# Bergvca/string_grouper

Hardware: AMD Instinct MI355X
Metric: hot-path rows/sec (the device path of match_strings: tokenise + tf-idf + postings + SpGEMM-topn, inputs resident in HBM), 663k-name self-join ntop=10 min_sim=0.8; match_strings end to end: match_strings_rows_per_s (higher is better)
Workload: dtype f32

## Files before the change

string_grouper_amd/csrc/sg_api.hip:

```cpp
#include <stdarg.h>
#include <stdlib.h>

#include "sg_internal.h"
#include "sg_scan.h"

static thread_local char g_err[512] = "";

void sg_set_error(const char *fmt, ...) {
    va_list ap;
    va_start(ap, fmt);
    vsnprintf(g_err, sizeof(g_err), fmt, ap);
    va_end(ap);
}

extern "C" const char *sg_last_error(void) { return g_err; }
extern "C" int sg_abi_version(void) { return SG_ABI_VERSION; }

extern "C" int sg_device_count(int *count) {
    SG_REQUIRE(count != nullptr, "count is null");
    int n = 0;
    hipError_t e = hipGetDeviceCount(&n);
    if (e != hipSuccess) {
        (void)hipGetLastError();
        n = 0;
// ... 345 lines not shown
    SG_HIP_TRY(hipMemcpyAsync(dp, indptr, sizeof(int64_t) * (size_t)(n_rows + 1), hipMemcpyHostToDevice, ctx->stream));
    if (nnz > 0) {
        SG_HIP_TRY(hipMemcpyAsync(di, indices, sizeof(int32_t) * (size_t)nnz, hipMemcpyHostToDevice, ctx->stream));
        SG_HIP_TRY(hipMemcpyAsync(dd, data, dtype_size(dtype) * (size_t)nnz, hipMemcpyHostToDevice, ctx->stream));
    }
    SG_HIP_TRY(hipStreamSynchronize(ctx->stream));
    *out = m;
    return SG_OK;
}

extern "C" int sg_csr_from_device(sg_ctx *ctx, int64_t n_rows, int64_t n_cols, int64_t nnz, const int64_t *d_indptr,
                                  const int32_t *d_indices, const void *d_data, int32_t dtype, sg_csr **out) {
    SG_REQUIRE(ctx && d_indptr && out, "null argument");
    SG_REQUIRE(n_rows >= 0 && n_cols >= 0 && nnz >= 0, "negative shape");
    SG_REQUIRE(dtype == SG_F32 || dtype == SG_F64, "dtype must be SG_F32 or SG_F64");
    if (n_cols > INT32_MAX || n_rows > INT32_MAX) {
        sg_set_error("matrix shape exceeds int32 indices");
        return SG_ERR_OVERFLOW;
    }
    sg_csr *m = new (std::nothrow) sg_csr();
    if (!m) return SG_ERR_OOM;
    m->ctx = ctx;
    m->n_rows = n_rows;
    m->n_cols = n_cols;
    m->nnz = nnz;
    m->dtype = dtype;
    m->d_indptr = d_indptr;
    m->d_indices = d_indices;
    m->d_data = d_data;
    m->owned = false;
    *out = m;
    return SG_OK;
}

extern "C" int sg_csr_dims(const sg_csr *m, int64_t *n_rows, int64_t *n_cols, int64_t *nnz, int32_t *dtype) {
    SG_REQUIRE(m != nullptr, "matrix is null");
    if (n_rows) *n_rows = m->n_rows;
    if (n_cols) *n_cols = m->n_cols;
    if (nnz) *nnz = m->nnz;
    if (dtype) *dtype = m->dtype;
    return SG_OK;
}

extern "C" int sg_csr_device_ptrs(const sg_csr *m, const int64_t **d_indptr, const int32_t **d_indices,
                                  const void **d_data) {
    SG_REQUIRE(m != nullptr, "matrix is null");
    if (d_indptr) *d_indptr = m->d_indptr;
    if (d_indices) *d_indices = m->d_indices;
    if (d_data) *d_data = m->d_data;
    return SG_OK;
}

extern "C" int sg_csr_to_host(sg_ctx *ctx, const sg_csr *m, int64_t *indptr, int32_t *indices, void *data) {
    SG_REQUIRE(ctx && m && indptr, "null argument");
    SG_HIP_TRY(hipMemcpyAsync(indptr, m->d_indptr, sizeof(int64_t) * (size_t)(m->n_rows + 1), hipMemcpyDeviceToHost,
                              ctx->stream));
    SG_HIP_TRY(hipStreamSynchronize(ctx->stream));
    const int64_t base = indptr[0];
    const int64_t nnz = indptr[m->n_rows] - base;
    if (nnz > 0) {
        SG_REQUIRE(indices && data, "null output");
        SG_HIP_TRY(hipMemcpyAsync(indices, m->d_indices + base, sizeof(int32_t) * (size_t)nnz, hipMemcpyDeviceToHost,
                                  ctx->stream));
        SG_HIP_TRY(hipMemcpyAsync(data, (const char *)m->d_data + dtype_size(m->dtype) * (size_t)base,
                                  dtype_size(m->dtype) * (size_t)nnz, hipMemcpyDeviceToHost, ctx->stream));
        SG_HIP_TRY(hipStreamSynchronize(ctx->stream));
    }
    if (base != 0)
        for (int64_t i = 0; i <= m->n_rows; ++i) indptr[i] -= base;
    return SG_OK;
}

extern "C" int sg_csr_row_block(sg_ctx *ctx, const sg_csr *m, int64_t r0, int64_t r1, sg_csr **out) {
    SG_REQUIRE(ctx && m && out, "null argument");
    SG_REQUIRE(0 <= r0 && r0 <= r1 && r1 <= m->n_rows, "row range out of bounds");
    sg_csr *v = new (std::nothrow) sg_csr();
    if (!v) return SG_ERR_OOM;
    *v = *m;
    v->owned = false;
    v->left_groups = nullptr;
    v->left_state = 0;
    v->n_rows = r1 - r0;
    v->d_indptr = m->d_indptr + r0;
    int64_t ends[2] = {0, 0};
    SG_HIP_TRY(hipMemcpyAsync(&ends[0], m->d_indptr + r0, sizeof(int64_t), hipMemcpyDeviceToHost, ctx->stream));
    SG_HIP_TRY(hipMemcpyAsync(&ends[1], m->d_indptr + r1, sizeof(int64_t), hipMemcpyDeviceToHost, ctx->stream));
    SG_HIP_TRY(hipStreamSynchronize(ctx->stream));
    v->nnz = ends[1] - ends[0];
    *out = v;
    return SG_OK;
}

extern "C" int sg_csr_free(sg_csr *m) {
    if (!m) return SG_OK;
    if (m->left_groups) sg_collapse_free(m->left_groups);
    if (m->owned) {
        m->ctx->release((void *)m->d_indptr);
        m->ctx->release((void *)m->d_indices);
        m->ctx->release((void *)m->d_data);
        m->ctx->release(m->d_props_words);
    }
    delete m;
    return SG_OK;
}

struct SgZeroJobs {
    uint32_t *ptr[8];
    uint64_t words[8];
    uint64_t first[8];
    int n;
};
__global__ void __launch_bounds__(256) zero_ranges_kernel(SgZeroJobs jobs) {
    const uint64_t total = jobs.first[jobs.n < 8 ? jobs.n : 7] + (jobs.n == 8 ? jobs.words[7] : 0);
    for (uint64_t q = ((uint64_t)blockIdx.x * blockDim.x + threadIdx.x) * 4; q < total; q += (uint64_t)gridDim.x * blockDim.x * 4) {
        int r = 0;
#pragma unroll
        for (int i = 1; i < 8; ++i)
            if (i < jobs.n && q >= jobs.first[i]) r = i;
        const uint64_t w = q - jobs.first[r];
        uint32_t *p = jobs.ptr[r] + w;
        const uint64_t left = jobs.words[r] - w;
        if (left >= 4 && ((uintptr_t)p & 15u) == 0) {
            *reinterpret_cast<uint4 *>(p) = make_uint4(0u, 0u, 0u, 0u);
        } else {
            for (uint64_t e = 0; e < 4 && e < left; ++e) p[e] = 0u;
        }
    }
}

int sg_zero_ranges(sg_ctx *ctx, int n, void *const *ptrs, const size_t *bytes) {
    SgZeroJobs jobs;
    jobs.n = 0;
    uint64_t first = 0;
    for (int i = 0; i < n; ++i) {
        if (!ptrs[i] || bytes[i] == 0) continue;
        if (jobs.n == 8 || (bytes[i] & 3u) || ((uintptr_t)ptrs[i] & 3u)) {
            SG_HIP_TRY(hipMemsetAsync(ptrs[i], 0, bytes[i], ctx->stream));
            continue;
        }
        jobs.ptr[jobs.n] = (uint32_t *)ptrs[i];
        jobs.words[jobs.n] = bytes[i] / 4;
        jobs.first[jobs.n] = first;
        first += (jobs.words[jobs.n] + 3) & ~(uint64_t)3;
        ++jobs.n;
    }
    if (jobs.n == 0) return SG_OK;
    for (int i = jobs.n; i < 8; ++i) {
        jobs.ptr[i] = nullptr;
        jobs.words[i] = 0;
        jobs.first[i] = first;
    }
    uint64_t threads = first / 4;
    unsigned grid = (unsigned)((threads + 255) / 256);
    if (grid > (unsigned)ctx->num_cu * 16u) grid = (unsigned)ctx->num_cu * 16u;
    if (grid < 1) grid = 1;
    hipLaunchKernelGGL(zero_ranges_kernel, dim3(grid), dim3(256), 0, ctx->stream, jobs);
    SG_HIP_TRY(hipGetLastError());
    return SG_OK;
}

int sg_exclusive_scan_u32(sg_ctx *ctx, const uint32_t *d_in, uint32_t *d_out, int64_t n, uint32_t *d_total) {
    return scan_impl<uint32_t, uint32_t>(ctx, d_in, d_out, n, d_total);
}

int sg_exclusive_scan_positive_i32(sg_ctx *ctx, const int32_t *d_in, uint32_t *d_out, int64_t n, uint32_t *d_total) {
    return scan_impl<int32_t, uint32_t, true>(ctx, d_in, d_out, n, d_total);
}

int sg_exclusive_scan_i32_to_i64(sg_ctx *ctx, const int32_t *d_in, int64_t *d_out, int64_t n) {
    return scan_impl<int32_t, int64_t>(ctx, d_in, d_out, n, d_out + n);
}

extern "C" int sg_device_upload(sg_ctx *ctx, const void *host, int64_t bytes, void **d_out) {
    SG_REQUIRE(ctx && d_out && bytes >= 0 && (bytes == 0 || host != nullptr), "null argument or negative size");
    void *d = nullptr;
    SG_TRY(ctx->alloc((size_t)std::max<int64_t>(bytes, 16), &d));
    hipError_t e = bytes > 0 ? hipMemcpyAsync(d, host, (size_t)bytes, hipMemcpyHostToDevice, ctx->stream) : hipSuccess;
    if (e == hipSuccess) e = hipStreamSynchronize(ctx->stream);
    if (e != hipSuccess) {
        ctx->release(d);
        sg_set_error("sg_device_upload: %s", hipGetErrorString(e));
        return SG_ERR_HIP;
    }
    *d_out = d;
    return SG_OK;
}
```

string_grouper_amd/csrc/sg_collapse.hip:

```cpp
#include "sg_internal.h"
#include "sg_scan.h"

template <typename T>
__global__ void __launch_bounds__(256) row_hash_kernel(const int64_t *__restrict__ indptr, const int32_t *__restrict__ indices,
                                                       const T *__restrict__ data, int64_t n_rows, uint64_t *__restrict__ hash,
                                                       uint32_t *__restrict__ row_id ) {
    const int64_t r = ((int64_t)blockIdx.x * blockDim.x + threadIdx.x) >> 4;
    const int sub = threadIdx.x & 15;
    uint64_t h = 0;
    if (r < n_rows) {
        const int64_t lo = indptr[r], hi = indptr[r + 1];
        for (int64_t p = lo + sub; p < hi; p += 16) {
            uint64_t v;
            if (sizeof(T) == 4) v = (uint64_t)__float_as_uint((float)data[p]);
            else v = (uint64_t)__double_as_longlong((double)data[p]);
            uint64_t x = ((uint64_t)(uint32_t)indices[p] << 32) ^ v ^ ((uint64_t)(p - lo) * 0x9E3779B97F4A7C15ull);
            x ^= x >> 33;
            x *= 0xff51afd7ed558ccdull;
            x ^= x >> 33;
            x *= 0xc4ceb9fe1a85ec53ull;
            x ^= x >> 33;
            h += x;
        }
    }
#pragma unroll
    for (int d = 8; d > 0; d >>= 1) {
        const uint32_t lo32 = (uint32_t)__shfl_xor((int)(uint32_t)h, d, 64), hi32 = (uint32_t)__shfl_xor((int)(uint32_t)(h >> 32), d, 64);
        h += ((uint64_t)hi32 << 32) | lo32;
    }
    if (r < n_rows && sub == 0) {
        const int64_t len = indptr[r + 1] - indptr[r];
        hash[r] = h ^ ((uint64_t)len * 0xD6E8FEB86659FD93ull);
        if (row_id) row_id[r] = (uint32_t)r;
    }
}

#define SG_GROUP_SORT_LDS 8192
#define SG_GROUP_LARGE_MAX 28u
#define SG_GROUP_NO_SLOT 0xFFFFFFFFu

#define SG_GROUP_ROWS 2
template <typename T>
__global__ void __launch_bounds__(256) group_rows_kernel(const int64_t *__restrict__ indptr, const int32_t *__restrict__ indices,
                                                         const T *__restrict__ data, int64_t n_rows, unsigned long long *table,
                                                         uint32_t mask, uint32_t *__restrict__ slot_of_row) {
    const int64_t grp = ((int64_t)blockIdx.x * blockDim.x + threadIdx.x) >> 4;
    const int sub = threadIdx.x & 15;
    const int lead = (int)(threadIdx.x & 48u);
    int64_t r[SG_GROUP_ROWS], lo[SG_GROUP_ROWS];
    int32_t len[SG_GROUP_ROWS];
    bool valid[SG_GROUP_ROWS];
#pragma unroll
    for (int i = 0; i < SG_GROUP_ROWS; ++i) {
        r[i] = grp * SG_GROUP_ROWS + i;
        valid[i] = r[i] < n_rows;
        lo[i] = valid[i] ? indptr[r[i]] : 0;
        len[i] = valid[i] ? (int32_t)(indptr[r[i] + 1] - lo[i]) : 0;
    }
    int32_t k0[SG_GROUP_ROWS], k1[SG_GROUP_ROWS];
    T v0[SG_GROUP_ROWS], v1[SG_GROUP_ROWS];
#pragma unroll
    for (int i = 0; i < SG_GROUP_ROWS; ++i) {
        k0[i] = k1[i] = -1;
        v0[i] = v1[i] = (T)0;
        if (sub < len[i]) {
            k0[i] = indices[lo[i] + sub];
            v0[i] = data[lo[i] + sub];
        }
        if (sub + 16 < len[i]) {
            k1[i] = indices[lo[i] + sub + 16];
            v1[i] = data[lo[i] + sub + 16];
        }
    }
    unsigned long long mine[SG_GROUP_ROWS];
    uint32_t s[SG_GROUP_ROWS], result[SG_GROUP_ROWS];
    bool walking[SG_GROUP_ROWS];
#pragma unroll
    for (int i = 0; i < SG_GROUP_ROWS; ++i) {
        uint64_t h = 0;
        for (int32_t e = sub; e < len[i]; e += 16) {
            const int32_t k = e < 16 ? k0[i] : (e < 32 ? k1[i] : indices[lo[i] + e]);
            const T v = e < 16 ? v0[i] : (e < 32 ? v1[i] : data[lo[i] + e]);
            uint64_t vb;
            if (sizeof(T) == 4) vb = (uint64_t)__float_as_uint((float)v);
            else vb = (uint64_t)__double_as_longlong((double)v);
            uint64_t x = ((uint64_t)(uint32_t)k << 32) ^ vb ^ ((uint64_t)e * 0x9E3779B97F4A7C15ull);
            x ^= x >> 33;
            x *= 0xff51afd7ed558ccdull;
            x ^= x >> 33;
            x *= 0xc4ceb9fe1a85ec53ull;
            x ^= x >> 33;
            h += x;
        }
#pragma unroll
        for (int d = 8; d > 0; d >>= 1) {
            const uint32_t lo32 = (uint32_t)__shfl_xor((int)(uint32_t)h, d, 64), hi32 = (uint32_t)__shfl_xor((int)(uint32_t)(h >> 32), d, 64);
            h += ((uint64_t)hi32 << 32) | lo32;
        }
        h ^= (uint64_t)(uint32_t)len[i] * 0xD6E8FEB86659FD93ull;
        h ^= h >> 31;
        mine[i] = ((unsigned long long)(uint32_t)(h >> 32) << 32) | (unsigned long long)(~(uint32_t)r[i]);
        s[i] = (uint32_t)h & mask;
        result[i] = SG_GROUP_NO_SLOT;
        walking[i] = valid[i];
    }
    while (__ballot(walking[0] || walking[1]) != 0) {
        unsigned long long cur[SG_GROUP_ROWS];
#pragma unroll
        for (int i = 0; i < SG_GROUP_ROWS; ++i) {
            cur[i] = 0;
            if (walking[i] && sub == 0) cur[i] = __hip_atomic_load(&table[s[i]], __ATOMIC_RELAXED, __HIP_MEMORY_SCOPE_AGENT);
        }
#pragma unroll
        for (int i = 0; i < SG_GROUP_ROWS; ++i)
            if (walking[i] && sub == 0 && cur[i] == 0ull) cur[i] = atomicCAS(&table[s[i]], 0ull, mine[i]);
        uint32_t c_lo[SG_GROUP_ROWS], c_hi[SG_GROUP_ROWS];
        bool cmp[SG_GROUP_ROWS];
        int64_t o[SG_GROUP_ROWS], olo[SG_GROUP_ROWS];
        int32_t olen[SG_GROUP_ROWS];
#pragma unroll
        for (int i = 0; i < SG_GROUP_ROWS; ++i) {
            c_lo[i] = (uint32_t)__shfl((int)(uint32_t)cur[i], lead, 64);
            c_hi[i] = (uint32_t)__shfl((int)(uint32_t)(cur[i] >> 32), lead, 64);
            cmp[i] = walking[i] && !(c_lo[i] == 0u && c_hi[i] == 0u) && c_hi[i] == (uint32_t)(mine[i] >> 32);
            o[i] = (int64_t)(~c_lo[i]);
            olo[i] = cmp[i] ? indptr[o[i]] : 0;
            olen[i] = cmp[i] ? (int32_t)(indptr[o[i] + 1] - olo[i]) : -1;
        }
        int32_t ok0[SG_GROUP_ROWS], ok1[SG_GROUP_ROWS];
        T ov0[SG_GROUP_ROWS], ov1[SG_GROUP_ROWS];
#pragma unroll
        for (int i = 0; i < SG_GROUP_ROWS; ++i) {
            const bool go = cmp[i] && olen[i] == len[i];
            ok0[i] = ok1[i] = -1;
            ov0[i] = ov1[i] = (T)0;
            if (go && sub < len[i]) {
                ok0[i] = indices[olo[i] + sub];
                ov0[i] = data[olo[i] + sub];
            }
            if (go && sub + 16 < len[i]) {
                ok1[i] = indices[olo[i] + sub + 16];
                ov1[i] = data[olo[i] + sub + 16];
            }
        }
#pragma unroll
        for (int i = 0; i < SG_GROUP_ROWS; ++i) {
            if (!walking[i]) continue;
            if (c_lo[i] == 0u && c_hi[i] == 0u) {
                result[i] = s[i];
                walking[i] = false;
            } else if (cmp[i]) {
                bool same = olen[i] == len[i];
                if (same) {
                    same = ok0[i] == k0[i] && ov0[i] == v0[i] && ok1[i] == k1[i] && ov1[i] == v1[i];
                    for (int32_t e = sub + 32; e < len[i]; e += 16)
                        same = same && indices[olo[i] + e] == indices[lo[i] + e] && data[olo[i] + e] == data[lo[i] + e];
                }
#pragma unroll
                for (int d = 8; d > 0; d >>= 1) same = same && (__shfl_xor((int)same, d, 64) != 0);
                if (same) {
                    if (sub == 0 && o[i] > r[i]) atomicMax(&table[s[i]], mine[i]);
                    result[i] = s[i];
                }
                walking[i] = false;
            } else {
                s[i] = (s[i] + 1u) & mask;
            }
        }
    }
#pragma unroll
    for (int i = 0; i < SG_GROUP_ROWS; ++i)
        if (valid[i] && sub == 0) slot_of_row[r[i]] = result[i];
}

__device__ __forceinline__ uint32_t sg_group_rep(const unsigned long long *__restrict__ table, const uint32_t *__restrict__ slot_of_row,
                                                 int64_t r) {
    const uint32_t s = slot_of_row[r];
    return s == SG_GROUP_NO_SLOT ? (uint32_t)r : ~(uint32_t)table[s];
}
struct GroupRepLoad {
    const unsigned long long *table;
    const uint32_t *slot_of_row;
    uint32_t *rep_of_row;
    __device__ __forceinline__ uint32_t operator()(int64_t r) const {
        const uint32_t rep = sg_group_rep(table, slot_of_row, r);
        rep_of_row[r] = rep;
        return rep == (uint32_t)r ? 1u : 0u;
    }
};

__global__ void __launch_bounds__(256) group_scatter_kernel(const uint32_t *__restrict__ gid, const uint32_t *__restrict__ group_ptr,
                                                            int64_t n_rows, uint32_t *cursor, uint32_t *__restrict__ members) {
    const int64_t r = (int64_t)blockIdx.x * blockDim.x + threadIdx.x;
    if (r >= n_rows) return;
    const uint32_t g = gid[r];
    const uint32_t lo = group_ptr[g], m = group_ptr[g + 1] - lo;
    if (m > (uint32_t)SG_GROUP_SORT_LDS) return;
    members[lo + (m == 1u ? 0u : atomicAdd(&cursor[g], 1u))] = (uint32_t)r;
}

__global__ void __launch_bounds__(256) large_group_flag_kernel(const uint32_t *__restrict__ gid, int64_t n_rows, uint32_t g,
                                                               uint32_t *__restrict__ flag) {
    const int64_t r = (int64_t)blockIdx.x * blockDim.x + threadIdx.x;
    if (r < n_rows) flag[r] = gid[r] == g ? 1u : 0u;
}
__global__ void __launch_bounds__(256) large_group_fill_kernel(const uint32_t *__restrict__ gid, const uint32_t *__restrict__ at,
                                                               int64_t n_rows, uint32_t g, const uint32_t *__restrict__ group_ptr,
                                                               uint32_t *__restrict__ members) {
    const int64_t r = (int64_t)blockIdx.x * blockDim.x + threadIdx.x;
    if (r < n_rows && gid[r] == g) members[group_ptr[g] + at[r]] = (uint32_t)r;
// ... 235 lines not shown
    }
    return st;
}

static int collapse_unique_matrix(sg_ctx *ctx, const sg_csr *B, SgCollapse *c, int64_t nnz_u, int64_t *ptr ,
                                  bool defer_rows) {
    const int64_t n_u = c->n_u;
    int32_t *idx = nullptr;
    void *val = nullptr;
    const size_t vs = B->dtype == SG_F64 ? 8 : 4;
    int st = SG_OK;
    if (!ptr) st = sg_alloc(ctx, (size_t)n_u + 2, &ptr);
    if (st == SG_OK) st = sg_alloc(ctx, (size_t)nnz_u + 64, &idx);
    if (st == SG_OK) st = ctx->alloc(((size_t)nnz_u + 64) * vs, &val);
    sg_csr *m = st == SG_OK ? new (std::nothrow) sg_csr() : nullptr;
    if (st == SG_OK && !m) st = SG_ERR_OOM;
    if (st != SG_OK) {
        ctx->release(ptr);
        ctx->release(idx);
        ctx->release(val);
        return st;
    }
    m->ctx = ctx;
    m->n_rows = n_u;
    m->n_cols = B->n_cols;
    m->nnz = nnz_u;
    m->dtype = B->dtype;
    m->d_indptr = ptr;
    m->d_indices = idx;
    m->d_data = val;
    m->owned = true;
    m->props_state = B->props_state;
    m->props_max_norm2 = B->props_max_norm2;
    m->props_max_nnz = B->props_max_nnz;
    m->rows_of = c;
    c->unique = m;
    c->pending_src = B;
    if (!defer_rows) return sg_collapse_materialize(ctx, c);
    return SG_OK;
}

static int collapse_groups_table(sg_ctx *ctx, const sg_csr *B, bool forced, bool defer_rows, SgCollapse **out) {
    *out = nullptr;
    ctx->group_table_overflow = false;
    const int64_t n = B->n_rows;
    uint64_t table_size = 1024;
    while (table_size < 2 * (uint64_t)n) table_size <<= 1;
    unsigned long long *table = nullptr;
    uint32_t *slot_of_row = nullptr, *rep_of_row = nullptr, *rep_excl = nullptr, *size = nullptr, *cursor = nullptr, *queue = nullptr;
    uint32_t *totals = nullptr;
    SgCollapse *c = new (std::nothrow) SgCollapse();
    if (!c) return SG_ERR_OOM;
    c->ctx = ctx;
    c->n_orig = n;
    int st = sg_alloc(ctx, (size_t)table_size, &table);
    if (st == SG_OK) st = sg_alloc(ctx, (size_t)n + 1, &slot_of_row);
    if (st == SG_OK) st = sg_alloc(ctx, (size_t)n + 1, &rep_of_row);
    if (st == SG_OK) st = sg_alloc(ctx, (size_t)n + 1, &rep_excl);
    if (st == SG_OK) st = sg_alloc(ctx, (size_t)n + 2, &size);
    if (st == SG_OK) st = sg_alloc(ctx, (size_t)n + 2, &cursor);
    if (st == SG_OK) st = sg_alloc(ctx, (size_t)n + 2, &queue);
    if (st == SG_OK) st = sg_alloc(ctx, (size_t)(64 + 32 * 32), &totals);
    if (st == SG_OK) st = sg_alloc(ctx, (size_t)n + 1, &c->d_gid);
    if (st == SG_OK) st = sg_alloc(ctx, (size_t)n + 2, &c->d_group_ptr);
    if (st == SG_OK) st = sg_alloc(ctx, (size_t)n + 1, &c->d_members);
    if (st == SG_OK) st = sg_alloc(ctx, (size_t)n + 1, &c->d_rep_rows);
    if (st == SG_OK) st = sg_alloc(ctx, (size_t)n + 2, &c->d_rep_start);
    if (st == SG_OK) st = sg_alloc(ctx, (size_t)n + 2, &c->d_rep_len);
    auto cleanup = [&]() {
        ctx->release(table);
        ctx->release(slot_of_row);
        ctx->release(rep_of_row);
        ctx->release(rep_excl);
        ctx->release(size);
        ctx->release(cursor);
        ctx->release(queue);
        ctx->release(totals);
    };
    const unsigned g1 = (unsigned)((n + 255) / 256), g16 = (unsigned)((((n + SG_GROUP_ROWS - 1) / SG_GROUP_ROWS) * 16 + 255) / 256);
    if (st == SG_OK)
        st = SG_ZERO4(ctx, table, sizeof(unsigned long long) * (size_t)table_size, size, sizeof(uint32_t) * (size_t)(n + 2), cursor,
                      sizeof(uint32_t) * (size_t)(n + 2), totals, (64 + 32 * 32) * sizeof(uint32_t));
    if (st == SG_OK) {
        if (B->dtype == SG_F64)
            hipLaunchKernelGGL(group_rows_kernel<double>, dim3(g16), dim3(256), 0, ctx->stream, B->d_indptr, B->d_indices,
                               (const double *)B->d_data, n, table, (uint32_t)(table_size - 1), slot_of_row);
        else
            hipLaunchKernelGGL(group_rows_kernel<float>, dim3(g16), dim3(256), 0, ctx->stream, B->d_indptr, B->d_indices,
                               (const float *)B->d_data, n, table, (uint32_t)(table_size - 1), slot_of_row);
        st = sg_scan_launch<uint32_t>(ctx, GroupRepLoad{table, slot_of_row, rep_of_row}, SgScanStoreArray<uint32_t>{rep_excl}, n, totals);
    }
    if (st == SG_OK) {
        hipLaunchKernelGGL(group_ids_kernel, dim3(g1), dim3(256), 0, ctx->stream, (const uint32_t *)rep_of_row, (const uint32_t *)rep_excl,
                           (const uint32_t *)nullptr, n, c->d_gid, size, c->d_rep_rows, B->d_indptr, c->d_rep_start, c->d_rep_len,
                           (unsigned long long *)(totals + 64));
        st = sg_exclusive_scan_u32(ctx, size, c->d_group_ptr, n + 1, nullptr);
    }
    if (st == SG_OK) {
        hipLaunchKernelGGL(group_scatter_kernel, dim3(g1), dim3(256), 0, ctx->stream, (const uint32_t *)c->d_gid,
                           (const uint32_t *)c->d_group_ptr, n, cursor, c->d_members);
        hipLaunchKernelGGL(group_sort_small_kernel, dim3(g1), dim3(256), 0, ctx->stream, (const uint32_t *)c->d_group_ptr,
                           (const uint32_t *)totals, c->d_members, totals + 4, queue);
        hipLaunchKernelGGL(group_sort_lds_kernel, dim3(512), dim3(256), 0, ctx->stream, (const uint32_t *)c->d_group_ptr, c->d_members,
                           (const uint32_t *)(totals + 4), (const uint32_t *)queue);
        if (hipGetLastError() != hipSuccess) st = SG_ERR_HIP;
    }
    uint32_t h[64 + 32 * 32];
    for (auto &w : h) w = 0;
    static_assert(sizeof(h) <= SG_H_FETCH_WORDS * sizeof(uint32_t), "the pinned read-back buffer holds the grouping's words");
    if (st == SG_OK) {
        if (hipMemcpyAsync(ctx->h_fetch, totals, sizeof(h), hipMemcpyDeviceToHost, ctx->stream) != hipSuccess ||
            hipStreamSynchronize(ctx->stream) != hipSuccess)
            st = SG_ERR_HIP;
        else memcpy(h, ctx->h_fetch, sizeof(h));
    }
    const uint32_t n_groups = h[0];
    int64_t nnz_u = 0;
    for (int q = 0; q < 32; ++q) nnz_u += (int64_t)(((uint64_t)h[64 + 32 * q + 1] << 32) | (uint64_t)h[64 + 32 * q]);
    const uint32_t *h_words = h + 4;
    if (st != SG_OK || n_groups == 0 || (!forced && (double)n_groups > 0.97 * (double)n) || (int64_t)n_groups == n) {
        cleanup();
        sg_collapse_free(c);
        return st;
    }
    if (h_words[2] > SG_GROUP_LARGE_MAX) {
        ctx->group_table_overflow = true;
        cleanup();
        sg_collapse_free(c);
        return SG_OK;
    }
    c->n_u = n_groups;
    for (uint32_t q = 0; q < h_words[2] && st == SG_OK; ++q) {
        const uint32_t g = h_words[3 + q];
        hipLaunchKernelGGL(large_group_flag_kernel, dim3(g1), dim3(256), 0, ctx->stream, (const uint32_t *)c->d_gid, n, g, size);
        st = sg_exclusive_scan_u32(ctx, size, rep_excl, n, nullptr);
        if (st == SG_OK) {
            hipLaunchKernelGGL(large_group_fill_kernel, dim3(g1), dim3(256), 0, ctx->stream, (const uint32_t *)c->d_gid,
                               (const uint32_t *)rep_excl, n, g, (const uint32_t *)c->d_group_ptr, c->d_members);
            if (hipGetLastError() != hipSuccess) st = SG_ERR_HIP;
        }
    }
    cleanup();
    if (st == SG_OK) st = collapse_unique_matrix(ctx, B, c, nnz_u, nullptr, defer_rows);
    if (st != SG_OK) {
        sg_collapse_free(c);
        return st;
    }
    *out = c;
    return SG_OK;
}

static int collapse_groups(sg_ctx *ctx, const sg_csr *B, bool forced, bool by_table, bool defer_rows, SgCollapse **out) {
    if (by_table) return collapse_groups_table(ctx, B, forced, defer_rows, out);
    *out = nullptr;
    ctx->group_table_overflow = false;
    const int64_t n = B->n_rows;
    uint64_t *hash = nullptr, *hash_sorted = nullptr;
    uint32_t *row_id = nullptr, *row_sorted = nullptr, *head = nullptr, *run_excl = nullptr, *head_pos = nullptr;
    uint32_t *rep_of_row = nullptr, *rank_of_row = nullptr, *is_rep = nullptr, *rep_excl = nullptr, *size = nullptr;
    uint32_t *totals = nullptr;
    SgCollapse *c = nullptr;
    int st = sg_alloc(ctx, (size_t)n + 1, &hash);
    if (st == SG_OK) st = sg_alloc(ctx, (size_t)40, &totals);
    if (st == SG_OK) st = sg_alloc(ctx, (size_t)n + 1, &hash_sorted);
    if (st == SG_OK) st = sg_alloc(ctx, (size_t)n + 1, &row_id);
    if (st == SG_OK) st = sg_alloc(ctx, (size_t)n + 1, &row_sorted);
    if (st == SG_OK) st = sg_alloc(ctx, (size_t)n + 1, &head);
    if (st == SG_OK) st = sg_alloc(ctx, (size_t)n + 1, &run_excl);
    auto cleanup = [&]() {
        ctx->release(hash);
        ctx->release(hash_sorted);
        ctx->release(row_id);
// ... 254 lines not shown
```

string_grouper_amd/csrc/sg_internal.h:

```cpp
#pragma once

#include <hip/hip_runtime.h>
#include <stdint.h>
#include <stdio.h>
#include <stdlib.h>
#include <string.h>

#include <map>
#include <mutex>
#include <new>
#include <string>
#include <vector>

#include "../../include/sg_hip.h"

#define SG_WAVE 64
#define SG_NUM_XCD 8

void sg_set_error(const char *fmt, ...);

#define SG_HIP_TRY(expr)                                                                        \
    do {                                                                                        \
        hipError_t _e = (expr);                                                                 \
        if (_e != hipSuccess) {                                                                 \
// ... 44 lines not shown
    uint32_t *h_fetch = nullptr;

    std::map<std::string, std::string> opts;
    const char *opt(const char *name) const {
        auto it = opts.find(name);
        return it == opts.end() ? nullptr : it->second.c_str();
    }
    int opt_int(const char *name, int dflt) const {
        const char *v = opt(name);
        return v && *v ? atoi(v) : dflt;
    }
    double opt_double(const char *name, double dflt) const {
        const char *v = opt(name);
        return v && *v ? atof(v) : dflt;
    }
    bool opt_is(const char *name, char c) const {
        const char *v = opt(name);
        return v && v[0] == c;
    }
    bool poison = false;

    unsigned long long *d_scan_desc = nullptr;
    size_t scan_desc_cap = 0;
    uint32_t scan_ticket_base = 0, scan_epoch = 0;
    struct IdfTable {
        int64_t n_docs;
        int32_t dtype;
        void *d;
        bool trusted;
    };
    std::vector<IdfTable> idf_tables;
    int inner_multiply_depth = 0;
    bool group_table_overflow = false;

    int alloc(size_t bytes, void **out);
    void release(void *p);
    void trim();
};

template <typename T>
static inline int sg_alloc(sg_ctx *ctx, size_t count, T **out) {
    void *p = nullptr;
    int s = ctx->alloc(count * sizeof(T), &p);
    *out = (T *)p;
    return s;
}

struct SgTimer {
    sg_ctx *ctx;
    int which;
    SgTimer(sg_ctx *c, int w) : ctx(c), which(w) { (void)hipEventRecord(ctx->ev_start[w], ctx->stream); }
    ~SgTimer() {
        (void)hipEventRecord(ctx->ev_stop[which], ctx->stream);
        ctx->ev_valid[which] = true;
    }
};

struct sg_strings {
    sg_ctx *ctx = nullptr;
    const uint8_t *d_bytes = nullptr;
    const int64_t *d_offsets = nullptr;
    int64_t n = 0;
    int64_t total_bytes = 0;
    bool owned = false;
    int32_t sym_width = 1;
    int32_t alphabet = 0;
    bool prelowered = false;
};

struct sg_csr {
    sg_ctx *ctx = nullptr;
    int64_t n_rows = 0, n_cols = 0, nnz = 0;
    int32_t dtype = SG_F32;
    const int64_t *d_indptr = nullptr;
    const int32_t *d_indices = nullptr;
    const void *d_data = nullptr;
    bool owned = false;
    mutable int props_state = 0;
    mutable float props_max_norm2 = 0.f;
    mutable uint32_t props_max_nnz = 0;
    bool from_vectoriser = false;
    mutable bool props_by_construction = false;
    uint32_t *d_props_words = nullptr;
    mutable int left_state = 0;
    mutable struct SgCollapse *left_groups = nullptr;
    struct SgCollapse *rows_of = nullptr;
};

struct SgScoreCtx {
    const uint32_t *fwd_ptr = nullptr;
    const void *fwd = nullptr;
    const uint32_t *orig_of = nullptr;
    const void *blk = nullptr;
    uint32_t blk_bytes = 0;
    const uint4 *q8 = nullptr;
    float q8_scale = 0.f;
    uint32_t pad_ = 0;
};
#define SG_Q8_STRIDE 256u
#define SG_Q8_MAX_ENTRIES 60u

struct SgCollapse {
    sg_ctx *ctx = nullptr;
    int64_t n_orig = 0, n_u = 0;
    uint32_t *d_gid = nullptr;
    uint32_t *d_group_ptr = nullptr;
    uint32_t *d_members = nullptr;
    uint32_t *d_rep_rows = nullptr;
    int64_t *d_rep_start = nullptr;
    int32_t *d_rep_len = nullptr;
    struct sg_csr *unique = nullptr;
    const struct sg_csr *pending_src = nullptr;
};

struct sg_postings {
    sg_ctx *ctx = nullptr;
    int64_t n_right = 0, n_terms = 0, nnz = 0;
    int32_t dtype = SG_F32;
    int32_t tile_log2 = 12;
    int32_t n_tiles = 0;
    const int64_t *b_indptr = nullptr;
    const int32_t *b_indices = nullptr;
    const void *b_data = nullptr;
    uint32_t *d_seg = nullptr;
    uint32_t *d_term_len = nullptr;
    uint32_t *d_term_start = nullptr;
    int32_t *d_rows = nullptr;
    void *d_vals = nullptr;
    sg_csr src;
    int32_t split = 1;
    void *d_fwd = nullptr;
    uint32_t *d_fwd_ptr = nullptr;
    void *d_blk = nullptr;
    uint32_t blk_bytes = 0;
    void *d_q8 = nullptr;
    uint32_t *d_filt = nullptr;
    sg_csr *permuted = nullptr;
    uint32_t *d_orig_of = nullptr, *d_pos_of = nullptr;
    struct SgScoreCtx *d_score_ctx = nullptr;
    uint32_t *d_ends = nullptr;
    int32_t nt_pad = 0;
    int32_t fold_log2 = 0;
    uint32_t *d_ends8 = nullptr;
    int32_t nv_pad = 0;
    float norm_up = 0.f;
    uint32_t freq_min = 0;
    bool cosine_like = false;
    float max_norm2 = 0.f;
    SgCollapse *collapse = nullptr;
    const sg_csr *caller_b = nullptr;
    sg_csr caller_b_copy;
    int64_t n_right_caller = 0;
    mutable sg_postings *plain = nullptr;
    mutable sg_postings *exact_native = nullptr;
    mutable sg_postings *alt_tile = nullptr;
    sg_csr built_from;
    bool built_from_valid = false;
    bool tile_form = false;
    const sg_postings *view_of = nullptr;
    int32_t build_tile_cols = 0, build_flags = 0;
};

struct sg_topn {
    sg_ctx *ctx = nullptr;
    int64_t n_rows = 0, n_cols = 0;
    int32_t stride = 0;
    int32_t dtype = SG_F32;
    int32_t top_n_asked = 0;
    int32_t *d_cols = nullptr;
    void *d_vals = nullptr;
    int32_t *d_counts = nullptr;
};

struct sg_vocab {
    sg_ctx *ctx = nullptr;
    sg_vec_params params;
    int32_t bits_per_char = 7;
    int64_t n_terms = 0, n_docs = 0;
    int64_t key_space = 0;
    bool sorted_mode = false;
    int32_t *d_key_to_col = nullptr;
    uint64_t *d_keys = nullptr;
    int32_t *d_df = nullptr;
    void *d_idf = nullptr;
    bool idf_trusted = false;
    struct VocabImpl *impl = nullptr;
};

int sg_matchlist_device_view(const sg_matchlist *ml, int64_t *n_rows, int64_t *n_cols, int64_t *n_entries, int32_t *dtype,
                             const int64_t **row_ptr, const int32_t **cols, const void **vals);

#define SG_POSTINGS_NO_COLLAPSE (1 << 8)
#define SG_POSTINGS_TILE_FORM (1 << 11)
#define SG_POSTINGS_EXACT_ONLY (1 << 10)
int sg_csr_props(sg_ctx *ctx, const sg_csr *m, bool *cosine_like, float *max_norm2, uint32_t *max_nnz = nullptr);
bool sg_pruned_supports_tile(int32_t tile_log2);
int sg_postings_ensure_full(sg_ctx *ctx, const sg_postings *p);
bool sg_q8_applies(const sg_ctx *ctx, const sg_postings *Bt, double threshold);
int sg_spgemm_pruned_launch(sg_ctx *ctx, const sg_csr *A, const sg_postings *Bt, int32_t keep, sg_topn *r,
                            double threshold, double delta, uint32_t *row_counter,
                            uint32_t *flagged_count, uint32_t *flagged_rows, unsigned long long *stats);

int sg_spgemm_pruned_symmetric(sg_ctx *ctx, const sg_csr *A, const sg_postings *Bt, int32_t keep, sg_topn *r,
                               double threshold, double delta, unsigned long long *stats, bool *done, int64_t row_lo = 0,
                               int64_t row_hi = -1 , int32_t **export_pairs = nullptr,
                               int64_t *export_n = nullptr, int64_t row_step = 1 ,
                               bool exact_all = false );
int sg_selfjoin_merge_pairs(sg_ctx *ctx, sg_topn *r, const int32_t *d_pairs, int64_t n_pairs, int64_t row_lo, int64_t row_hi,
                            const uint32_t *pos_of ,
                            int64_t row_step = 1);

#define SG_PAIR_CHUNK 256u
#define SG_PAIR_NO_CHUNK 0xFFFFFFFFu
struct SgPairSink {
    uint32_t *d_i = nullptr;
    uint32_t *d_j = nullptr;
    void *d_s = nullptr;
    uint32_t *d_row_count = nullptr;
    uint32_t *d_chunk_count = nullptr;
    uint32_t *d_chunks_used = nullptr;
    unsigned long long *d_totals = nullptr;
    uint32_t chunks = 0;
};
unsigned sg_spgemm_exact_selfjoin_grid(const sg_ctx *ctx, const sg_postings *Bt = nullptr );
int sg_spgemm_exact_selfjoin_rows(sg_ctx *ctx, const sg_csr *A, const sg_postings *Bt, int32_t keep, sg_topn *r,
                                  double threshold, uint32_t *row_counter, const uint32_t *row_list,
                                  const uint32_t *row_list_len, const SgPairSink &sink, bool all_rows = false);

int sg_collapse_build(sg_ctx *ctx, const sg_csr *B, SgCollapse **out, bool left_side = false, bool defer_rows = false);
int sg_collapse_materialize(sg_ctx *ctx, SgCollapse *c);
int sg_csr_ensure_rows(sg_ctx *ctx, const sg_csr *m);
void sg_collapse_free(SgCollapse *c);
int sg_collapse_expand(sg_ctx *ctx, const SgCollapse *c, const sg_topn *ru, bool rows_are_groups, sg_topn *out,
                       const int32_t *row_list = nullptr);
int sg_sort_pairs_u64_u32(sg_ctx *ctx, const uint64_t *d_keys, const uint32_t *d_vals, int64_t n, uint64_t *d_keys_out,
                          uint32_t *d_vals_out);
int sg_sort_unique_u64(sg_ctx *ctx, uint64_t *d_keys, int64_t n, uint64_t *d_unique, int32_t *d_counts, int64_t *n_unique);

int sg_zero_ranges(sg_ctx *ctx, int n, void *const *ptrs, const size_t *bytes);
#define SG_ZERO2(ctx, p0, b0, p1, b1) [&]() { void *const pp_[] = {(void *)(p0), (void *)(p1)}; const size_t bb_[] = {(size_t)(b0), (size_t)(b1)}; return sg_zero_ranges(ctx, 2, pp_, bb_); }()
#define SG_ZERO3(ctx, p0, b0, p1, b1, p2, b2) [&]() { void *const pp_[] = {(void *)(p0), (void *)(p1), (void *)(p2)}; const size_t bb_[] = {(size_t)(b0), (size_t)(b1), (size_t)(b2)}; return sg_zero_ranges(ctx, 3, pp_, bb_); }()
#define SG_ZERO4(ctx, p0, b0, p1, b1, p2, b2, p3, b3) [&]() { void *const pp_[] = {(void *)(p0), (void *)(p1), (void *)(p2), (void *)(p3)}; const size_t bb_[] = {(size_t)(b0), (size_t)(b1), (size_t)(b2), (size_t)(b3)}; return sg_zero_ranges(ctx, 4, pp_, bb_); }()
int sg_exclusive_scan_positive_i32(sg_ctx *ctx, const int32_t *d_in, uint32_t *d_out, int64_t n, uint32_t *d_total);
int sg_exclusive_scan_u32(sg_ctx *ctx, const uint32_t *d_in, uint32_t *d_out, int64_t n, uint32_t *d_total);
int sg_exclusive_scan_i32_to_i64(sg_ctx *ctx, const int32_t *d_in, int64_t *d_out, int64_t n);
```

string_grouper_amd/csrc/sg_postings.hip:

```cpp
#include <stdlib.h>

#include "sg_internal.h"
#include "sg_scan.h"

__device__ __forceinline__ int64_t row_of_thread(int64_t g, int32_t tile_log2, int32_t n_tiles) {
    return ((g % n_tiles) << tile_log2) | (g / n_tiles);
}

template <typename T>
__global__ void __launch_bounds__(256) postings_count(const int64_t *__restrict__ indptr,
                                                      const int32_t *__restrict__ indices, int64_t n_rows,
                                                      int32_t tile_log2, int32_t n_tiles, uint32_t *seg_counts) {
    const int64_t j = row_of_thread((int64_t)blockIdx.x * blockDim.x + threadIdx.x, tile_log2, n_tiles);
    if (j >= n_rows) return;
    const int64_t lo = indptr[j], hi = indptr[j + 1];
    const uint32_t t = (uint32_t)(j >> tile_log2);
    for (int64_t p = lo; p < hi; ++p) {
        const int64_t bin = (int64_t)indices[p] * n_tiles + t;
        atomicAdd(&seg_counts[bin], 1u);
    }
}

template <typename T>
__device__ __forceinline__ void store_posting(int32_t *rows, T *vals, uint32_t pos, int32_t j, T v);
// ... 205 lines not shown
    uint32_t *freq_bits = cursor + n_terms;
    const int64_t t = blockIdx.x / split;
    const int32_t part = blockIdx.x % split;
    for (int k = threadIdx.x; k < (n_terms + 31) / 32; k += blockDim.x) freq_bits[k] = 0;
    const uint32_t *mine = cnt + (int64_t)blockIdx.x * n_terms;
    for (int k = threadIdx.x; k < n_terms; k += blockDim.x) cursor[k] = term_start[k] + mine[k];
    __syncthreads();
    if (out_filt)
        for (int k = threadIdx.x; k < n_terms; k += blockDim.x)
            if (is_frequent[k]) atomicOr(&freq_bits[k >> 5], 1u << (k & 31));
    __syncthreads();
    const int64_t part_rows = ((int64_t)1 << tile_log2) / split;
    const int64_t j0 = (t << tile_log2) + part * part_rows;
    int64_t j1 = j0 + part_rows;
    if (j1 > n_rows) j1 = n_rows;
    const int lane = threadIdx.x & 63, sub = lane & 15;
    (void)lane;
    const int64_t groups = blockDim.x >> 4;
    const int64_t trips = (j1 - j0 + groups * SG_POST_ROWS - 1) / (groups * SG_POST_ROWS);
    for (int64_t it = 0; it < trips; ++it) {
        const int64_t jb = j0 + (it * groups + (threadIdx.x >> 4)) * SG_POST_ROWS;
        int64_t lo[SG_POST_ROWS], hi[SG_POST_ROWS];
#pragma unroll
        for (int r = 0; r < SG_POST_ROWS; ++r) {
            const bool valid = jb + r < j1;
            lo[r] = valid ? indptr[jb + r] : 0;
            hi[r] = valid ? indptr[jb + r + 1] : 0;
        }
        int32_t k0[SG_POST_ROWS];
        T v0[SG_POST_ROWS];
#pragma unroll
        for (int r = 0; r < SG_POST_ROWS; ++r) {
            const bool have = lo[r] + sub < hi[r];
            k0[r] = have ? indices[lo[r] + sub] : -1;
            v0[r] = have ? data[lo[r] + sub] : (T)0;
        }
        float fq[SG_POST_ROWS];
#pragma unroll
        for (int r = 0; r < SG_POST_ROWS; ++r) {
            fq[r] = 0.f;
#if defined(SG_K3_PROBE_NO_FQ)
            if (out_filt && n_rows < 0) {
#else
            if (out_filt) {
#endif
                double f2 = 0.0;
                if (k0[r] >= 0 && ((freq_bits[k0[r] >> 5] >> (k0[r] & 31)) & 1u)) f2 = (double)v0[r] * (double)v0[r];
                for (int64_t p = lo[r] + sub + 16; p < hi[r]; p += 16) {
                    const int32_t k = indices[p];
                    if ((freq_bits[k >> 5] >> (k & 31)) & 1u) f2 += (double)data[p] * (double)data[p];
                }
#pragma unroll
                for (int d = 8; d > 0; d >>= 1) {
                    const uint64_t bits = (uint64_t)__double_as_longlong(f2);
                    const uint32_t l = (uint32_t)__shfl_xor((int)(uint32_t)bits, d, 64), h = (uint32_t)__shfl_xor((int)(uint32_t)(bits >> 32), d, 64);
                    f2 += __longlong_as_double((long long)(((uint64_t)h << 32) | l));
                }
                fq[r] = frequent_norm_ratio_of(f2, inv_norm_up);
            }
        }
#pragma unroll
        for (int r = 0; r < SG_POST_ROWS; ++r) {
            const uint32_t col = (uint32_t)(jb + r - (t << tile_log2));
            if (k0[r] >= 0) {
#if defined(SG_K3_PROBE_NO_ATOMIC)
                const uint32_t pos = cursor[k0[r]] + (uint32_t)(threadIdx.x & 3);
#else
                const uint32_t pos = atomicAdd(&cursor[k0[r]], 1u);
#endif
#if defined(SG_K3_PROBE_NO_STORE)
                if (pos == 0xFFFFFFF0u)
#endif
                emit_posting<T>(out_rows, out_vals, out_filt, pos, col, v0[r], fq[r], tile_log2, inv_norm_up, (uint32_t)t, fold_log2);
            }
            for (int64_t p = lo[r] + sub + 16; p < hi[r]; p += 16) {
                const uint32_t pos = atomicAdd(&cursor[indices[p]], 1u);
                emit_posting<T>(out_rows, out_vals, out_filt, pos, col, data[p], fq[r], tile_log2, inv_norm_up, (uint32_t)t, fold_log2);
            }
        }
    }
}

__device__ __forceinline__ uint32_t lds_get16(const uint32_t *w, uint32_t k) { return (w[k >> 1] >> ((k & 1u) << 4)) & 0xffffu; }
template <typename T>
__global__ void __launch_bounds__(1024) postings_fill_staged(const int64_t *__restrict__ indptr, const int32_t *__restrict__ indices,
                                                             const T *__restrict__ data, int64_t n_rows, int32_t tile_log2,
                                                             int32_t n_terms, int32_t split, int32_t chunk_rows, uint32_t stage_cap,
                                                             uint32_t *cnt , const uint32_t *__restrict__ term_start,
                                                             const uint8_t *__restrict__ is_frequent, uint32_t *__restrict__ out_filt,
                                                             float inv_norm_up, int32_t fold_log2) {
    extern __shared__ uint32_t lds[];
    const uint32_t w16 = ((uint32_t)n_terms + 1u) >> 1;
    uint32_t *lcnt = lds;
    uint32_t *freq_bits = lcnt + ((w16 + 3u) & ~3u);
    float *fqrow = reinterpret_cast<float *>(freq_bits + (((uint32_t)n_terms + 31u) >> 5));
    uint32_t *wave_tot = reinterpret_cast<uint32_t *>(fqrow + chunk_rows);
    uint32_t *stage = wave_tot + 32;
    const int64_t t = blockIdx.x / split;
    const int32_t part = blockIdx.x % split;
    uint32_t *mine = cnt + (int64_t)blockIdx.x * n_terms;
    for (uint32_t k = threadIdx.x; k < (((uint32_t)n_terms + 31u) >> 5); k += blockDim.x) freq_bits[k] = 0;
    __syncthreads();
    for (int k = threadIdx.x; k < n_terms; k += blockDim.x)
        if (is_frequent[k]) atomicOr(&freq_bits[k >> 5], 1u << (k & 31));
    __syncthreads();
    const int64_t part_rows = ((int64_t)1 << tile_log2) / split;
    const int64_t j0 = (t << tile_log2) + part * part_rows;
    int64_t j1 = j0 + part_rows;
    if (j1 > n_rows) j1 = n_rows;
    const int lane = threadIdx.x & 63, sub = lane & 15, wave = threadIdx.x >> 6;
    const int64_t groups = blockDim.x >> 4;
    const uint32_t last_k = (uint32_t)n_terms - 1u;
    bool any_big = false;
    for (int64_t c0 = j0; c0 < j1; c0 += chunk_rows) {
        const int64_t c1 = c0 + chunk_rows < j1 ? c0 + chunk_rows : j1;
        const int64_t e = indptr[c1] - indptr[c0];
        any_big = any_big || e > (int64_t)stage_cap || e > 65535;
    }
    for (int64_t c0 = j0; c0 < j1; c0 += chunk_rows) {
        const int64_t c1 = c0 + chunk_rows < j1 ? c0 + chunk_rows : j1;
        const int64_t trips = (c1 - c0 + groups * SG_POST_ROWS - 1) / (groups * SG_POST_ROWS);
        if (any_big) {
            for (int64_t it = 0; it < trips; ++it) {
                const int64_t jb = c0 + (it * groups + (threadIdx.x >> 4)) * SG_POST_ROWS;
#pragma unroll
                for (int r = 0; r < SG_POST_ROWS; ++r) {
                    const bool valid = jb + r < c1;
                    const int64_t lo = valid ? indptr[jb + r] : 0, hi = valid ? indptr[jb + r + 1] : 0;
                    double f2 = 0.0;
                    for (int64_t p = lo + sub; p < hi; p += 16) {
                        const int32_t k = indices[p];
                        if ((freq_bits[k >> 5] >> (k & 31)) & 1u) f2 += (double)data[p] * (double)data[p];
                    }
#pragma unroll
                    for (int d = 8; d > 0; d >>= 1) {
                        const uint64_t bits = (uint64_t)__double_as_longlong(f2);
                        const uint32_t l = (uint32_t)__shfl_xor((int)(uint32_t)bits, d, 64), h = (uint32_t)__shfl_xor((int)(uint32_t)(bits >> 32), d, 64);
                        f2 += __longlong_as_double((long long)(((uint64_t)h << 32) | l));
                    }
                    const float fq = frequent_norm_ratio_of(f2, inv_norm_up);
                    const uint32_t col = (uint32_t)(jb + r - (t << tile_log2));
                    for (int64_t p = lo + sub; p < hi; p += 16) {
                        const int32_t k = indices[p];
                        const uint32_t pos = term_start[k] + atomicAdd(&mine[k], 1u);
                        out_filt[pos] = filter_posting(col, (float)data[p], fq, tile_log2, inv_norm_up, (uint32_t)t, fold_log2);
                    }
                }
            }
            __syncthreads();
            continue;
        }
        for (uint32_t w = threadIdx.x; w < w16; w += blockDim.x) lcnt[w] = 0;
        __syncthreads();
        for (int64_t it = 0; it < trips; ++it) {
            const int64_t jb = c0 + (it * groups + (threadIdx.x >> 4)) * SG_POST_ROWS;
            int64_t lo[SG_POST_ROWS], hi[SG_POST_ROWS];
#pragma unroll
            for (int r = 0; r < SG_POST_ROWS; ++r) {
                const bool valid = jb + r < c1;
                lo[r] = valid ? indptr[jb + r] : 0;
                hi[r] = valid ? indptr[jb + r + 1] : 0;
            }
            int32_t k0[SG_POST_ROWS];
            T v0[SG_POST_ROWS];
#pragma unroll
            for (int r = 0; r < SG_POST_ROWS; ++r) {
                const bool have = lo[r] + sub < hi[r];
                k0[r] = have ? indices[lo[r] + sub] : -1;
                v0[r] = have ? data[lo[r] + sub] : (T)0;
            }
#pragma unroll
            for (int r = 0; r < SG_POST_ROWS; ++r) {
                double f2 = 0.0;
                if (k0[r] >= 0) {
                    atomicAdd(&lcnt[(uint32_t)k0[r] >> 1], 1u << (((uint32_t)k0[r] & 1u) << 4));
                    if ((freq_bits[k0[r] >> 5] >> (k0[r] & 31)) & 1u) f2 = (double)v0[r] * (double)v0[r];
                }
                for (int64_t p = lo[r] + sub + 16; p < hi[r]; p += 16) {
                    const int32_t k = indices[p];
                    atomicAdd(&lcnt[(uint32_t)k >> 1], 1u << (((uint32_t)k & 1u) << 4));
                    if ((freq_bits[k >> 5] >> (k & 31)) & 1u) f2 += (double)data[p] * (double)data[p];
                }
#pragma unroll
                for (int d = 8; d > 0; d >>= 1) {
                    const uint64_t bits = (uint64_t)__double_as_longlong(f2);
                    const uint32_t l = (uint32_t)__shfl_xor((int)(uint32_t)bits, d, 64), h = (uint32_t)__shfl_xor((int)(uint32_t)(bits >> 32), d, 64);
                    f2 += __longlong_as_double((long long)(((uint64_t)h << 32) | l));
                }
                if (sub == 0 && jb + r < c1) fqrow[jb + r - c0] = frequent_norm_ratio_of(f2, inv_norm_up);
            }
        }
        __syncthreads();
        {
            const uint32_t per = (w16 + blockDim.x - 1u) / blockDim.x;
            const uint32_t wa = threadIdx.x * per, wb = wa + per < w16 ? wa + per : w16;
            uint32_t sum = 0;
            for (uint32_t w = wa; w < wb; ++w) sum += (lcnt[w] & 0xffffu) + (lcnt[w] >> 16);
            uint32_t tot;
            uint32_t run = block_exclusive_scan<uint32_t>(sum, wave_tot, &tot);
            for (uint32_t w = wa; w < wb; ++w) {
                const uint32_t c = lcnt[w];
                const uint32_t a = run;
                run += c & 0xffffu;
                const uint32_t b = run;
                run += c >> 16;
                lcnt[w] = a | (b << 16);
            }
        }
        __syncthreads();
        for (int64_t it = 0; it < trips; ++it) {
            const int64_t jb = c0 + (it * groups + (threadIdx.x >> 4)) * SG_POST_ROWS;
            int64_t lo[SG_POST_ROWS], hi[SG_POST_ROWS];
#pragma unroll
            for (int r = 0; r < SG_POST_ROWS; ++r) {
                const bool valid = jb + r < c1;
                lo[r] = valid ? indptr[jb + r] : 0;
                hi[r] = valid ? indptr[jb + r + 1] : 0;
            }
            int32_t k0[SG_POST_ROWS];
            T v0[SG_POST_ROWS];
#pragma unroll
            for (int r = 0; r < SG_POST_ROWS; ++r) {
                const bool have = lo[r] + sub < hi[r];
                k0[r] = have ? indices[lo[r] + sub] : -1;
                v0[r] = have ? data[lo[r] + sub] : (T)0;
            }
#pragma unroll
            for (int r = 0; r < SG_POST_ROWS; ++r) {
                const float fq = jb + r < c1 ? fqrow[jb + r - c0] : 0.f;
                const uint32_t col = (uint32_t)(jb + r - (t << tile_log2));
                if (k0[r] >= 0) {
                    const uint32_t sh = ((uint32_t)k0[r] & 1u) << 4;
                    const uint32_t pos = (atomicAdd(&lcnt[(uint32_t)k0[r] >> 1], 1u << sh) >> sh) & 0xffffu;
                    stage[pos] = filter_posting(col, (float)v0[r], fq, tile_log2, inv_norm_up, (uint32_t)t, fold_log2);
                }
                for (int64_t p = lo[r] + sub + 16; p < hi[r]; p += 16) {
                    const uint32_t k = (uint32_t)indices[p];
                    const uint32_t sh = (k & 1u) << 4;
                    const uint32_t pos = (atomicAdd(&lcnt[k >> 1], 1u << sh) >> sh) & 0xffffu;
                    stage[pos] = filter_posting(col, (float)data[p], fq, tile_log2, inv_norm_up, (uint32_t)t, fold_log2);
                }
            }
        }
        __syncthreads();
        {
            constexpr int FB = 8;
            const uint32_t n_tg = ((uint32_t)n_terms + 63u) >> 6, waves = (uint32_t)(blockDim.x >> 6);
            for (uint32_t tg0 = (uint32_t)wave; tg0 < n_tg; tg0 += waves * FB) {
                uint32_t end_k[FB], start_k[FB], before[FB], G[FB];
                bool mine_has[FB];
#pragma unroll
                for (int b = 0; b < FB; ++b) {
                    const uint32_t tg = tg0 + (uint32_t)b * waves;
                    const uint32_t k = tg * 64u + (uint32_t)lane;
                    const bool live = tg < n_tg;
                    const uint32_t kc = k < last_k ? k : last_k;
                    end_k[b] = live ? lds_get16(lcnt, kc) : 0u;
                    start_k[b] = (!live || k == 0u) ? 0u : lds_get16(lcnt, (k - 1u) < last_k ? k - 1u : last_k);
                    mine_has[b] = live && k <= last_k && end_k[b] > start_k[b];
                }
#pragma unroll
                for (int b = 0; b < FB; ++b) {
                    const uint32_t k = (tg0 + (uint32_t)b * waves) * 64u + (uint32_t)lane;
                    before[b] = mine_has[b] ? mine[k] : 0u;
                    G[b] = mine_has[b] ? term_start[k] : 0u;
                }
#pragma unroll
                for (int b = 0; b < FB; ++b) {
                    const uint32_t tg = tg0 + (uint32_t)b * waves;
                    if (tg >= n_tg) break;
                    const uint32_t k = tg * 64u + (uint32_t)lane;
                    G[b] += before[b];
                    const uint32_t S = (uint32_t)__builtin_amdgcn_readlane((int)start_k[b], 0);
                    const uint32_t Eg = (uint32_t)__builtin_amdgcn_readlane((int)end_k[b], 63);
                    for (uint32_t e0 = S; e0 < Eg; e0 += 64u) {
                        const uint32_t e = e0 + (uint32_t)lane;
                        uint32_t lo = 0u, hi = 63u;
#pragma unroll
                        for (int step = 0; step < 6; ++step) {
                            const uint32_t mid = (lo + hi) >> 1;
                            const uint32_t km = tg * 64u + mid;
                            const bool right = lds_get16(lcnt, km < last_k ? km : last_k) > e;
                            hi = right ? mid : hi;
                            lo = right ? lo : mid + 1u;
                        }
                        const uint32_t tsel = lo < 63u ? lo : 63u;
                        const uint32_t kt = tg * 64u + tsel;
                        const uint32_t start_t = kt == 0u ? 0u : lds_get16(lcnt, (kt - 1u) < last_k ? kt - 1u : last_k);
                        const uint32_t G_t = (uint32_t)__shfl((int)G[b], (int)tsel, 64);
                        if (e < Eg) out_filt[G_t + (e - start_t)] = stage[e];
                    }
                    if (mine_has[b]) mine[k] = before[b] + (end_k[b] - start_k[b]);
                }
            }
        }
        __syncthreads();
    }
}

__global__ void __launch_bounds__(256) term_len_kernel(const uint32_t *__restrict__ seg, int64_t n_terms, int32_t n_tiles,
                                                       uint32_t *__restrict__ term_len) {
    const int64_t k = (int64_t)blockIdx.x * blockDim.x + threadIdx.x;
    if (k < n_terms) term_len[k] = seg[(k + 1) * n_tiles] - seg[k * n_tiles];
}

template <typename T>
__global__ void __launch_bounds__(256) fwd_pack(const int64_t *__restrict__ indptr, const int32_t *__restrict__ indices,
                                                const T *__restrict__ data, int64_t n_rows, int64_t nnz,
                                                const uint32_t *__restrict__ orig_of ,
                                                uint32_t *__restrict__ fwd_ptr , void *__restrict__ fwd) {
    const int64_t i = (int64_t)blockIdx.x * blockDim.x + threadIdx.x;
    const int64_t base = indptr[0];
    if (i <= n_rows)
        reinterpret_cast<uint2 *>(fwd_ptr)[i] = make_uint2((uint32_t)(indptr[i] - base), i < n_rows ? (orig_of ? orig_of[i] : (uint32_t)i) : 0u);
    if (i >= nnz || fwd == nullptr) return;
    const int64_t p = base + i;
    if (sizeof(T) == 4) {
        reinterpret_cast<int2 *>(fwd)[i] = make_int2(indices[p], __float_as_int((float)data[p]));
    } else {
        const long long bits = __double_as_longlong((double)data[p]);
        reinterpret_cast<int4 *>(fwd)[i] = make_int4(indices[p], 0, (int)(bits & 0xffffffffll), (int)(bits >> 32));
    }
}

template <typename T>
__global__ void __launch_bounds__(256) row_blocks_kernel(const int64_t *__restrict__ indptr, const int32_t *__restrict__ indices,
                                                         const T *__restrict__ data, int64_t n_rows,
                                                         const uint32_t *__restrict__ orig_of ,
                                                         uint32_t blk_bytes, void *__restrict__ blk) {
    constexpr int ES = sizeof(T) == 4 ? 8 : 16;
    const int64_t chunks = blk_bytes / 16;
    const int64_t g = (int64_t)blockIdx.x * blockDim.x + threadIdx.x;
    const int64_t p = g / chunks;
    const int32_t c = (int32_t)(g - p * chunks);
    if (p >= n_rows) return;
    const int64_t lo = indptr[p];
    const int32_t nnz = (int32_t)(indptr[p + 1] - lo);
    const int32_t used = (((nnz + 1) * ES + 127) / 128) * 128;
    if (c * 16 >= used) return;
    uint4 w = make_uint4(0u, 0u, 0u, 0u);
    if (sizeof(T) == 4) {
        const int32_t e0 = 2 * c, e1 = 2 * c + 1;
        if (e0 == 0) {
            w.x = orig_of ? orig_of[p] : (uint32_t)p;
            w.y = (uint32_t)nnz;
        } else if (e0 <= nnz) {
            w.x = (uint32_t)indices[lo + e0 - 1];
            w.y = __float_as_uint((float)data[lo + e0 - 1]);
        }
        if (e1 <= nnz) {
            w.z = (uint32_t)indices[lo + e1 - 1];
            w.w = __float_as_uint((float)data[lo + e1 - 1]);
        }
    } else {
        if (c == 0) {
            w.x = orig_of ? orig_of[p] : (uint32_t)p;
            w.y = (uint32_t)nnz;
        } else if (c <= nnz) {
            const long long bits = __double_as_longlong((double)data[lo + c - 1]);
            w.x = (uint32_t)indices[lo + c - 1];
            w.z = (uint32_t)(bits & 0xffffffffll);
            w.w = (uint32_t)(bits >> 32);
        }
    }
    reinterpret_cast<uint4 *>(reinterpret_cast<char *>(blk) + (size_t)p * blk_bytes)[c] = w;
}

__global__ void __launch_bounds__(256) ends_from_seg_kernel(const uint32_t *__restrict__ seg, int64_t n_terms, int32_t n_tiles,
                                                            uint32_t *__restrict__ ends, int32_t nt_pad, uint32_t *__restrict__ ends8,
                                                            int32_t nv_pad, int32_t fold_log2) {
    const int64_t k = (int64_t)blockIdx.x * blockDim.x + threadIdx.x;
    if (k > n_terms) return;
    if (ends)
        for (int32_t t = 0; t < nt_pad; ++t)
            ends[k * nt_pad + t] = k == n_terms ? 0u : seg[k * n_tiles + (t < n_tiles ? t : n_tiles - 1) + 1] << 2;
// ... 235 lines not shown
    if (st == SG_OK) st = sg_alloc(ctx, (size_t)B->nnz + 64, &idx);
    if (st == SG_OK) st = ctx->alloc(((size_t)B->nnz + 64) * vs, &val);
    if (st == SG_OK)
        st = sg_scan_launch<int64_t>(ctx, PermutedLenLoad{n, minv, (uint64_t)(~0ull / n) + 1ull, by_group ? pending->d_rep_len : (const int32_t *)nullptr, B->d_indptr, pos_of, orig_of},
                                     SgScanStoreArray<int64_t>{ptr}, (int64_t)n, ptr + n);
    if (st == SG_OK) {
        const unsigned grid = (unsigned)((((n + 1 + SG_GATHER_ROWS - 1) / SG_GATHER_ROWS) * 16 + 255) / 256);
        const sg_csr *src = from_groups ? pending->pending_src : B;
        const uint32_t *rep_rows = from_groups ? pending->d_rep_rows : nullptr;
        const int64_t *rep_start = by_group ? pending->d_rep_start : nullptr;
        const int32_t *rep_len = by_group ? pending->d_rep_len : nullptr;
        if (B->dtype == SG_F64)
            hipLaunchKernelGGL(gather_rows_kernel<double>, dim3(grid), dim3(256), 0, ctx->stream, src->d_indptr, src->d_indices,
                               (const double *)src->d_data, B->n_rows, (const uint32_t *)orig_of, rep_rows, rep_start, rep_len,
                               (const int64_t *)ptr, idx, (double *)val, fwd_ptr, fwd, (uint4 *)(fwd_ptr ? q8 : nullptr), inv_norm);
        else
            hipLaunchKernelGGL(gather_rows_kernel<float>, dim3(grid), dim3(256), 0, ctx->stream, src->d_indptr, src->d_indices,
                               (const float *)src->d_data, B->n_rows, (const uint32_t *)orig_of, rep_rows, rep_start, rep_len,
                               (const int64_t *)ptr, idx, (float *)val, fwd_ptr, fwd, (uint4 *)(fwd_ptr ? q8 : nullptr), inv_norm);
        if (hipGetLastError() != hipSuccess) st = SG_ERR_HIP;
        if (st == SG_OK) *fwd_done = fwd_ptr != nullptr;
    }
    ctx->release(len_by_pos);
    sg_csr *m = st == SG_OK ? new (std::nothrow) sg_csr() : nullptr;
    if (st == SG_OK && !m) st = SG_ERR_OOM;
    if (st != SG_OK) {
        ctx->release(orig_of);
        ctx->release(pos_of);
        ctx->release(ptr);
        ctx->release(idx);
        ctx->release(val);
        return st;
    }
    m->ctx = ctx;
    m->n_rows = B->n_rows;
    m->n_cols = B->n_cols;
    m->nnz = B->nnz;
    m->dtype = B->dtype;
    m->d_indptr = ptr;
    m->d_indices = idx;
    m->d_data = val;
    m->owned = true;
    m->props_state = B->props_state;
    m->props_max_norm2 = B->props_max_norm2;
    m->props_max_nnz = B->props_max_nnz;
    *out_perm = m;
    *out_orig_of = orig_of;
    *out_pos_of = pos_of;
    return SG_OK;
}

extern "C" int sg_postings_build(sg_ctx *ctx, const sg_csr *B, int32_t tile_cols, sg_postings **out) {
    return sg_postings_build_flags(ctx, B, tile_cols, 0, out);
}

#define SG_POSTINGS_INNER (1 << 9)

static thread_local SgCollapse *tl_pending_groups = nullptr;

extern "C" int sg_postings_build_flags(sg_ctx *ctx, const sg_csr *B_in, int32_t tile_cols, int32_t flags, sg_postings **out) {
    SG_REQUIRE(ctx && B_in && out, "null argument");
    SgCollapse *pending = tl_pending_groups;
    tl_pending_groups = nullptr;
    if (!(flags & SG_POSTINGS_NO_COLLAPSE)) {
        bool cl = false;
        float n2 = 0.f;
        SG_TRY(sg_csr_props(ctx, B_in, &cl, &n2));
        SgCollapse *col = nullptr;
        SgTimer timer(ctx, SG_K_POSTINGS);
        if (cl) SG_TRY(sg_collapse_build(ctx, B_in, &col, false, true));
        if (col) {
            sg_postings *inner = nullptr;
            tl_pending_groups = col;
            const int st = sg_postings_build_flags(ctx, col->unique, tile_cols, flags | SG_POSTINGS_NO_COLLAPSE | SG_POSTINGS_INNER, &inner);
            tl_pending_groups = nullptr;
            if (st != SG_OK) {
                sg_collapse_free(col);
                return st;
            }
            inner->collapse = col;
            inner->caller_b_copy = *B_in;
            inner->caller_b_copy.owned = false;
            inner->caller_b_copy.d_props_words = nullptr;
            inner->caller_b_copy.left_groups = nullptr;
            inner->caller_b_copy.left_state = 0;
            inner->caller_b = &inner->caller_b_copy;
            inner->n_right_caller = B_in->n_rows;
            inner->build_tile_cols = tile_cols;
            inner->build_flags = flags;
            *out = inner;
            return SG_OK;
        }
        flags |= SG_POSTINGS_INNER;
        const int st = sg_postings_build_flags(ctx, B_in, tile_cols, flags | SG_POSTINGS_NO_COLLAPSE, out);
        if (st == SG_OK) {
            (*out)->build_tile_cols = tile_cols;
            (*out)->build_flags = flags & 0xff;
        }
        return st;
    }
    const sg_csr *B = B_in;
    bool cosine_like = false;
    float max_norm2 = 0.f;
    SG_TRY(sg_csr_props(ctx, B, &cosine_like, &max_norm2));
    const char *pr = ctx->opt("SG_PRUNE");
    const bool want_pruned = cosine_like && !(pr && pr[0] == '0') && !(flags & SG_POSTINGS_EXACT_ONLY);
    if (tile_cols == 0) {
        tile_cols = B->dtype == SG_F64 ? 1024 : 2048;
        if (want_pruned) {
            tile_cols = 4096;
            if (flags & SG_POSTINGS_TILE_FORM) tile_cols = 2048;
            else if (const char *v = ctx->opt("SG_PRUNE_TILE")) tile_cols = atoi(v) == 13 ? 8192 : (atoi(v) == 11 ? 2048 : 4096);
        }
    }
    SG_REQUIRE(tile_cols >= 256 && tile_cols <= 32768 && (tile_cols & (tile_cols - 1)) == 0,
               "tile_cols must be a power of two in [256, 32768]");
    int64_t max_entries = (int64_t)1 << 29;
    if (const char *v = ctx->opt("SG_MAX_POSTINGS")) {
        const long long o = atoll(v);
        if (o > 0 && o < max_entries) max_entries = o;
    }
    if (B->nnz + 64 >= max_entries) {
        sg_set_error("right-hand matrix has %lld non-zeros; one postings block holds < 2^29 (use more right-hand blocks)",
                     (long long)B->nnz);
        return SG_ERR_OVERFLOW;
    }
    int32_t tile_log2 = 0;
    while ((1 << tile_log2) < tile_cols) ++tile_log2;
    const int64_t n_tiles64 = B->n_rows == 0 ? 1 : ((B->n_rows + tile_cols - 1) >> tile_log2);
    const int64_t n_bins = B->n_cols * n_tiles64;
    if (n_bins + 1 >= (int64_t)1 << 31) {
        sg_set_error("segment table of %lld x %lld entries is too large; use more right-hand blocks",
                     (long long)B->n_cols, (long long)n_tiles64);
        return SG_ERR_OVERFLOW;
    }
    sg_csr *permuted = nullptr;
    uint32_t *orig_of = nullptr, *pos_of = nullptr;
    SgTimer *timer = (flags & SG_POSTINGS_INNER) ? nullptr : new (std::nothrow) SgTimer(ctx, SG_K_POSTINGS);
    struct TimerGuard {
        SgTimer *t;
        ~TimerGuard() { delete t; }
    } timer_guard{timer};
    void *early_fwd = nullptr;
    uint32_t *early_fwd_ptr = nullptr;
    void *early_q8 = nullptr;
    const float norm_up_build = __builtin_nextafterf(sqrtf(max_norm2) * 1.000001f, 2.f);
    const bool q8_forced = ctx->opt("SG_Q8") && ctx->opt("SG_Q8")[0] == '1';
    const bool want_q8 = want_pruned && !(flags & SG_POSTINGS_TILE_FORM) && B_in->n_cols < ((int64_t)1 << 24) && !(ctx->opt("SG_Q8") && ctx->opt("SG_Q8")[0] == '0') &&
                         (q8_forced || (double)B_in->nnz <= 45.0 * (double)B_in->n_rows) &&
                         (ctx->total_mem == 0 || (size_t)SG_Q8_STRIDE * ((size_t)B_in->n_rows + 1) < ctx->total_mem / 16);
    bool fwd_done = false;
    bool aux_written = false;
    {
        const bool filt = want_pruned && sg_pruned_supports_tile(tile_log2) &&
                          (B->n_cols + 1) * ((n_tiles64 + 3) & ~(int64_t)3) < ((int64_t)1 << 30);
        const bool blk = ctx->opt("SG_ROW_BLOCKS") && ctx->opt("SG_ROW_BLOCKS")[0] == '1';
        if (filt && !blk && !(flags & SG_POSTINGS_NO_PERMUTATION) && B_in->n_rows > 0) {
            int st0 = ctx->alloc(((size_t)B_in->nnz + 8) * (B_in->dtype == SG_F64 ? 16 : 8), &early_fwd);
            if (st0 == SG_OK) st0 = sg_alloc(ctx, 2 * ((size_t)B_in->n_rows + 2), &early_fwd_ptr);
            if (st0 == SG_OK && want_q8) st0 = ctx->alloc((size_t)SG_Q8_STRIDE * ((size_t)B_in->n_rows + 1), &early_q8);
            if (st0 != SG_OK) {
                ctx->release(early_fwd);
                ctx->release(early_fwd_ptr);
                return st0;
            }
        }
    }
    if (!(flags & SG_POSTINGS_NO_PERMUTATION)) {
        const int stp = build_permuted(ctx, B_in, tile_cols, &permuted, &orig_of, &pos_of, pending, early_fwd_ptr, early_fwd, &fwd_done,
                                       early_q8, 1.0f / norm_up_build);
        if (stp != SG_OK) {
            ctx->release(early_fwd);
            ctx->release(early_fwd_ptr);
            ctx->release(early_q8);
            return stp;
        }
    }
    if (!fwd_done) {
        ctx->release(early_fwd);
        ctx->release(early_fwd_ptr);
        ctx->release(early_q8);
        early_fwd = nullptr;
        early_fwd_ptr = nullptr;
        early_q8 = nullptr;
    }
    if (pending && pending->pending_src && !permuted) {
        const int stm = sg_collapse_materialize(ctx, pending);
        if (stm != SG_OK) {
            sg_csr_free(permuted);
            ctx->release(orig_of);
            ctx->release(pos_of);
            return stm;
        }
    }
    if (permuted) B = permuted;
    sg_postings *p = new (std::nothrow) sg_postings();
    if (!p) {
        sg_csr_free(permuted);
        ctx->release(orig_of);
        ctx->release(pos_of);
        ctx->release(early_fwd);
        ctx->release(early_fwd_ptr);
        ctx->release(early_q8);
        return SG_ERR_OOM;
    }
    p->permuted = permuted;
    p->d_orig_of = orig_of;
    p->d_pos_of = pos_of;
    p->ctx = ctx;
    p->n_right = B->n_rows;
    p->n_terms = B->n_cols;
    p->nnz = B->nnz;
    p->dtype = B->dtype;
    p->tile_log2 = tile_log2;
    p->tile_form = (flags & SG_POSTINGS_TILE_FORM) != 0;
    p->built_from = *B_in;
    p->built_from.owned = false;
    p->built_from.d_props_words = nullptr;
    p->built_from.left_groups = nullptr;
    p->built_from.left_state = 0;
    p->built_from_valid = true;
    p->n_tiles = (int32_t)n_tiles64;
    p->b_indptr = B_in->d_indptr;
    p->b_indices = B_in->d_indices;
    p->b_data = B_in->d_data;
    p->cosine_like = cosine_like;
    p->max_norm2 = max_norm2;
    const size_t vs = 8;
    int st = sg_alloc(ctx, (size_t)n_bins + 1, &p->d_seg);
    if (st == SG_OK) st = sg_alloc(ctx, (size_t)B->n_cols + 1, &p->d_term_len);
    const bool will_filter = want_pruned && sg_pruned_supports_tile(tile_log2) &&
                             (B->n_cols + 1) * ((n_tiles64 + 3) & ~(int64_t)3) < ((int64_t)1 << 30);
    const size_t lds_need = (size_t)B->n_cols * 4 + ((size_t)(B->n_cols + 31) / 32) * 4;
    bool lds_path = B->n_rows > 0 && lds_need <= 124 * 1024 && B->n_cols > 0;
    if (const char *e = ctx->opt("SG_POSTINGS_LDS")) lds_path = lds_path && e[0] != '0';
    const bool lazy_full = will_filter && lds_path && !(ctx->opt("SG_POSTINGS_LAZY") && ctx->opt("SG_POSTINGS_LAZY")[0] == '0');
    p->src = *B;
    p->src.owned = false;
    p->src.d_props_words = nullptr;
    p->src.left_groups = nullptr;
    p->src.left_state = 0;
    if (st == SG_OK && !lazy_full && B->dtype == SG_F64) st = sg_alloc(ctx, (size_t)B->nnz + 64, &p->d_rows);
    if (st == SG_OK && !lazy_full) st = ctx->alloc(((size_t)B->nnz + 64) * vs, &p->d_vals);
    if (st == SG_OK && will_filter) {
        {
            uint32_t max_nnz = 0;
            bool cl = false;
            float n2 = 0.f;
            const bool want_blk = ctx->opt("SG_ROW_BLOCKS") && ctx->opt("SG_ROW_BLOCKS")[0] == '1';
            if (want_blk) {
                if (B->props_max_nnz == 0 && !B->d_props_words) B->props_state = 0;
                st = sg_csr_props(ctx, B, &cl, &n2, &max_nnz);
            }
            const size_t es = B->dtype == SG_F64 ? 16 : 8;
            const size_t need = (((size_t)max_nnz + 1) * es + 127) / 128 * 128;
            if (st == SG_OK && want_blk && need <= 1024 && (double)need * (double)B->n_rows < 3.5e9 &&
                (ctx->total_mem == 0 || need * (size_t)B->n_rows < ctx->total_mem / 8)) {
                p->blk_bytes = (uint32_t)need;
                st = ctx->alloc(need * ((size_t)B->n_rows + 1), &p->d_blk);
            }
        }
        if (early_fwd && !p->d_blk) {
            p->d_fwd = early_fwd;
            p->d_fwd_ptr = early_fwd_ptr;
            p->d_q8 = early_q8;
            early_fwd = nullptr;
            early_fwd_ptr = nullptr;
            early_q8 = nullptr;
        } else {
            if (st == SG_OK && !p->d_blk) st = ctx->alloc(((size_t)B->nnz + 8) * (B->dtype == SG_F64 ? 16 : 8), &p->d_fwd);
            if (st == SG_OK) st = sg_alloc(ctx, 2 * ((size_t)B->n_rows + 2), &p->d_fwd_ptr);
            if (st == SG_OK && want_q8 && !p->d_blk) st = ctx->alloc((size_t)SG_Q8_STRIDE * ((size_t)B->n_rows + 1), &p->d_q8);
            fwd_done = false;
        }
        if (st == SG_OK) st = sg_alloc(ctx, (size_t)B->nnz + 512, &p->d_filt);
        p->nt_pad = (int32_t)((n_tiles64 + 3) & ~(int64_t)3);
        if (st == SG_OK) st = sg_alloc(ctx, (size_t)(B->n_cols + 1) * (size_t)p->nt_pad + 4, &p->d_ends);
        p->fold_log2 = 0;
        if (tile_log2 == 12 && !(ctx->opt("SG_K4_STREAM") && ctx->opt("SG_K4_STREAM")[0] == '0')) p->fold_log2 = 3;
        if (p->fold_log2 > 0) {
            const int64_t n_super = (n_tiles64 + ((int64_t)1 << p->fold_log2) - 1) >> p->fold_log2;
            p->nv_pad = (int32_t)((n_super + 3) & ~(int64_t)3);
            if (st == SG_OK) st = sg_alloc(ctx, (size_t)(B->n_cols + 1) * (size_t)p->nv_pad + 4, &p->d_ends8);
        }
        p->norm_up = norm_up_build;
        double frac = 0.005;
        if (const char *v = ctx->opt("SG_PRUNE_FREQ")) frac = atof(v);
        const double fm = frac * (double)B->n_rows;
        p->freq_min = fm < 1.0 ? 1u : (uint32_t)fm;
    }
    ctx->release(early_fwd);
    ctx->release(early_fwd_ptr);
    ctx->release(early_q8);
    if (st != SG_OK) {
        sg_postings_free(p);
        return st;
    }
    {
        const unsigned grid = (unsigned)((((int64_t)p->n_tiles << tile_log2) + 255) / 256);
        const size_t lds = (size_t)B->n_cols * 4 + ((size_t)(B->n_cols + 31) / 32) * 4;
        bool in_lds = B->n_rows > 0 && lds <= 124 * 1024 && B->n_cols > 0;
        if (const char *e = ctx->opt("SG_POSTINGS_LDS")) in_lds = in_lds && e[0] != '0';
        const float inv_norm = p->d_filt ? 1.0f / p->norm_up : 0.f;
        bool tables_done = false;
        if (in_lds) {
            static bool attr_done = false;
            if (!attr_done) {
                (void)hipFuncSetAttribute((const void *)postings_count_lds, hipFuncAttributeMaxDynamicSharedMemorySize, 124 * 1024);
                (void)hipFuncSetAttribute((const void *)postings_fill_lds<float>, hipFuncAttributeMaxDynamicSharedMemorySize, 124 * 1024);
                (void)hipFuncSetAttribute((const void *)postings_fill_lds<double>, hipFuncAttributeMaxDynamicSharedMemorySize, 124 * 1024);
                (void)hipFuncSetAttribute((const void *)postings_fill_staged<float>, hipFuncAttributeMaxDynamicSharedMemorySize, 160 * 1024);
                (void)hipFuncSetAttribute((const void *)postings_fill_staged<double>, hipFuncAttributeMaxDynamicSharedMemorySize, 160 * 1024);
                attr_done = true;
            }
            bool staged = p->d_filt != nullptr && p->d_vals == nullptr && !(ctx->opt("SG_FILL_STAGED") && ctx->opt("SG_FILL_STAGED")[0] == '0');
            uint32_t stage_cap = 0;
            int32_t chunk_rows = 0;
            size_t staged_lds = 0;
            const double mean_nnz = B->n_rows > 0 ? (double)B->nnz / (double)B->n_rows : 1.0;
            if (staged) {
                const size_t fixed0 = ((((size_t)B->n_cols + 1) / 2 + 3) & ~(size_t)3) * 4 + (((size_t)B->n_cols + 31) / 32) * 4 + 32 * 4;
                chunk_rows = 2048;
                for (;;) {
                    const size_t fixed = fixed0 + (size_t)chunk_rows * 4;
                    const size_t room = fixed + 16384 < 158 * 1024 ? 158 * 1024 - fixed : 0;
                    stage_cap = (uint32_t)(room / 4);
                    if (stage_cap > 65535u) stage_cap = 65535u;
                    if ((double)chunk_rows * mean_nnz * 1.2 + 64.0 <= (double)stage_cap || chunk_rows <= 64) break;
                    chunk_rows >>= 1;
                }
                staged = (double)chunk_rows * mean_nnz * 1.2 + 64.0 <= (double)stage_cap;
                staged_lds = fixed0 + (size_t)chunk_rows * 4 + (size_t)stage_cap * 4;
                if (const char *v = ctx->opt("SG_FILL_STAGE_CAP"))
                    if (atoi(v) > 0 && (uint32_t)atoi(v) < stage_cap) stage_cap = (uint32_t)atoi(v);
            }
            int32_t split = 1;
            while (split < 4 && (int64_t)p->n_tiles * split < ctx->num_cu && (tile_cols / (split * 2)) >= 1024 &&
                   (n_bins * split * 2 + 1) < ((int64_t)1 << 31))
                split *= 2;
            if (staged)
                while (split < 8 && (int64_t)p->n_tiles * split < 2 * (int64_t)ctx->num_cu && (tile_cols / (split * 2)) >= 512 &&
                       (n_bins * split * 2 + 1) < ((int64_t)1 << 31))
                    split *= 2;
            if (const char *e = ctx->opt("SG_POSTINGS_SPLIT")) {
                const int o = atoi(e);
                if ((o == 1 || o == 2 || o == 4) && tile_cols / o >= 64 && n_bins * o + 1 < ((int64_t)1 << 31)) split = o;
            }
            p->split = split;
            const int64_t wgs64 = (int64_t)p->n_tiles * split;
            uint32_t *cnt = nullptr;
            uint8_t *is_frequent = nullptr;
            st = sg_alloc(ctx, (size_t)(wgs64 * B->n_cols) + 1, &cnt);
            if (st == SG_OK) st = sg_alloc(ctx, (size_t)B->n_cols + 4, &is_frequent);
            if (st == SG_OK) st = sg_alloc(ctx, (size_t)B->n_cols + 2, &p->d_term_start);
            if (st == SG_OK) {
                const unsigned wgs = (unsigned)wgs64;
                const unsigned strips = (unsigned)((B->n_cols + 63) / 64), strips1 = (unsigned)((B->n_cols + 64) / 64);
                hipLaunchKernelGGL(postings_count_lds, dim3(wgs), dim3(1024), (size_t)B->n_cols * 4, ctx->stream, B->d_indptr,
                                   B->d_indices, B->n_rows, tile_log2, (int32_t)B->n_cols, split, cnt);
                hipLaunchKernelGGL(postings_colscan_kernel, dim3(strips), dim3(1024), 0, ctx->stream, cnt, (int32_t)wgs64,
                                   (int32_t)B->n_cols, p->freq_min, p->d_term_len, is_frequent);
                st = sg_exclusive_scan_u32(ctx, p->d_term_len, p->d_term_start, B->n_cols, p->d_term_start + B->n_cols);
                if (st == SG_OK) {
                    if (staged)
                        ;
                    else if (B->dtype == SG_F64)
                        hipLaunchKernelGGL(postings_fill_lds<double>, dim3(wgs), dim3(1024), lds, ctx->stream, B->d_indptr,
                                           B->d_indices, (const double *)B->d_data, B->n_rows, tile_log2, (int32_t)B->n_cols, split,
                                           (const uint32_t *)cnt, (const uint32_t *)p->d_term_start, (const uint8_t *)is_frequent,
                                           p->d_rows, (double *)p->d_vals, p->d_filt, inv_norm, p->fold_log2);
                    else
                        hipLaunchKernelGGL(postings_fill_lds<float>, dim3(wgs), dim3(1024), lds, ctx->stream, B->d_indptr,
                                           B->d_indices, (const float *)B->d_data, B->n_rows, tile_log2, (int32_t)B->n_cols, split,
                                           (const uint32_t *)cnt, (const uint32_t *)p->d_term_start, (const uint8_t *)is_frequent,
                                           p->d_rows, (float *)p->d_vals, p->d_filt, inv_norm, p->fold_log2);
                    SgScoreCtx sc;
                    if (p->d_fwd_ptr) {
                        st = ctx->alloc(256, (void **)&p->d_score_ctx);
                        sc.fwd_ptr = p->d_fwd_ptr;
                        sc.fwd = p->d_fwd;
                        sc.blk = p->d_blk;
                        sc.blk_bytes = p->blk_bytes;
                        sc.orig_of = p->d_orig_of;
                        sc.q8 = (const uint4 *)p->d_q8;
                        sc.q8_scale = p->d_q8 ? __builtin_nextafterf((float)(255.0 / (double)p->norm_up * (1.0 - 1e-6)), 0.f) : 0.f;
                    }
                    if (st == SG_OK) {
                        hipLaunchKernelGGL(postings_tables_kernel, dim3(strips1), dim3(1024), 0, ctx->stream, (const uint32_t *)cnt,
                                           (const uint32_t *)p->d_term_start, (int32_t)B->n_cols, p->n_tiles, split, p->d_seg, p->d_ends,
                                           p->nt_pad, p->d_ends8, p->nv_pad, p->fold_log2, sc, p->d_score_ctx,
                                           p->d_filt ? p->d_filt + B->nnz : (uint32_t *)nullptr);
                        if (staged && B->dtype == SG_F64)
                            hipLaunchKernelGGL(postings_fill_staged<double>, dim3(wgs), dim3(1024), staged_lds, ctx->stream, B->d_indptr,
                                               B->d_indices, (const double *)B->d_data, B->n_rows, tile_log2, (int32_t)B->n_cols, split,
                                               chunk_rows, stage_cap, cnt, (const uint32_t *)p->d_term_start, (const uint8_t *)is_frequent,
                                               p->d_filt, inv_norm, p->fold_log2);
                        else if (staged)
                            hipLaunchKernelGGL(postings_fill_staged<float>, dim3(wgs), dim3(1024), staged_lds, ctx->stream, B->d_indptr,
                                               B->d_indices, (const float *)B->d_data, B->n_rows, tile_log2, (int32_t)B->n_cols, split,
                                               chunk_rows, stage_cap, cnt, (const uint32_t *)p->d_term_start, (const uint8_t *)is_frequent,
                                               p->d_filt, inv_norm, p->fold_log2);
                        if (hipGetLastError() != hipSuccess) st = SG_ERR_HIP;
                        aux_written = st == SG_OK;
                    }
                }
            }
            ctx->release(cnt);
            ctx->release(is_frequent);
            tables_done = true;
        } else {
            uint32_t *cursor = nullptr;
            st = sg_alloc(ctx, (size_t)n_bins + 1, &cursor);
            if (st == SG_OK) {
                SG_HIP_TRY(hipMemsetAsync(p->d_seg, 0, sizeof(uint32_t) * (size_t)(n_bins + 1), ctx->stream));
                SG_HIP_TRY(hipMemsetAsync(cursor, 0, sizeof(uint32_t) * (size_t)(n_bins + 1), ctx->stream));
            }
            if (st == SG_OK && grid > 0) {
                if (B->dtype == SG_F64)
                    hipLaunchKernelGGL(postings_count<double>, dim3(grid), dim3(256), 0, ctx->stream, B->d_indptr,
                                       B->d_indices, B->n_rows, tile_log2, p->n_tiles, p->d_seg);
                else
                    hipLaunchKernelGGL(postings_count<float>, dim3(grid), dim3(256), 0, ctx->stream, B->d_indptr,
                                       B->d_indices, B->n_rows, tile_log2, p->n_tiles, p->d_seg);
                SG_HIP_TRY(hipGetLastError());
            }
            if (st == SG_OK) st = sg_exclusive_scan_u32(ctx, p->d_seg, p->d_seg, n_bins, p->d_seg + n_bins);
            if (st == SG_OK && grid > 0) {
                if (B->dtype == SG_F64)
                    hipLaunchKernelGGL(postings_fill<double>, dim3(grid), dim3(256), 0, ctx->stream, B->d_indptr,
                                       B->d_indices, (const double *)B->d_data, B->n_rows, tile_log2, p->n_tiles,
                                       p->d_seg, cursor, p->d_rows, (double *)p->d_vals, p->d_filt, p->freq_min, inv_norm, p->fold_log2);
                else
                    hipLaunchKernelGGL(postings_fill<float>, dim3(grid), dim3(256), 0, ctx->stream, B->d_indptr,
                                       B->d_indices, (const float *)B->d_data, B->n_rows, tile_log2, p->n_tiles,
                                       p->d_seg, cursor, p->d_rows, (float *)p->d_vals, p->d_filt, p->freq_min, inv_norm, p->fold_log2);
                if (hipGetLastError() != hipSuccess) st = SG_ERR_HIP;
            }
            ctx->release(cursor);
        }
        if (st == SG_OK && !tables_done && B->n_cols > 0) {
            hipLaunchKernelGGL(term_len_kernel, dim3((unsigned)((B->n_cols + 255) / 256)), dim3(256), 0, ctx->stream,
                               (const uint32_t *)p->d_seg, B->n_cols, p->n_tiles, p->d_term_len);
            if (p->d_ends || p->d_ends8)
                hipLaunchKernelGGL(ends_from_seg_kernel, dim3((unsigned)((B->n_cols + 256) / 256)), dim3(256), 0, ctx->stream,
                                   (const uint32_t *)p->d_seg, B->n_cols, p->n_tiles, p->d_ends, p->nt_pad, p->d_ends8, p->nv_pad,
                                   p->fold_log2);
            if (hipGetLastError() != hipSuccess) st = SG_ERR_HIP;
        }
        if (st == SG_OK && p->d_fwd && !fwd_done) {
            const size_t es = B->dtype == SG_F64 ? 16 : 8;
            if (hipMemsetAsync((char *)p->d_fwd + (size_t)B->nnz * es, 0, 8 * es, ctx->stream) != hipSuccess) st = SG_ERR_HIP;
        }
        if (st == SG_OK && p->d_blk && B->n_rows > 0) {
            const int64_t work = B->n_rows * (int64_t)(p->blk_bytes / 16);
            const unsigned g3 = (unsigned)((work + 255) / 256);
            if (B->dtype == SG_F64)
                hipLaunchKernelGGL(row_blocks_kernel<double>, dim3(g3), dim3(256), 0, ctx->stream, B->d_indptr, B->d_indices,
                                   (const double *)B->d_data, B->n_rows, (const uint32_t *)p->d_orig_of, p->blk_bytes, p->d_blk);
            else
                hipLaunchKernelGGL(row_blocks_kernel<float>, dim3(g3), dim3(256), 0, ctx->stream, B->d_indptr, B->d_indices,
                                   (const float *)B->d_data, B->n_rows, (const uint32_t *)p->d_orig_of, p->blk_bytes, p->d_blk);
            if (hipGetLastError() != hipSuccess) st = SG_ERR_HIP;
        }
        if (st == SG_OK && p->d_fwd_ptr && !fwd_done) {
            const int64_t work = B->nnz > B->n_rows + 1 ? B->nnz : B->n_rows + 1;
            const unsigned g2 = (unsigned)((work + 255) / 256);
            if (B->dtype == SG_F64)
                hipLaunchKernelGGL(fwd_pack<double>, dim3(g2), dim3(256), 0, ctx->stream, B->d_indptr, B->d_indices,
                                   (const double *)B->d_data, B->n_rows, B->nnz, (const uint32_t *)p->d_orig_of, p->d_fwd_ptr, p->d_fwd);
            else
                hipLaunchKernelGGL(fwd_pack<float>, dim3(g2), dim3(256), 0, ctx->stream, B->d_indptr, B->d_indices,
                                   (const float *)B->d_data, B->n_rows, B->nnz, (const uint32_t *)p->d_orig_of, p->d_fwd_ptr, p->d_fwd);
            if (p->d_q8 && B->n_rows > 0) {
                const unsigned g4 = (unsigned)((B->n_rows * 16 + 255) / 256);
                if (B->dtype == SG_F64)
                    hipLaunchKernelGGL(q8_pack_kernel<double>, dim3(g4), dim3(256), 0, ctx->stream, B->d_indptr, B->d_indices,
                                       (const double *)B->d_data, B->n_rows, (const uint32_t *)p->d_orig_of, (uint4 *)p->d_q8, 1.0f / p->norm_up);
                else
                    hipLaunchKernelGGL(q8_pack_kernel<float>, dim3(g4), dim3(256), 0, ctx->stream, B->d_indptr, B->d_indices,
                                       (const float *)B->d_data, B->n_rows, (const uint32_t *)p->d_orig_of, (uint4 *)p->d_q8, 1.0f / p->norm_up);
            }
            if (hipGetLastError() != hipSuccess) st = SG_ERR_HIP;
        }
    }
// ... 101 lines not shown
```

string_grouper_amd/csrc/sg_spgemm_pruned.hip:

```cpp
#define SG_WATCH_NAME sg_debug_watch_pruned
#include "sg_k4_device.h"

#ifdef SG_DEBUG_WAVE_TIMES
__device__ unsigned long long sg_debug_wave_times[4 * 16384];
extern "C" int sg_debug_read_wave_times(unsigned long long *out, int clear) {
    if (hipMemcpyFromSymbol(out, HIP_SYMBOL(sg_debug_wave_times), sizeof(sg_debug_wave_times)) != hipSuccess) return 1;
    if (clear) {
        static unsigned long long zero[4 * 16384];
        if (hipMemcpyToSymbol(HIP_SYMBOL(sg_debug_wave_times), zero, sizeof(zero)) != hipSuccess) return 1;
    }
    return 0;
}
#endif

#ifndef SG_F64_STREAM_WAVES
#define SG_F64_STREAM_WAVES 4
#endif
#define SG_SCHED_FENCE() __builtin_amdgcn_sched_barrier(0)
#define SG_ROW_PARTS_LOG2 6
#define SG_ROW_PARTS 64u
#define SG_SURV_CAP 128

__device__ __forceinline__ uint64_t ballot64(bool p) { return __builtin_amdgcn_ballot_w64(p); }

// ... 1358 lines not shown
        len = (uint32_t)(indptr[i + 1] - indptr[i]);
        double s = 0.0;
        int prev = -1;
        for (int64_t p = indptr[i]; p < indptr[i + 1]; ++p) {
            const T v = data[p];
            const int k = indices[p];
            if (!(v >= (T)0)) bad = 1;
            if (k <= prev) bad = 1;
            prev = k;
            s += (double)v * (double)v;
        }
        n2 = __double2float_ru(s);
    }
    uint32_t nb = __float_as_uint(n2);
#pragma unroll
    for (int d = 32; d > 0; d >>= 1) {
        nb = max(nb, (uint32_t)__shfl_xor((int)nb, d, 64));
        len = max(len, (uint32_t)__shfl_xor((int)len, d, 64));
        bad |= (uint32_t)__shfl_xor((int)bad, d, 64);
    }
    if ((threadIdx.x & 63) == 0) {
        if (bad) atomicOr(out, 1u);
        atomicMax(out + 1, nb);
        atomicMax(out + 2, len);
    }
}

int sg_csr_props(sg_ctx *ctx, const sg_csr *m, bool *cosine_like, float *max_norm2, uint32_t *max_nnz) {
    if (m->props_state == 0 && m->from_vectoriser && max_nnz == nullptr) {
        m->props_max_norm2 = 1.000001f;
        m->props_max_nnz = 0;
        m->props_state = 1;
        m->props_by_construction = true;
    }
    if (m->props_state == 0 || (max_nnz != nullptr && m->props_by_construction && m->props_max_nnz == 0)) {
        uint32_t *d = nullptr;
        SG_TRY(sg_alloc(ctx, (size_t)4, &d));
        uint32_t h[4] = {0, 0, 0, 0};
        hipError_t e = hipMemsetAsync(d, 0, 16, ctx->stream);
        if (e == hipSuccess && m->d_props_words) {
            e = hipMemcpyAsync(d, m->d_props_words, 12, hipMemcpyDeviceToDevice, ctx->stream);
        } else if (e == hipSuccess && m->n_rows > 0) {
            const unsigned grid = (unsigned)((m->n_rows + 255) / 256);
            if (m->dtype == SG_F64)
                hipLaunchKernelGGL(csr_props_kernel<double>, dim3(grid), dim3(256), 0, ctx->stream, m->d_indptr,
                                   m->d_indices, (const double *)m->d_data, m->n_rows, d);
            else
                hipLaunchKernelGGL(csr_props_kernel<float>, dim3(grid), dim3(256), 0, ctx->stream, m->d_indptr,
                                   m->d_indices, (const float *)m->d_data, m->n_rows, d);
            e = hipGetLastError();
        }
        if (e == hipSuccess) e = hipMemcpyAsync(h, d, 16, hipMemcpyDeviceToHost, ctx->stream);
        if (e == hipSuccess) e = hipStreamSynchronize(ctx->stream);
        ctx->release(d);
        if (e != hipSuccess) {
            sg_set_error("sg_csr_props: %s", hipGetErrorString(e));
            return SG_ERR_HIP;
        }
        float n2;
        memcpy(&n2, &h[1], 4);
        if (!m->props_by_construction) m->props_max_norm2 = n2;
        m->props_max_nnz = h[2];
        m->props_state = (h[0] == 0 && n2 <= 1.0001f) ? 1 : 2;
    }
    *cosine_like = m->props_state == 1;
    *max_norm2 = m->props_max_norm2;
    if (max_nnz) *max_nnz = m->props_max_nnz;
    return SG_OK;
}

struct PairList {
    uint32_t *d_i = nullptr;
    uint32_t *d_j = nullptr;
    void *d_s = nullptr;
    uint32_t *d_row_count = nullptr;
    uint32_t *d_chunk_count = nullptr;
    uint32_t *d_chunks_used = nullptr;
    unsigned long long *d_totals = nullptr;
    uint32_t chunks = 0;
    uint32_t row_lo = 0, row_hi = 0;
    uint32_t row_step = 1;
    uint32_t rows() const { return (row_hi - row_lo + row_step - 1u) / row_step; }
    const SgPairSink *d_sink = nullptr;
};

__global__ void pair_sink_kernel(SgPairSink v, SgPairSink *out) { *out = v; }

bool sg_q8_applies(const sg_ctx *ctx, const sg_postings *Bt, double threshold) {
    if (!Bt->d_q8 || Bt->fold_log2 <= 0) return false;
    return threshold >= ctx->opt_double("SG_Q8_MIN_THRESHOLD", 0.65);
}

static size_t pruned_lds(int32_t tile_log2, int32_t fold_log2, int32_t dtype) {
    return ((size_t)2 << tile_log2) + 512 + 1024 + (size_t)SG_SURV_CAP * 4 + (fold_log2 > 0 && dtype == SG_F64 ? 512 : 0);
}
static unsigned pruned_grid(const sg_ctx *ctx, int32_t tile_log2, int64_t n_rows, int32_t fold_log2 = 0, int32_t dtype = SG_F32) {
    const size_t lds = pruned_lds(tile_log2, fold_log2, dtype);
    int waves_per_cu = (int)(ctx->lds_per_cu / lds);
    if (waves_per_cu > 32) waves_per_cu = 32;
    if (waves_per_cu < 1) waves_per_cu = 1;
    const int forced = ctx->opt_int("SG_PRUNE_WAVES_PER_CU", 0);
    if (forced > 0) waves_per_cu = forced;
    unsigned grid = (unsigned)ctx->num_cu * (unsigned)waves_per_cu;
    if ((int64_t)grid > n_rows) grid = (unsigned)(n_rows > 0 ? n_rows : 1);
    return grid;
}

template <typename T, int TILE_LOG2, bool SYM, bool WIDE, int FOLD_LOG2>
static int launch_pruned(sg_ctx *ctx, const sg_csr *A, const sg_postings *Bt, int32_t keep, sg_topn *r, T thr,
                         float s_budget, uint32_t *row_counter, uint32_t *flagged_count, uint32_t *flagged_rows,
                         unsigned long long *stats, const PairList &pl, const uint32_t *row_list, const uint32_t *row_list_len,
                         uint32_t *heavy_count = nullptr, uint32_t *heavy_rows = nullptr, uint32_t part_cfg = 0) {
    const size_t lds = pruned_lds(TILE_LOG2, FOLD_LOG2, A->dtype);
    unsigned grid = pruned_grid(ctx, TILE_LOG2, SYM ? (int64_t)pl.rows() : A->n_rows, FOLD_LOG2, A->dtype);
    if (WIDE && grid > (unsigned)ctx->num_cu * 4u && (double)A->nnz <= 48.0 * (double)A->n_rows) grid = (unsigned)ctx->num_cu * 4u;
    constexpr bool SPLITS = SYM && !WIDE && FOLD_LOG2 > 0;
    const bool share = SPLITS && (heavy_count != nullptr || part_cfg != 0u);
    auto kernel = share ? spgemm_topn_pruned_kernel<T, TILE_LOG2, SYM, WIDE, FOLD_LOG2, SPLITS>
                        : spgemm_topn_pruned_kernel<T, TILE_LOG2, SYM, WIDE, FOLD_LOG2, false>;
    hipLaunchKernelGGL(kernel, dim3(grid), dim3(64), lds, ctx->stream, A->d_indptr,
                       A->d_indices, (const T *)A->d_data, (uint32_t)A->n_rows, (const uint32_t *)Bt->d_seg,
                       (const uint32_t *)Bt->d_ends, Bt->nt_pad, (uint32_t)Bt->n_terms,
                       (const uint32_t *)Bt->d_filt, Bt->n_tiles,
                       (const SgScoreCtx *)Bt->d_score_ctx + (sg_q8_applies(ctx, Bt, (double)thr) ? 0 : 1), keep, r->stride, thr, s_budget,
                       Bt->norm_up, Bt->freq_min, r->d_cols,
                       (T *)r->d_vals,
                       r->d_counts, row_counter, flagged_count, flagged_rows, stats, pl.d_sink, pl.chunks, pl.row_lo, pl.row_hi, row_list,
                       row_list_len, (const uint32_t *)Bt->d_ends8, Bt->nv_pad, (uint32_t)(Bt->nnz * 4), (uint32_t)Bt->n_right,
                       heavy_count, heavy_rows, pl.row_step, part_cfg);
    SG_HIP_TRY(hipGetLastError());
    return SG_OK;
}

template <typename T, int TILE_LOG2, bool SYM, int FOLD_LOG2>
static int launch_both(sg_ctx *ctx, const sg_csr *A, const sg_postings *Bt, int32_t keep, sg_topn *r, T thr,
                       float s_budget, uint32_t *row_counter, uint32_t *flagged_count, uint32_t *flagged_rows,
                       unsigned long long *stats, const PairList &pl) {
    uint32_t *l1 = nullptr;
    SG_TRY(sg_alloc(ctx, (size_t)A->n_rows + 8, &l1));
    int st = hipMemsetAsync(l1, 0, 4 * sizeof(uint32_t), ctx->stream) == hipSuccess ? SG_OK : SG_ERR_HIP;
    uint32_t *heavy = nullptr;
    uint32_t heavy_rounds = 0;
    if (SYM && FOLD_LOG2 > 0 && st == SG_OK) {
        if ((pl.row_lo > 0 || (int64_t)pl.row_hi < A->n_rows || pl.row_step > 1) && 2 * (int64_t)pl.rows() < A->n_rows) {
            const double n_idx = (double)A->n_rows;
            const double rows_per_wave = (double)pl.rows() / (double)pruned_grid(ctx, TILE_LOG2, (int64_t)pl.rows(), FOLD_LOG2, A->dtype);
            const double rounds_per_row = 2.0 * 7.2e-5 * n_idx * (0.5 * ((double)pl.row_lo + (double)pl.row_hi) / n_idx);
            const double share = ctx->opt_double("SG_HEAVY_SHARE", 0.0);
            const double bar_share = share > 0.0 ? share : 0.05;
            const double bar = bar_share * rows_per_wave * rounds_per_row;
            heavy_rounds = bar < 128.0 ? 128u : (bar > 1.0e9 ? 1000000000u : (uint32_t)bar);
        }
        heavy_rounds = (uint32_t)ctx->opt_int("SG_HEAVY_ROUNDS", (int)heavy_rounds) & 0x7fffffffu;
        if (heavy_rounds > 0x0fffffffu) heavy_rounds = 0x0fffffffu;
        uint32_t handover_shift = heavy_rounds >= 512u ? 1u : (heavy_rounds >= 256u ? 2u : 3u);
        handover_shift = (uint32_t)ctx->opt_int("SG_HANDOVER_SHIFT", (int)handover_shift) & 7u;
        if (heavy_rounds) heavy_rounds |= handover_shift << 28;
        if (heavy_rounds) {
            st = sg_alloc(ctx, 2 * (size_t)A->n_rows + 8, &heavy);
            if (st == SG_OK && hipMemsetAsync(heavy, 0, 4 * sizeof(uint32_t), ctx->stream) != hipSuccess) st = SG_ERR_HIP;
        }
    }
    if (st == SG_OK)
        st = launch_pruned<T, TILE_LOG2, SYM, false, FOLD_LOG2>(ctx, A, Bt, keep, r, thr, s_budget, row_counter, l1, l1 + 4, stats, pl,
                                                     nullptr, nullptr, heavy, heavy ? heavy + 4 : nullptr, heavy ? heavy_rounds : 0u);
    if (st == SG_OK && heavy)
        st = launch_pruned<T, TILE_LOG2, SYM, false, FOLD_LOG2>(ctx, A, Bt, keep, r, thr, s_budget, heavy + 1, l1, l1 + 4, stats, pl,
                                                     heavy + 4, heavy, nullptr, nullptr, 0x80000000u);
    if (heavy) ctx->release(heavy);
    if (st == SG_OK && !ctx->opt_is("SG_PRUNE_WIDE", '0'))
        st = launch_pruned<T, TILE_LOG2, SYM, true, FOLD_LOG2>(ctx, A, Bt, keep, r, thr, s_budget, l1 + 1, flagged_count, flagged_rows, stats,
                                                    pl, l1 + 4, l1);
    else if (st == SG_OK) {
        if (hipMemcpyAsync(flagged_count, l1, 4, hipMemcpyDeviceToDevice, ctx->stream) != hipSuccess ||
            hipMemcpyAsync(flagged_rows, l1 + 4, sizeof(uint32_t) * (size_t)A->n_rows, hipMemcpyDeviceToDevice, ctx->stream) !=
                hipSuccess)
            st = SG_ERR_HIP;
    }
    ctx->release(l1);
    return st;
}

template <typename T, bool SYM>
static int dispatch_pruned(sg_ctx *ctx, const sg_csr *A, const sg_postings *Bt, int32_t keep, sg_topn *r, T thr,
                           float s_budget, uint32_t *row_counter, uint32_t *flagged_count, uint32_t *flagged_rows,
                           unsigned long long *stats, const PairList &pl) {
    if (Bt->fold_log2 > 0) {
        if (Bt->fold_log2 != 3 || Bt->tile_log2 != 12 || !Bt->d_ends8) {
            sg_set_error("postings folded 2^%d over tiles of 2^%d columns are not supported by the pruned multiply", Bt->fold_log2,
                         Bt->tile_log2);
            return SG_ERR_UNSUPPORTED;
        }
        return launch_both<T, 12, SYM, 3>(ctx, A, Bt, keep, r, thr, s_budget, row_counter, flagged_count, flagged_rows, stats, pl);
    }
    switch (Bt->tile_log2) {
        case 11: return launch_both<T, 11, SYM, 0>(ctx, A, Bt, keep, r, thr, s_budget, row_counter, flagged_count, flagged_rows, stats, pl);
        case 12: return launch_both<T, 12, SYM, 0>(ctx, A, Bt, keep, r, thr, s_budget, row_counter, flagged_count, flagged_rows, stats, pl);
        case 13: return launch_both<T, 13, SYM, 0>(ctx, A, Bt, keep, r, thr, s_budget, row_counter, flagged_count, flagged_rows, stats, pl);
        default:
            sg_set_error("postings tile of 2^%d columns is not supported by the pruned multiply (2^11..2^13)", Bt->tile_log2);
            return SG_ERR_UNSUPPORTED;
    }
}

bool sg_pruned_supports_tile(int32_t tile_log2) { return tile_log2 >= 11 && tile_log2 <= 13; }

static float prune_budget(const sg_postings *Bt, double threshold, double delta) {
    const double nb = (double)Bt->norm_up;
    const double beta = threshold - delta;
    const double budget = (beta / nb) * (beta / nb) * (1.0 - 1e-6);
    return __builtin_nextafterf((float)budget, 0.f);
}

int sg_spgemm_pruned_launch(sg_ctx *ctx, const sg_csr *A, const sg_postings *Bt, int32_t keep, sg_topn *r,
                            double threshold, double delta, uint32_t *row_counter, uint32_t *flagged_count,
                            uint32_t *flagged_rows, unsigned long long *stats) {
    const float s_budget = prune_budget(Bt, threshold, delta);
    PairList none;
    if (A->dtype == SG_F64)
        return dispatch_pruned<double, false>(ctx, A, Bt, keep, r, (double)threshold, s_budget, row_counter, flagged_count,
                                              flagged_rows, stats, none);
    return dispatch_pruned<float, false>(ctx, A, Bt, keep, r, (float)threshold, s_budget, row_counter, flagged_count,
                                         flagged_rows, stats, none);
}

__global__ void __launch_bounds__(256) all_rows_descending_kernel(uint32_t n, uint32_t first, uint32_t count, uint32_t *__restrict__ rows,
                                                                  uint32_t *len, uint32_t *listed) {
    const uint32_t i = blockIdx.x * blockDim.x + threadIdx.x;
    if (i < count) rows[i] = n - 1u - first - i;
    if (i == 0) {
        *len = count;
        *listed = first + count;
    }
}

int sg_spgemm_pruned_symmetric(sg_ctx *ctx, const sg_csr *A, const sg_postings *Bt, int32_t keep, sg_topn *r,
                               double threshold, double delta, unsigned long long *stats, bool *done, int64_t row_lo,
                               int64_t row_hi, int32_t **export_pairs, int64_t *export_n, int64_t row_step, bool exact_all) {
    *done = false;
    if (A->n_rows >= ((int64_t)1 << 30)) return SG_OK;
    if (Bt->permuted) A = Bt->permuted;
    else SG_TRY(sg_csr_ensure_rows(ctx, A));
    const size_t vs = A->dtype == SG_F64 ? 8 : 4;
    const int64_t n = A->n_rows;
    if (row_hi < 0) row_hi = n;
    PairList pl;
    pl.row_lo = (uint32_t)row_lo;
    pl.row_hi = (uint32_t)row_hi;
    pl.row_step = row_step > 1 ? (uint32_t)row_step : 1u;
    int64_t cap = (exact_all ? 512 : ((keep > SG_TOPN_LANES || Bt->tile_form) ? 256 : 64)) * n + ((int64_t)1 << 20);
    if (ctx->total_mem > 0) {
        const int64_t by_memory = (int64_t)(ctx->total_mem / 16 / (8 + vs));
        if (cap > by_memory) cap = by_memory;
    }
    if (cap < 8 * n + ((int64_t)1 << 20)) cap = 8 * n + ((int64_t)1 << 20);
    bool cap_forced = false;
    if (const char *v = ctx->opt("SG_SYM_PAIR_CAP"))
        if (atoll(v) > 0) {
            cap = atoll(v);
            cap_forced = true;
        }
    if (cap >= ((int64_t)1 << 31)) cap = ((int64_t)1 << 31) - 1;
    pl.chunks = (uint32_t)(cap / SG_PAIR_CHUNK);
    if (!cap_forced) pl.chunks += 2u * pruned_grid(ctx, Bt->tile_log2, n, Bt->fold_log2, A->dtype) + (uint32_t)ctx->num_cu * 4u +
                                  sg_spgemm_exact_selfjoin_grid(ctx, Bt);
    if (pl.chunks < 1) pl.chunks = 1;
    cap = (int64_t)pl.chunks * SG_PAIR_CHUNK;
    uint32_t *words = nullptr;
    uint32_t *cnt = nullptr, *cursor = nullptr;
    int32_t *lcol = nullptr;
    void *lval = nullptr;
    uint32_t *flagged_rows = nullptr;
    int st = sg_alloc(ctx, (size_t)128 + pl.chunks, &words);
    if (st == SG_OK) st = sg_alloc(ctx, (size_t)cap, &pl.d_i);
    if (st == SG_OK) st = sg_alloc(ctx, (size_t)cap, &pl.d_j);
    if (st == SG_OK) st = ctx->alloc((size_t)cap * vs, &pl.d_s);
    if (st == SG_OK) st = sg_alloc(ctx, (size_t)n + 2, &cnt);
    if (st == SG_OK) st = sg_alloc(ctx, (size_t)n + 2, &cursor);
    if (st == SG_OK) st = sg_alloc(ctx, (size_t)n + 2, &flagged_rows);
    unsigned long long *h = (unsigned long long *)ctx->h_stat_words;
    auto cleanup = [&]() {
        ctx->release(words);
        ctx->release(pl.d_i);
        ctx->release(pl.d_j);
        ctx->release(pl.d_s);
        ctx->release(cnt);
        ctx->release(cursor);
        ctx->release(flagged_rows);
        ctx->release(lcol);
        ctx->release(lval);
    };
    if (st != SG_OK) {
        cleanup();
        return st;
    }
    pl.d_totals = (unsigned long long *)(words + 2);
    pl.d_chunks_used = words + 4;
    pl.d_row_count = cnt;
    pl.d_chunk_count = words + 128;
    pl.d_sink = reinterpret_cast<const SgPairSink *>(words + 64);
    static_assert(sizeof(SgPairSink) <= 64, "the pair list's struct must fit the sixteen words reserved for it");
    unsigned long long *d_stats3 = nullptr;
    st = sg_alloc(ctx, (size_t)8, &d_stats3);
    hipError_t e = hipSuccess;
    if (st == SG_OK) {
        st = SG_ZERO4(ctx, words, (128 + (size_t)pl.chunks) * sizeof(uint32_t), d_stats3, 8 * sizeof(unsigned long long), cnt,
                      sizeof(uint32_t) * (size_t)(n + 2), cursor, sizeof(uint32_t) * (size_t)(n + 2));
    }
    const float s_budget = prune_budget(Bt, threshold, delta);
    SgPairSink sink;
    sink.d_i = pl.d_i;
    sink.d_j = pl.d_j;
    sink.d_s = pl.d_s;
    sink.d_row_count = pl.d_row_count;
    sink.d_chunk_count = pl.d_chunk_count;
    sink.d_chunks_used = pl.d_chunks_used;
    sink.d_totals = pl.d_totals;
    sink.chunks = pl.chunks;
    if (st == SG_OK) {
        hipLaunchKernelGGL(pair_sink_kernel, dim3(1), dim3(1), 0, ctx->stream, sink, (SgPairSink *)(words + 64));
        if (hipGetLastError() != hipSuccess) st = SG_ERR_HIP;
    }
    if (st == SG_OK && exact_all) {
        SgTimer kt(ctx, SG_K_SPGEMM_KERNEL);
        st = sg_postings_ensure_full(ctx, Bt);
        uint32_t k_first = 0;
        if (n >= (int64_t)1000000 && !cap_forced) k_first = (uint32_t)(n / 256 > 4096 ? n / 256 : 4096);
        if (const char *v = ctx->opt("SG_EXACT_SYM_PILOT_ROWS")) k_first = (uint32_t)atoll(v) < (uint32_t)n ? (uint32_t)atoll(v) : 0u;
        auto list_and_launch = [&](uint32_t first, uint32_t count, uint32_t *len_word, uint32_t *counter_word) {
            hipLaunchKernelGGL(all_rows_descending_kernel, dim3((count + 255u) / 256u), dim3(256), 0, ctx->stream, (uint32_t)n, first, count,
                               flagged_rows + first, len_word, words + 1);
            if (hipGetLastError() != hipSuccess) return (int)SG_ERR_HIP;
            return sg_spgemm_exact_selfjoin_rows(ctx, A, Bt, keep, r, threshold, counter_word, flagged_rows + first, len_word, sink,
                                                 true);
        };
        if (st == SG_OK && n > 0 && k_first > 0) {
            st = list_and_launch(0u, k_first, words + 6, words + 5);
            if (st == SG_OK) {
                e = hipMemcpyAsync(h, words, 24, hipMemcpyDeviceToHost, ctx->stream);
                if (e == hipSuccess) e = hipStreamSynchronize(ctx->stream);
                if (e != hipSuccess) st = SG_ERR_HIP;
            }
            if (st == SG_OK) {
                const double open_chunks = 0.5 * (double)sg_spgemm_exact_selfjoin_grid(ctx, Bt);
                const double used = (double)(uint32_t)h[2] > open_chunks ? (double)(uint32_t)h[2] - open_chunks : 0.0;
                if (used * (double)n / (2.0 * (double)k_first) > 0.9 * (double)pl.chunks) {
                    ctx->release(d_stats3);
                    cleanup();
                    return SG_OK;
                }
                st = list_and_launch(k_first, (uint32_t)n - k_first, words + 8, words + 7);
            }
        } else if (st == SG_OK && n > 0) {
            st = list_and_launch(0u, (uint32_t)n, words + 6, words + 5);
        }
    } else if (st == SG_OK) {
        SgTimer kt(ctx, SG_K_SPGEMM_KERNEL);
        auto pruned_pass = [&](const PairList &range) {
            if (A->dtype == SG_F64)
                return dispatch_pruned<double, true>(ctx, A, Bt, keep, r, (double)threshold, s_budget, words, words + 1, flagged_rows,
                                                     d_stats3, range);
            return dispatch_pruned<float, true>(ctx, A, Bt, keep, r, (float)threshold, s_budget, words, words + 1, flagged_rows, d_stats3,
                                                range);
        };
        uint32_t k_first = 0;
        const bool whole = pl.row_lo == 0 && (int64_t)pl.row_hi == n && pl.row_step == 1 && !export_pairs;
        if (Bt->tile_form && whole && n >= (int64_t)1000000 && !cap_forced) k_first = (uint32_t)(n / 256 > 4096 ? n / 256 : 4096);
        if (const char *v = ctx->opt("SG_SYM_PILOT_ROWS"))
            k_first = whole && atoll(v) > 0 && atoll(v) < n ? (uint32_t)atoll(v) : 0u;
        if (k_first > 0) {
            PairList first = pl, rest = pl;
            first.row_lo = (uint32_t)n - k_first;
            rest.row_hi = (uint32_t)n - k_first;
            st = pruned_pass(first);
            if (st == SG_OK) {
                e = hipMemcpyAsync(h, words, 24, hipMemcpyDeviceToHost, ctx->stream);
                if (e == hipSuccess) e = hipStreamSynchronize(ctx->stream);
                if (e != hipSuccess) st = SG_ERR_HIP;
            }
            if (st == SG_OK) {
                const double open_chunks = 0.5 * (double)pruned_grid(ctx, Bt->tile_log2, (int64_t)k_first, Bt->fold_log2, A->dtype);
                const double used = (double)(uint32_t)h[2] > open_chunks ? (double)(uint32_t)h[2] - open_chunks : 0.0;
                if (used * (double)n / (2.0 * (double)k_first) > 0.9 * (double)pl.chunks) {
                    ctx->release(d_stats3);
                    cleanup();
                    return SG_OK;
                }
                if (hipMemsetAsync(words, 0, sizeof(uint32_t), ctx->stream) != hipSuccess) st = SG_ERR_HIP;
            }
            if (st == SG_OK) st = pruned_pass(rest);
        } else {
            st = pruned_pass(pl);
        }
    }
    auto read_back = [&]() {
        e = hipMemcpyAsync(h, words, 24, hipMemcpyDeviceToHost, ctx->stream);
        if (e == hipSuccess) e = hipStreamSynchronize(ctx->stream);
        if (e != hipSuccess) {
            sg_set_error("symmetric multiply: %s", hipGetErrorString(e));
            st = SG_ERR_HIP;
        }
    };
    if (st == SG_OK) read_back();
    if (st == SG_OK && (uint32_t)(h[0] >> 32) > 0 && !exact_all) {
        st = sg_postings_ensure_full(ctx, Bt);
        const bool many = (uint32_t)(h[0] >> 32) > 2u * sg_spgemm_exact_selfjoin_grid(ctx);
        if (st == SG_OK) st = sg_spgemm_exact_selfjoin_rows(ctx, A, Bt, keep, r, threshold, words + 5, flagged_rows, words + 1, sink, many);
        if (st == SG_OK) read_back();
    }
    if (st != SG_OK) {
        ctx->release(d_stats3);
        cleanup();
        return st;
    }
    const unsigned long long n_pairs = h[1];
    const uint32_t chunks_used = (uint32_t)h[2];
    if (chunks_used > pl.chunks) {
        ctx->release(d_stats3);
        cleanup();
        return SG_OK;
    }
    const dim3 pgrid(chunks_used > 0 ? chunks_used : 1);
    if (export_pairs) {
        const int W = A->dtype == SG_F64 ? 4 : 3;
        uint32_t *chunk_start = nullptr;
        int32_t *flat = nullptr;
        st = sg_alloc(ctx, (size_t)chunks_used + 2, &chunk_start);
        if (st == SG_OK && chunks_used > 0)
            st = sg_exclusive_scan_u32(ctx, pl.d_chunk_count, chunk_start, chunks_used, nullptr);
        if (st == SG_OK) st = sg_alloc(ctx, (size_t)(n_pairs + 1) * W, &flat);
        if (st == SG_OK && chunks_used > 0) {
            if (A->dtype == SG_F64)
                hipLaunchKernelGGL(pairs_export_kernel<double>, pgrid, dim3(SG_PAIR_CHUNK), 0, ctx->stream, pl.d_i, pl.d_j,
                                   (const double *)pl.d_s, pl.d_chunk_count, chunk_start, flat,
                                   (const unsigned long long *)d_stats3, (const uint32_t *)(words + 1), stats);
            else
                hipLaunchKernelGGL(pairs_export_kernel<float>, pgrid, dim3(SG_PAIR_CHUNK), 0, ctx->stream, pl.d_i, pl.d_j,
                                   (const float *)pl.d_s, pl.d_chunk_count, chunk_start, flat,
                                   (const unsigned long long *)d_stats3, (const uint32_t *)(words + 1), stats);
            if (hipGetLastError() != hipSuccess) st = SG_ERR_HIP;
        } else if (st == SG_OK && (hipMemcpyAsync(stats, d_stats3, 3 * sizeof(unsigned long long), hipMemcpyDeviceToDevice,
                                                  ctx->stream) != hipSuccess ||
                                   hipMemcpyAsync(stats + 4, d_stats3 + 4, sizeof(unsigned long long), hipMemcpyDeviceToDevice,
                                                  ctx->stream) != hipSuccess ||
                                   hipMemcpyAsync(stats + 3, words + 1, 4, hipMemcpyDeviceToDevice, ctx->stream) != hipSuccess))
            st = SG_ERR_HIP;
        ctx->release(chunk_start);
        ctx->release(d_stats3);
        cleanup();
        if (st != SG_OK) {
            ctx->release(flat);
            return st;
        }
        *export_pairs = flat;
        *export_n = (int64_t)n_pairs;
        *done = true;
// ... 82 lines not shown
```

string_grouper_amd/csrc/sg_spgemm_topn.hip:

```cpp
#include <cstring>
#include <math.h>

#include <memory>
#include <optional>

#include "sg_internal.h"

#include "sg_k4_device.h"

typedef float f32x4 __attribute__((ext_vector_type(4)));
typedef double f64x2 __attribute__((ext_vector_type(2)));
template <typename T, typename V>
__device__ __forceinline__ bool any_above(const V &v, T thr);
template <>
__device__ __forceinline__ bool any_above<float, f32x4>(const f32x4 &v, float thr) {
    const uint32_t a = __float_as_uint(v[0]), b = __float_as_uint(v[1]), c = __float_as_uint(v[2]),
                   d = __float_as_uint(v[3]);
    const uint32_t ab = a > b ? a : b, cd = c > d ? c : d;
    return (ab > cd ? ab : cd) > __float_as_uint(thr);
}
template <>
__device__ __forceinline__ bool any_above<double, f64x2>(const f64x2 &v, double thr) {
    return __builtin_fmax(v[0], v[1]) > thr;
}
// ... 544 lines not shown
                                  double threshold, uint32_t *row_counter, const uint32_t *row_list,
                                  const uint32_t *row_list_len, const SgPairSink &sink, bool all_rows) {
    if (A->dtype == SG_F64)
        return dispatch_selfjoin_rows<double>(ctx, A, Bt, keep, r, (double)threshold, row_counter, row_list, row_list_len, sink, all_rows);
    return dispatch_selfjoin_rows<float>(ctx, A, Bt, keep, r, (float)threshold, row_counter, row_list, row_list_len, sink, all_rows);
}

struct TopnFree {
    void operator()(sg_topn *r) const { sg_topn_free(r); }
};
using TopnPtr = std::unique_ptr<sg_topn, TopnFree>;

static int topn_alloc(sg_ctx *ctx, int64_t n_rows, int64_t n_cols, int32_t stride, int32_t dtype, TopnPtr *out) {
    TopnPtr r(new (std::nothrow) sg_topn());
    if (!r) return SG_ERR_OOM;
    r->ctx = ctx;
    r->n_rows = n_rows;
    r->n_cols = n_cols;
    r->stride = stride;
    r->dtype = dtype;
    const size_t cells = (size_t)n_rows * (size_t)stride + 64;
    SG_TRY(sg_alloc(ctx, cells, &r->d_cols));
    SG_TRY(ctx->alloc(cells * (dtype == SG_F64 ? 8 : 4), &r->d_vals));
    SG_TRY(sg_alloc(ctx, (size_t)n_rows + 64, &r->d_counts));
    *out = std::move(r);
    return SG_OK;
}

static bool result_stride(int64_t n_rows, int64_t top_n, int64_t n_cols, int32_t *stride) {
    *stride = (int32_t)(top_n < n_cols ? top_n : (n_cols > 0 ? n_cols : 1));
    return (double)n_rows * (double)*stride <= 2.0e9;
}

static int result_overflow(int64_t n_rows, int32_t stride, const char *advice) {
    sg_set_error("result of %lld rows x top_n %lld does not fit the 32-bit result index%s", (long long)n_rows, (long long)stride,
                 advice);
    return SG_ERR_OVERFLOW;
}

static int sort_rows_by_column(sg_ctx *ctx, sg_topn *r) {
    if (r->n_rows <= 0) return SG_OK;
    const unsigned grid = (unsigned)(r->n_rows < 65535 * 16 ? r->n_rows : 65535 * 16);
    const size_t lds = (size_t)r->stride * (4 + (r->dtype == SG_F64 ? 8 : 4));
    if (lds > 64 * 1024) {
        sg_set_error("sort=0 with top_n=%d is not supported", r->stride);
        return SG_ERR_UNSUPPORTED;
    }
    if (r->dtype == SG_F64)
        hipLaunchKernelGGL(topn_sort_by_col_kernel<double>, dim3(grid), dim3(64), lds, ctx->stream, r->d_cols, (double *)r->d_vals,
                           r->d_counts, r->n_rows, r->stride);
    else
        hipLaunchKernelGGL(topn_sort_by_col_kernel<float>, dim3(grid), dim3(64), lds, ctx->stream, r->d_cols, (float *)r->d_vals,
                           r->d_counts, r->n_rows, r->stride);
    return SG_OK;
}

static void record_bytes(sg_ctx *ctx, const sg_csr *A, const sg_postings *Bt, double threshold) {
    const size_t s = A->dtype == SG_F64 ? 8 : 4;
    ctx->spgemm_entry_bytes = (int64_t)(4 + s);
    ctx->spgemm_fixed_bytes = A->nnz * (int64_t)(4 + s) + (A->n_rows + Bt->n_terms + 2) * 4;
    const double mean_row = Bt->n_right > 0 ? (double)Bt->nnz / (double)Bt->n_right : 0.0;
    ctx->prune_q8_bytes = sg_q8_applies(ctx, Bt, s == 8 ? threshold : (double)(float)threshold) ? 16.0 + 4.0 * mean_row : 0.0;
    ctx->prune_row_bytes = (ctx->prune_q8_bytes > 0.0 ? 0.0 : 8.0) + mean_row * (s == 8 ? 16.0 : 8.0);
}

static int prune_pilot(sg_ctx *ctx, const sg_csr *A, const sg_postings *Bt, int32_t stride, double threshold, double delta,
                       bool symmetric, bool *keep_pruned) {
    *keep_pruned = true;
    const int64_t block = 512;
    TopnPtr scratch;
    SG_TRY(topn_alloc(ctx, block, Bt->n_right, stride, A->dtype, &scratch));
    uint32_t *words = nullptr;
    unsigned long long *d_stats = nullptr;
    int st = sg_alloc(ctx, (size_t)block + 8, &words);
    if (st == SG_OK) st = sg_alloc(ctx, (size_t)8, &d_stats);
    hipError_t e = hipSuccess;
    if (st == SG_OK) e = hipMemsetAsync(d_stats, 0, 8 * sizeof(unsigned long long), ctx->stream);
    const int64_t starts[3] = {0, (A->n_rows - block) / 2, A->n_rows - block};
    for (int b = 0; b < 3 && st == SG_OK && e == hipSuccess; ++b) {
        sg_csr view = *A;
        view.n_rows = block;
        view.d_indptr = A->d_indptr + starts[b];
        view.owned = false;
        e = hipMemsetAsync(words, 0, 8 * sizeof(uint32_t), ctx->stream);
        if (e == hipSuccess) e = hipMemsetAsync(scratch->d_counts, 0, sizeof(int32_t) * (size_t)block, ctx->stream);
        if (e == hipSuccess)
            st = sg_spgemm_pruned_launch(ctx, &view, Bt, stride < SG_TOPN_LANES ? stride : SG_TOPN_LANES, scratch.get(), threshold,
                                         delta, words, words + 1, words + 8, d_stats);
    }
    if (st == SG_OK && e == hipSuccess) {
        hipLaunchKernelGGL(count_macs_kernel, dim3(512), dim3(256), 0, ctx->stream, A->d_indptr, A->d_indices, A->n_rows,
                           (const uint32_t *)Bt->d_term_len, d_stats + 3);
        e = hipGetLastError();
    }
    unsigned long long h[4] = {0, 0, 0, 0};
    if (st == SG_OK && e == hipSuccess) e = hipMemcpyAsync(h, d_stats, sizeof(h), hipMemcpyDeviceToHost, ctx->stream);
    if (st == SG_OK && e == hipSuccess) e = hipStreamSynchronize(ctx->stream);
    ctx->release(words);
    ctx->release(d_stats);
    if (st != SG_OK) return st;
    if (e != hipSuccess) {
        sg_set_error("pruning pilot: %s", hipGetErrorString(e));
        return SG_ERR_HIP;
    }
    const double s = A->dtype == SG_F64 ? 8.0 : 4.0;
    const double rows = (double)A->n_rows, sampled = h[0] > 0 ? (double)h[0] : 1.0;
    const double candidates = (double)h[2] * rows / sampled;
    const double row_len = Bt->n_right > 0 ? (double)Bt->nnz / (double)Bt->n_right : 0.0;
    double ms_pruned = rows * (double)Bt->n_tiles * 2.0e-7 + candidates * 2.9e-9 * row_len;
    if (symmetric) ms_pruned = 0.55 * ms_pruned + 0.3;
    const double ms_exact = (double)h[3] * (4.0 + s) * 0.6 / 3.7e9 + rows * (double)Bt->n_tiles * 8.0e-7;
    *keep_pruned = ms_pruned <= ms_exact;
    ctx->pilot_ms_pruned = ms_pruned;
    ctx->pilot_ms_exact = ms_exact;
    return SG_OK;
}

static bool built_from(const sg_csr *A, const sg_postings *Bt) {
    if (Bt->collapse) {
        const sg_csr *cb = &Bt->caller_b_copy;
        return A->n_rows == Bt->collapse->n_orig && A->d_indptr == cb->d_indptr && A->d_indices == cb->d_indices &&
               A->d_data == cb->d_data;
    }
    return A->n_rows == Bt->n_right && A->d_indptr == Bt->b_indptr && A->d_indices == Bt->b_indices && A->d_data == Bt->b_data;
}

static const sg_postings *owner(const sg_postings *Bt) { return Bt->view_of ? Bt->view_of : Bt; }

enum class SgCompanion { plain, alt_tile, exact_native };
static std::mutex g_companion_mu;

static int companion(sg_ctx *ctx, const sg_postings *home, SgCompanion kind, const sg_csr *from, const sg_postings **out) {
    sg_postings **slot = kind == SgCompanion::plain      ? &home->plain
                         : kind == SgCompanion::alt_tile ? &home->alt_tile
                                                         : &home->exact_native;
    std::lock_guard<std::mutex> lock(g_companion_mu);
    if (!*slot) {
        if (kind == SgCompanion::plain) {
            SG_TRY(sg_postings_build_flags(ctx, from, home->build_tile_cols, (home->build_flags & 0xff) | SG_POSTINGS_NO_COLLAPSE, slot));
        } else {
            SG_TRY(sg_csr_ensure_rows(ctx, from));
            SG_TRY(sg_postings_build_flags(ctx, from, 0,
                                           (home->build_flags & SG_POSTINGS_NO_PERMUTATION) | SG_POSTINGS_NO_COLLAPSE |
                                               (kind == SgCompanion::alt_tile ? SG_POSTINGS_TILE_FORM : SG_POSTINGS_EXACT_ONLY),
                                           slot));
        }
    }
    *out = *slot;
    return SG_OK;
}

static const sg_csr *companion_source(const sg_csr *A, const sg_postings *Bt) {
    if (built_from(A, Bt)) return A;
    const sg_postings *home = owner(Bt);
    return home->collapse ? home->collapse->unique : (Bt->built_from_valid ? &Bt->built_from : nullptr);
}

struct SgPlan {
    enum Form { EXACT, EXACT_SELFJOIN, PRUNED, PRUNED_SELFJOIN };
    Form form = EXACT;
    const sg_postings *index = nullptr;
    int32_t stride = 0;
    double threshold = 0.0;
    double delta = 0.0;
};

// ... 710 lines not shown
```

string_grouper_amd/csrc/sg_vectorize.hip:

```cpp
#include <type_traits>

#include "sg_internal.h"

#define TOK_CAP 1024
#define SG_KEY_OOV32 0xFFFFFFFEu
#define SG_KEY_OOV64 0xFFFFFFFFFFFFFFFEull
#define SG_CHAR_ABSENT 0xFFFFu
#define TOK_CHARS (TOK_CAP + 16)

template <typename KeyT>
struct KeyTraits;
template <>
struct KeyTraits<uint32_t> {
    static constexpr uint32_t OOV = SG_KEY_OOV32;
    static constexpr uint32_t PAD = 0xFFFFFFFFu;
};
template <>
struct KeyTraits<uint64_t> {
    static constexpr uint64_t OOV = SG_KEY_OOV64;
    static constexpr uint64_t PAD = 0xFFFFFFFFFFFFFFFFull;
};

struct TokenCache {
    const sg_strings *src = nullptr;
// ... 582 lines not shown
    for (int q = 0; q < c; ++q) dst[d + q] = keys[b + q];
}

template <typename T>
__device__ __forceinline__ T tmul(T a, T b);
template <>
__device__ __forceinline__ float tmul<float>(float a, float b) { return __fmul_rn(a, b); }
template <>
__device__ __forceinline__ double tmul<double>(double a, double b) { return __dmul_rn(a, b); }

template <typename T, typename KeyT, typename Lookup>
__global__ void __launch_bounds__(256) weight_normalize_kernel(const int64_t *__restrict__ ub_ptr,
                                                               const int32_t *__restrict__ cnt,
                                                               const KeyT *__restrict__ keys,
                                                               const int32_t *__restrict__ tf, Lookup lookup,
                                                               const T *__restrict__ idf, int64_t n,
                                                               const int64_t *__restrict__ indptr,
                                                               int32_t *__restrict__ out_idx, T *__restrict__ out_val,
                                                               uint32_t *props ) {
    const int64_t i = (int64_t)blockIdx.x * blockDim.x + threadIdx.x;
    float n2 = 0.f;
    uint32_t len = 0;
    if (i < n) {
        const int64_t b = ub_ptr[i] - ub_ptr[0];
        const int c = cnt[i];
        int64_t o = indptr[i];
        const int64_t o0 = o;
        double acc = 0.0;
        for (int q = 0; q < c; ++q) {
            const int32_t col = lookup(keys[b + q]);
            if (col < 0) continue;
            const T w = tmul<T>((T)tf[b + q], idf[col]);
            out_idx[o] = col;
            out_val[o] = w;
            acc = __dadd_rn(acc, (double)tmul<T>(w, w));
            ++o;
        }
        len = (uint32_t)(o - o0);
        if (acc != 0.0) {
            const double nrm = __dsqrt_rn(acc);
            double s2 = 0.0;
            for (int64_t q = o0; q < o; ++q) {
                const T v = (T)__ddiv_rn((double)out_val[q], nrm);
                out_val[q] = v;
                s2 += (double)v * (double)v;
            }
            n2 = __double2float_ru(s2);
        }
    }
    uint32_t nb = __float_as_uint(n2);
#pragma unroll
    for (int d = 32; d > 0; d >>= 1) {
        nb = max(nb, (uint32_t)__shfl_xor((int)nb, d, 64));
        len = max(len, (uint32_t)__shfl_xor((int)len, d, 64));
    }
    if ((threadIdx.x & 63) == 0 && props) {
        const volatile uint32_t *seen = props;
        if (nb > seen[1]) atomicMax(props + 1, nb);
        if (len > seen[2]) atomicMax(props + 2, len);
    }
}

__device__ __forceinline__ double dpp_from_lower_lane(double v, double lane0_gets) {
    const uint64_t b = (uint64_t)__double_as_longlong(v), o = (uint64_t)__double_as_longlong(lane0_gets);
    const uint32_t lo = (uint32_t)__builtin_amdgcn_update_dpp((int)(uint32_t)o, (int)(uint32_t)b, 0x111 , 0xF, 0xF, false);
    const uint32_t hi =
        (uint32_t)__builtin_amdgcn_update_dpp((int)(uint32_t)(o >> 32), (int)(uint32_t)(b >> 32), 0x111, 0xF, 0xF, false);
    return __longlong_as_double((long long)(((uint64_t)hi << 32) | lo));
}
__device__ __forceinline__ double shfl_double(double v, int src_lane) {
    const uint64_t b = (uint64_t)__double_as_longlong(v);
    const uint32_t lo = (uint32_t)__shfl((int)(uint32_t)b, src_lane, 64), hi = (uint32_t)__shfl((int)(uint32_t)(b >> 32), src_lane, 64);
    return __longlong_as_double((long long)(((uint64_t)hi << 32) | lo));
}

template <typename T, typename KeyT, typename Lookup>
__global__ void __launch_bounds__(256) weight_normalize_rows16_kernel(const int64_t *__restrict__ ub_ptr,
                                                                      const int32_t *__restrict__ cnt,
                                                                      const KeyT *__restrict__ keys,
                                                                      const int32_t *__restrict__ tf, Lookup lookup,
                                                                      const T *__restrict__ idf, int64_t n,
                                                                      const int64_t *__restrict__ indptr,
                                                                      int32_t *__restrict__ out_idx, T *__restrict__ out_val,
                                                                      uint32_t *props) {
    const int lane = threadIdx.x & 63, sub = lane & 15, grp_shift = lane & 48;
    const int64_t row = ((int64_t)blockIdx.x * blockDim.x + threadIdx.x) >> 4;
    const bool valid = row < n;
    const int64_t b = valid ? ub_ptr[row] - ub_ptr[0] : 0;
    const int c = valid ? cnt[row] : 0;
    const int64_t o0 = valid ? indptr[row] : 0;
    int cmax = c;
    cmax = max(cmax, __shfl_xor(cmax, 16, 64));
    cmax = max(cmax, __shfl_xor(cmax, 32, 64));
    double carry = 0.0;
    int32_t col_keep[2] = {-1, -1};
    T w_keep[2] = {(T)0, (T)0};
    for (int base = 0; base < cmax; base += 16) {
        const int q = base + sub;
        double w2 = 0.0;
        if (q < c) {
            const int32_t col = lookup(keys[b + q]);
            if (col >= 0) {
                const T w = tmul<T>((T)tf[b + q], idf[col]);
                w2 = (double)tmul<T>(w, w);
                if (base == 0) {
                    col_keep[0] = col;
                    w_keep[0] = w;
                } else if (base == 16) {
                    col_keep[1] = col;
                    w_keep[1] = w;
                }
            }
        }
        double acc = w2;
#pragma unroll
        for (int k = 0; k < 16; ++k) acc = __dadd_rn(dpp_from_lower_lane(acc, carry), w2);
        carry = shfl_double(acc, lane | 15);
    }
    float n2 = 0.f;
    uint32_t len = 0;
    if (carry != 0.0) {
        const double nrm = __dsqrt_rn(carry);
        double s2 = 0.0;
        int kept_before = 0;
        for (int base = 0; base < cmax; base += 16) {
            const int q = base + sub;
            int32_t col = -1;
            T w = 0;
            if (base < 32) {
                col = base == 0 ? col_keep[0] : col_keep[1];
                w = base == 0 ? w_keep[0] : w_keep[1];
            } else if (q < c) {
                col = lookup(keys[b + q]);
                if (col >= 0) w = tmul<T>((T)tf[b + q], idf[col]);
            }
            const uint32_t km = (uint32_t)(__ballot(col >= 0) >> grp_shift) & 0xFFFFu;
            if (col >= 0) {
                const int64_t o = o0 + kept_before + __popc(km & ((1u << sub) - 1u));
                const T v = (T)__ddiv_rn((double)w, nrm);
                out_idx[o] = col;
                out_val[o] = v;
                s2 += (double)v * (double)v;
            }
            kept_before += __popc(km);
        }
        len = (uint32_t)kept_before;
#pragma unroll
        for (int d = 8; d > 0; d >>= 1) s2 += shfl_double(s2, lane ^ d);
        n2 = __double2float_ru(s2 * (1.0 + 1e-12));
    }
    uint32_t nb = __float_as_uint(n2);
#pragma unroll
    for (int d = 32; d > 0; d >>= 1) {
        nb = max(nb, (uint32_t)__shfl_xor((int)nb, d, 64));
        len = max(len, (uint32_t)__shfl_xor((int)len, d, 64));
    }
    if (lane == 0 && props) {
        const volatile uint32_t *seen = props;
        if (nb > seen[1]) atomicMax(props + 1, nb);
        if (len > seen[2]) atomicMax(props + 2, len);
    }
}

static void free_cache(sg_ctx *ctx, TokenCache &c) {
    ctx->release(c.d_longs);
    c.d_longs = nullptr;
    ctx->release(c.d_cnt);
    ctx->release(c.d_keys);
    ctx->release(c.d_tf);
    ctx->release(c.d_indptr);
    c = TokenCache();
}

static TokParams make_tok_params(const sg_vocab *v, const VocabImpl *im, const sg_strings *s) {
    TokParams tp;
    memset(&tp, 0, sizeof(tp));
    tp.ngram = v->params.ngram_size;
    tp.lower = (v->params.ascii_lower && !(s && s->prelowered)) ? 1 : 0;
    tp.bits = v->bits_per_char;
    for (int c = 0; c < 128; ++c)
        if (v->params.delete_table[c]) tp.del_mask[c >> 5] |= 1u << (c & 31);
    memcpy(tp.rank_of_byte, im->rank_of_byte, sizeof(tp.rank_of_byte));
    return tp;
}

template <typename KeyT, bool SYMBOLS>
static int tokenize_longs_t(sg_ctx *ctx, const sg_strings *s, const TokParams &tp, int32_t *df_table, int32_t df_replicas,
                            int64_t df_stride, TokenCache &c, uint32_t n_long) {
    if (n_long == 0) return SG_OK;
    uint32_t *longs = c.d_longs;
    KeyT *keys = (KeyT *)c.d_keys;
    int64_t *d_sizes = nullptr, *d_coff = nullptr, *d_koff = nullptr;
    std::vector<int64_t> sizes(n_long), coff(n_long + 1, 0), koff(n_long + 1, 0);
    int st = sg_alloc(ctx, (size_t)n_long, &d_sizes);
    if (st == SG_OK) st = sg_alloc(ctx, (size_t)n_long + 1, &d_coff);
    if (st == SG_OK) st = sg_alloc(ctx, (size_t)n_long + 1, &d_koff);
    hipError_t e = hipSuccess;
    if (st == SG_OK) {
        hipLaunchKernelGGL(long_sizes_kernel, dim3((n_long + 255) / 256), dim3(256), 0, ctx->stream, s->d_offsets,
                           (const uint32_t *)(longs + 1), n_long, d_sizes);
        e = hipMemcpyAsync(sizes.data(), d_sizes, sizeof(int64_t) * n_long, hipMemcpyDeviceToHost, ctx->stream);
        if (e == hipSuccess) e = hipStreamSynchronize(ctx->stream);
    }
    uint16_t *lchars = nullptr;
    KeyT *lkeys = nullptr;
    if (st == SG_OK && e == hipSuccess) {
        for (uint32_t i = 0; i < n_long; ++i) {
            int64_t p2 = 64;
            while (p2 < sizes[i]) p2 <<= 1;
            coff[i + 1] = coff[i] + sizes[i] + 8;
            koff[i + 1] = koff[i] + p2;
        }
        st = sg_alloc(ctx, (size_t)coff[n_long] + 8, &lchars);
        if (st == SG_OK) st = sg_alloc(ctx, (size_t)koff[n_long] + 8, &lkeys);
        if (st == SG_OK) {
            e = hipMemcpyAsync(d_coff, coff.data(), sizeof(int64_t) * (n_long + 1), hipMemcpyHostToDevice, ctx->stream);
            if (e == hipSuccess)
                e = hipMemcpyAsync(d_koff, koff.data(), sizeof(int64_t) * (n_long + 1), hipMemcpyHostToDevice, ctx->stream);
            if (e == hipSuccess) {
                hipLaunchKernelGGL((tokenize_long_kernel<KeyT, SYMBOLS>), dim3(n_long), dim3(256), 0, ctx->stream,
                                   (const void *)s->d_bytes, s->d_offsets, tp, (const uint32_t *)(longs + 1),
                                   (const int64_t *)d_coff, (const int64_t *)d_koff, lchars, lkeys,
                                   (const int64_t *)c.d_ub_ptr, c.d_cnt, keys, c.d_tf, df_table, df_replicas, df_stride);
                e = hipGetLastError();
            }
            if (e == hipSuccess) e = hipStreamSynchronize(ctx->stream);
        }
    }
    ctx->release(d_sizes);
    ctx->release(d_coff);
    ctx->release(d_koff);
    ctx->release(lchars);
    ctx->release(lkeys);
// ... 248 lines not shown
            if (st == SG_OK && (hipMemcpyAsync(&t, d + c.n, sizeof(int64_t), hipMemcpyDeviceToHost, ctx->stream) != hipSuccess ||
                                hipStreamSynchronize(ctx->stream) != hipSuccess))
                st = SG_ERR_HIP;
        }
        if (st != SG_OK) break;
        totals.push_back(t);
        total += t;
    }
    uint64_t *all = nullptr;
    if (st == SG_OK) st = sg_alloc(ctx, (size_t)total + 1, &all);
    if (st == SG_OK) st = sg_alloc(ctx, (size_t)total + 1, &v->d_keys);
    if (st == SG_OK) st = sg_alloc(ctx, (size_t)total + 1, &v->d_df);
    int64_t at = 0;
    for (size_t i = 0; i < im->caches.size() && st == SG_OK; ++i) {
        const TokenCache &c = im->caches[i];
        if (c.n > 0 && totals[i] > 0) {
            hipLaunchKernelGGL(gather_keys_kernel, dim3((unsigned)((c.n + 255) / 256)), dim3(256), 0, ctx->stream,
                               (const int64_t *)c.d_ub_ptr, (const int32_t *)c.d_cnt, (const uint64_t *)c.d_keys,
                               (const int64_t *)dst_ptrs[i], c.n, all + at);
            if (hipGetLastError() != hipSuccess) st = SG_ERR_HIP;
        }
        at += totals[i];
    }
    int64_t n_unique = 0;
    if (st == SG_OK) st = sg_sort_unique_u64(ctx, all, total, v->d_keys, v->d_df, &n_unique);
    for (int64_t *d : dst_ptrs) ctx->release(d);
    ctx->release(all);
    if (st != SG_OK) return st;
    if (n_unique > 0) {
        uint64_t last = 0;
        if (hipMemcpyAsync(&last, v->d_keys + (n_unique - 1), 8, hipMemcpyDeviceToHost, ctx->stream) != hipSuccess ||
            hipStreamSynchronize(ctx->stream) != hipSuccess)
            return SG_ERR_HIP;
        if (last == SG_KEY_OOV64) --n_unique;
    }
    v->n_terms = n_unique;
    return SG_OK;
}

static int count_df_by_column(sg_ctx *ctx, sg_vocab *v) {
    VocabImpl *im = v->impl;
    const int32_t max_cols = 30 * 1024;
    static bool attr_done = false;
    if (!attr_done) {
        (void)hipFuncSetAttribute((const void *)df_count_lds_kernel, hipFuncAttributeMaxDynamicSharedMemorySize, max_cols * 4);
        attr_done = true;
    }
    std::vector<int32_t> wgs;
    int32_t n_partial = 0;
    for (const auto &c : im->caches) {
        int64_t g = (c.n + 1023) / 1024;
        if (g > (int64_t)ctx->num_cu) g = (int64_t)ctx->num_cu;
        wgs.push_back((int32_t)g);
        n_partial += (int32_t)g;
    }
    uint32_t *partial = nullptr;
    int st = sg_alloc(ctx, (size_t)((int64_t)(n_partial > 0 ? n_partial : 1) * v->n_terms), &partial);
    if (st != SG_OK) return st;
    int32_t at = 0;
    const bool one_pass = v->n_terms <= max_cols && !(ctx->opt("SG_K2_COLUMNS") && ctx->opt("SG_K2_COLUMNS")[0] == '0');
    for (size_t i = 0; i < im->caches.size(); ++i) {
        TokenCache &c = im->caches[i];
        if (wgs[i] == 0) continue;
        for (int64_t col0 = 0; col0 < v->n_terms; col0 += max_cols) {
            const int32_t n_cols = (int32_t)(v->n_terms - col0 < max_cols ? v->n_terms - col0 : max_cols);
            hipLaunchKernelGGL(df_count_lds_kernel, dim3((unsigned)wgs[i]), dim3(1024), (size_t)n_cols * 4, ctx->stream,
                               (const int64_t *)c.d_ub_ptr, (const int32_t *)c.d_cnt, (uint32_t *)c.d_keys,
                               (const int32_t *)v->d_key_to_col, c.n, (int32_t)col0, n_cols, v->n_terms,
                               partial + (int64_t)at * v->n_terms, one_pass ? 1 : 0);
        }
        if (one_pass) c.keys_are_columns = true;
        at += wgs[i];
    }
    hipLaunchKernelGGL(df_sum_kernel, dim3((unsigned)((v->n_terms + 63) / 64)), dim3(256), 0, ctx->stream, (const uint32_t *)partial,
                       n_partial, v->n_terms, v->d_df);
    if (hipGetLastError() != hipSuccess) {
        sg_set_error("df_count_lds_kernel: %s", hipGetErrorString(hipGetLastError()));
        st = SG_ERR_HIP;
    }
    ctx->release(partial);
    return st;
}

extern "C" int sg_vec_fit_end(sg_ctx *ctx, sg_vocab *v, int64_t n_docs_total) {
    SG_REQUIRE(ctx && v && v->impl, "null argument");
    SG_REQUIRE(v->n_terms == 0, "the vocabulary is already finished");
    VocabImpl *im = v->impl;
    if (n_docs_total > 0) v->n_docs = n_docs_total;
    int st = SG_OK;
    {
        SgTimer timer(ctx, SG_K_VOCAB);
        if (v->sorted_mode) {
            st = finish_sorted_vocabulary(ctx, v);
        } else {
            uint32_t *d_total = nullptr;
            st = sg_alloc(ctx, 4, &d_total);
            if (st == SG_OK) {
                const unsigned grid = (unsigned)((v->key_space + 255) / 256);
                (void)grid;
                st = sg_exclusive_scan_positive_i32(ctx, im->d_df_table, (uint32_t *)v->d_key_to_col, v->key_space, d_total);
            }
            uint32_t n_terms = 0;
            for (int attempt = 0; attempt < 2 && st == SG_OK; ++attempt) {
                std::vector<uint32_t> n_long(im->caches.size(), 0u);
                std::vector<int64_t> nnz_of(im->caches.size(), -1);
                for (size_t q = 0; q < im->caches.size() && st == SG_OK; ++q) {
                    TokenCache &c = im->caches[q];
                    if (c.n <= 0) continue;
                    if (!c.d_indptr) st = sg_alloc(ctx, (size_t)c.n + 1, &c.d_indptr);
                    if (st == SG_OK) st = sg_exclusive_scan_i32_to_i64(ctx, c.d_cnt, c.d_indptr, c.n);
                }
                if (st != SG_OK) break;
                uint32_t *hf = ctx->h_fetch;
                const bool pinned = 4 * im->caches.size() + 4 <= SG_H_FETCH_WORDS;
                hipError_t e = hipMemcpyAsync(pinned ? (void *)hf : (void *)&n_terms, d_total, 4, hipMemcpyDeviceToHost, ctx->stream);
                for (size_t q = 0; q < im->caches.size() && e == hipSuccess; ++q) {
                    if (im->caches[q].d_longs)
                        e = hipMemcpyAsync(pinned ? (void *)(hf + 2 + 4 * q) : (void *)&n_long[q], im->caches[q].d_longs, 4, hipMemcpyDeviceToHost, ctx->stream);
                    if (e == hipSuccess && im->caches[q].d_indptr)
                        e = hipMemcpyAsync(pinned ? (void *)(hf + 4 + 4 * q) : (void *)&nnz_of[q], im->caches[q].d_indptr + im->caches[q].n, 8,
                                           hipMemcpyDeviceToHost, ctx->stream);
                }
                if (e == hipSuccess) e = hipStreamSynchronize(ctx->stream);
                if (pinned && e == hipSuccess) {
                    n_terms = hf[0];
                    for (size_t q = 0; q < im->caches.size(); ++q) {
                        if (im->caches[q].d_longs) n_long[q] = hf[2 + 4 * q];
                        if (im->caches[q].d_indptr) memcpy(&nnz_of[q], hf + 4 + 4 * q, 8);
                    }
                }
                for (size_t q = 0; q < im->caches.size(); ++q) im->caches[q].nnz = nnz_of[q];
                if (e != hipSuccess) {
                    sg_set_error("reading the vocabulary size failed: %s", hipGetErrorString(e));
                    st = SG_ERR_HIP;
                    break;
                }
                bool any_long = false;
                for (size_t q = 0; q < im->caches.size() && st == SG_OK; ++q) {
                    if (!im->caches[q].d_longs) continue;
                    any_long = any_long || n_long[q] > 0;
                    st = resolve_longs(ctx, v, im->caches[q], im->d_df_table, 0, im->df_stride, n_long[q]);
                }
                if (!any_long || st != SG_OK) break;
                const unsigned grid = (unsigned)((v->key_space + 255) / 256);
                (void)grid;
                st = sg_exclusive_scan_positive_i32(ctx, im->d_df_table, (uint32_t *)v->d_key_to_col, v->key_space, d_total);
            }
            ctx->release(d_total);
            if (st == SG_OK) {
                v->n_terms = n_terms;
                if (v->n_terms > 0) {
                    st = sg_alloc(ctx, (size_t)v->n_terms + 1, &v->d_keys);
                    if (st == SG_OK) st = sg_alloc(ctx, (size_t)v->n_terms + 1, &v->d_df);
                    if (st == SG_OK) {
                        const unsigned grid = (unsigned)((v->key_space + 255) / 256);
                        hipLaunchKernelGGL(vocab_finalize_kernel, dim3(grid), dim3(256), 0, ctx->stream, im->d_df_table,
                                           v->key_space, v->d_key_to_col, v->d_keys, v->d_df);
                        if (hipGetLastError() != hipSuccess) st = SG_ERR_HIP;
                    }
                    if (st == SG_OK && im->df_marks) st = count_df_by_column(ctx, v);
                }
            }
        }
        if (st == SG_OK && v->n_terms == 0) {
            sg_set_error("empty vocabulary; perhaps the documents only contain stop words");
            st = SG_ERR_BADARG;
        }
    }
    return st;
}

extern "C" int sg_vec_fit(sg_ctx *ctx, const sg_strings *const *sets, int32_t n_sets, const sg_vec_params *params,
                          sg_vocab **out) {
    SG_REQUIRE(out != nullptr, "null argument");
    sg_vocab *v = nullptr;
    SG_TRY(fit_begin(ctx, sets, n_sets, params, true, &v));
    const int st = sg_vec_fit_end(ctx, v, 0);
    if (st != SG_OK) {
        sg_vocab_free(v);
        return st;
    }
    *out = v;
    return SG_OK;
}

extern "C" int sg_vocab_size(const sg_vocab *v, int64_t *n_terms, int64_t *n_docs) {
    SG_REQUIRE(v != nullptr, "vocab is null");
    if (n_terms) *n_terms = v->n_terms;
    if (n_docs) *n_docs = v->n_docs;
    return SG_OK;
}

extern "C" int sg_vocab_coding(const sg_vocab *v, int32_t *bits_per_char, int32_t *symbols, int32_t *sorted_mode) {
    SG_REQUIRE(v && v->impl, "vocab is null");
    if (bits_per_char) *bits_per_char = v->bits_per_char;
    if (symbols) *symbols = v->impl->symbols ? 1 : 0;
    if (sorted_mode) *sorted_mode = v->sorted_mode ? 1 : 0;
    return SG_OK;
}

extern "C" int sg_vocab_to_host(sg_ctx *ctx, const sg_vocab *v, uint64_t *keys, int64_t *df) {
    SG_REQUIRE(ctx && v && keys && df, "null argument");
    const VocabImpl *im = impl_of(v);
    SG_REQUIRE(im != nullptr, "unknown vocab");
    std::vector<int32_t> hdf((size_t)v->n_terms);
    SG_HIP_TRY(hipMemcpyAsync(keys, v->d_keys, sizeof(uint64_t) * (size_t)v->n_terms, hipMemcpyDeviceToHost, ctx->stream));
    SG_HIP_TRY(hipMemcpyAsync(hdf.data(), v->d_df, sizeof(int32_t) * (size_t)v->n_terms, hipMemcpyDeviceToHost, ctx->stream));
    SG_HIP_TRY(hipStreamSynchronize(ctx->stream));
    for (int64_t i = 0; i < v->n_terms; ++i) df[i] = hdf[(size_t)i];
    return SG_OK;
}

extern "C" int sg_vocab_byte_alphabet(const sg_vocab *v, uint8_t *byte_of_code, int32_t *n_codes) {
    SG_REQUIRE(v && v->impl && byte_of_code && n_codes, "null argument");
    SG_REQUIRE(!v->impl->symbols, "the vocabulary was fitted on symbol columns: the caller holds their alphabet");
    *n_codes = 1 << v->bits_per_char;
    if (*n_codes > 128) *n_codes = 128;
    memcpy(byte_of_code, v->impl->byte_of_rank, (size_t)*n_codes);
    return SG_OK;
}

static bool weights_positive_and_finite(const void *w, int64_t n, int32_t dtype) {
    if (dtype == SG_F64) {
        const double *p = (const double *)w;
        for (int64_t i = 0; i < n; ++i)
            if (!(p[i] > 0.0) || !(p[i] <= 1.79e308)) return false;
    } else {
        const float *p = (const float *)w;
        for (int64_t i = 0; i < n; ++i)
            if (!(p[i] > 0.f) || !(p[i] <= 3.4e38f)) return false;
    }
// ... 19 lines not shown
    int64_t d = df[k];
    if (d < 0) d = 0;
    if (d > n_docs) d = n_docs;
    idf[k] = table[d];
}

extern "C" int sg_ctx_put_idf_table(sg_ctx *ctx, int64_t n_docs, int32_t dtype, const void *table) {
    SG_REQUIRE(ctx && table && n_docs >= 0, "null argument");
    SG_REQUIRE(dtype == SG_F32 || dtype == SG_F64, "dtype must be SG_F32 or SG_F64");
    const size_t bytes = ((size_t)n_docs + 1) * (dtype == SG_F64 ? 8 : 4);
    void *d = nullptr;
    SG_HIP_TRY(hipMalloc(&d, bytes));
    if (hipMemcpyAsync(d, table, bytes, hipMemcpyHostToDevice, ctx->stream) != hipSuccess ||
        hipStreamSynchronize(ctx->stream) != hipSuccess) {
        (void)hipFree(d);
        sg_set_error("upload of the idf table failed");
        return SG_ERR_HIP;
    }
    const bool trusted = weights_positive_and_finite((const char *)table + (dtype == SG_F64 ? 8 : 4), n_docs, dtype);
    for (auto &t : ctx->idf_tables)
        if (t.n_docs == n_docs && t.dtype == dtype) {
            (void)hipFree(t.d);
            t.d = d;
            t.trusted = trusted;
            return SG_OK;
        }
    if (ctx->idf_tables.size() >= 4) {
        (void)hipFree(ctx->idf_tables.front().d);
        ctx->idf_tables.erase(ctx->idf_tables.begin());
    }
    ctx->idf_tables.push_back({n_docs, dtype, d, trusted});
    return SG_OK;
}

extern "C" int sg_vocab_apply_idf_table(sg_ctx *ctx, sg_vocab *v, int32_t *applied) {
    SG_REQUIRE(ctx && v && applied, "null argument");
    *applied = 0;
    SG_REQUIRE(v->d_df != nullptr || v->n_terms == 0, "the vocabulary has no document counts (fit first)");
    const void *table = nullptr;
    bool trusted = false;
    for (const auto &t : ctx->idf_tables)
        if (t.n_docs == v->n_docs && t.dtype == v->params.dtype) {
            table = t.d;
            trusted = t.trusted;
        }
    if (!table) return SG_OK;
    v->idf_trusted = trusted;
    const size_t s = v->params.dtype == SG_F64 ? 8 : 4;
    if (!v->d_idf) SG_TRY(ctx->alloc(((size_t)v->n_terms + 1) * s, &v->d_idf));
    if (v->n_terms > 0) {
        const unsigned grid = (unsigned)((v->n_terms + 255) / 256);
        if (v->params.dtype == SG_F64)
            hipLaunchKernelGGL(idf_from_table_kernel<double>, dim3(grid), dim3(256), 0, ctx->stream, (const int32_t *)v->d_df, v->n_terms,
                               (const double *)table, v->n_docs, (double *)v->d_idf);
        else
            hipLaunchKernelGGL(idf_from_table_kernel<float>, dim3(grid), dim3(256), 0, ctx->stream, (const int32_t *)v->d_df, v->n_terms,
                               (const float *)table, v->n_docs, (float *)v->d_idf);
        SG_HIP_TRY(hipGetLastError());
    }
    *applied = 1;
    return SG_OK;
}

extern "C" int sg_vocab_free(sg_vocab *v) {
    if (!v) return SG_OK;
    VocabImpl *im = v->impl;
    v->impl = nullptr;
    sg_ctx *ctx = v->ctx;
    if (im) {
        for (auto &c : im->caches) free_cache(ctx, c);
        ctx->release(im->d_df_table);
        delete im;
    }
    ctx->release(v->d_key_to_col);
    ctx->release(v->d_keys);
    ctx->release(v->d_df);
    ctx->release(v->d_idf);
    delete v;
    return SG_OK;
}

template <typename T, typename KeyT, typename Lookup>
static void launch_weight(sg_ctx *ctx, const TokenCache *tc, Lookup lookup, const sg_vocab *v, int64_t n, const int64_t *indptr,
                          int32_t *idx, void *val, uint32_t *props) {
    const char *pe = ctx->opt("SG_K2_PLAIN");
    const bool plain = pe && pe[0] == '1';
    if (plain)
        hipLaunchKernelGGL((weight_normalize_kernel<T, KeyT, Lookup>), dim3((unsigned)((n + 255) / 256)), dim3(256), 0, ctx->stream,
                           (const int64_t *)tc->d_ub_ptr, (const int32_t *)tc->d_cnt, (const KeyT *)tc->d_keys,
                           (const int32_t *)tc->d_tf, lookup, (const T *)v->d_idf, n, indptr, idx, (T *)val, props);
    else
        hipLaunchKernelGGL((weight_normalize_rows16_kernel<T, KeyT, Lookup>), dim3((unsigned)((n + 15) / 16)), dim3(256), 0,
                           ctx->stream, (const int64_t *)tc->d_ub_ptr, (const int32_t *)tc->d_cnt, (const KeyT *)tc->d_keys,
                           (const int32_t *)tc->d_tf, lookup, (const T *)v->d_idf, n, indptr, idx, (T *)val, props);
}

extern "C" int sg_vec_transform(sg_ctx *ctx, const sg_vocab *v, const sg_strings *strings, sg_csr **out) {
    SG_REQUIRE(ctx && v && strings && out, "null argument");
    SG_REQUIRE(v->d_idf != nullptr, "sg_vocab_set_idf has not been called");
    VocabImpl *im = impl_of(v);
    SG_REQUIRE(im != nullptr, "unknown vocab");
    SG_REQUIRE((strings->sym_width == 2) == im->symbols && (!im->symbols || strings->alphabet == im->alphabet),
               "the strings are not of the kind (bytes / symbols of this alphabet) the vocabulary was fitted on");
    TokenCache local;
    const TokenCache *tc = nullptr;
    for (const auto &c : im->caches)
        if (c.src == strings && c.n == strings->n) tc = &c;
    int st = SG_OK;
    if (!tc) {
        SgTimer timer(ctx, SG_K_TOKENIZE);
        st = tokenize_set(ctx, v, strings, nullptr, 1, 0, &local);
        if (st != SG_OK) return st;
        tc = &local;
    }
    const int64_t n = strings->n;
    sg_csr *m = new (std::nothrow) sg_csr();
    if (!m) return SG_ERR_OOM;
    m->ctx = ctx;
    m->n_rows = n;
    m->n_cols = v->n_terms;
    m->dtype = v->params.dtype;
    m->owned = true;
    int32_t *kept = nullptr;
    int64_t *indptr = nullptr;
    int64_t nnz = 0;
    const DenseLookup dense{v->d_key_to_col};
    const SortedLookup sorted{v->d_keys, v->n_terms};
    {
        SgTimer timer(ctx, SG_K_WEIGHT);
        const bool all_kept = tc != &local;
        TokenCache *fitted = all_kept ? const_cast<TokenCache *>(tc) : nullptr;
        const bool have_ptr = fitted && fitted->d_indptr && fitted->nnz >= 0 && n > 0;
        if (have_ptr) {
            indptr = fitted->d_indptr;
            nnz = fitted->nnz;
            fitted->d_indptr = nullptr;
            fitted->nnz = -1;
        }
        if (!all_kept) st = sg_alloc(ctx, (size_t)n + 1, &kept);
        if (st == SG_OK && !have_ptr) st = sg_alloc(ctx, (size_t)n + 1, &indptr);
        if (have_ptr) {
            ;
        } else if (st == SG_OK && n > 0) {
            const unsigned grid = (unsigned)((n + 255) / 256);
            if (all_kept)
                ;
            else if (v->sorted_mode)
                hipLaunchKernelGGL((kept_count_kernel<uint64_t, SortedLookup>), dim3(grid), dim3(256), 0, ctx->stream,
                                   (const int64_t *)tc->d_ub_ptr, (const int32_t *)tc->d_cnt, (const uint64_t *)tc->d_keys,
                                   sorted, n, kept);
            else
                hipLaunchKernelGGL((kept_count_kernel<uint32_t, DenseLookup>), dim3(grid), dim3(256), 0, ctx->stream,
                                   (const int64_t *)tc->d_ub_ptr, (const int32_t *)tc->d_cnt, (const uint32_t *)tc->d_keys,
                                   dense, n, kept);
            st = sg_exclusive_scan_i32_to_i64(ctx, all_kept ? tc->d_cnt : kept, indptr, n);
        } else if (st == SG_OK) {
            (void)hipMemsetAsync(indptr, 0, sizeof(int64_t), ctx->stream);
        }
        if (st == SG_OK && !have_ptr) {
            if (hipMemcpyAsync(&nnz, indptr + n, sizeof(int64_t), hipMemcpyDeviceToHost, ctx->stream) != hipSuccess ||
                hipStreamSynchronize(ctx->stream) != hipSuccess)
                st = SG_ERR_HIP;
        }
        int32_t *idx = nullptr;
        void *val = nullptr;
        const size_t s = m->dtype == SG_F64 ? 8 : 4;
        if (st == SG_OK) st = sg_alloc(ctx, (size_t)nnz + 4, &idx);
        if (st == SG_OK) st = ctx->alloc(((size_t)nnz + 4) * s, &val);
        m->d_indptr = indptr;
        m->d_indices = idx;
        m->d_data = val;
        m->nnz = nnz;
        m->from_vectoriser = v->idf_trusted;
        if (st == SG_OK && ctx->opt("SG_ROW_BLOCKS") && ctx->opt("SG_ROW_BLOCKS")[0] == '1') {
            st = sg_alloc(ctx, (size_t)4, &m->d_props_words);
            if (st == SG_OK && hipMemsetAsync(m->d_props_words, 0, 16, ctx->stream) != hipSuccess) st = SG_ERR_HIP;
        }
        if (st == SG_OK && n > 0) {
            uint32_t *props = m->d_props_words;
            if (v->sorted_mode) {
                if (m->dtype == SG_F64) launch_weight<double, uint64_t>(ctx, tc, sorted, v, n, indptr, idx, val, props);
                else launch_weight<float, uint64_t>(ctx, tc, sorted, v, n, indptr, idx, val, props);
            } else if (tc->keys_are_columns) {
                const ColumnsLookup cols{};
                if (m->dtype == SG_F64) launch_weight<double, uint32_t>(ctx, tc, cols, v, n, indptr, idx, val, props);
                else launch_weight<float, uint32_t>(ctx, tc, cols, v, n, indptr, idx, val, props);
            } else {
                if (m->dtype == SG_F64) launch_weight<double, uint32_t>(ctx, tc, dense, v, n, indptr, idx, val, props);
                else launch_weight<float, uint32_t>(ctx, tc, dense, v, n, indptr, idx, val, props);
            }
            if (hipGetLastError() != hipSuccess) st = SG_ERR_HIP;
        }
    }
    ctx->release(kept);
    if (tc == &local) free_cache(ctx, local);
    if (st != SG_OK) {
        sg_csr_free(m);
        return st;
    }
    *out = m;
    return SG_OK;
}
```

Baseline: 104.8 million.

## Fuse row hashing into weighting, add one-pass postings fill, pack fit readbacks

The tf-idf weighting kernel now also computes a per-row content hash, so the collapse grouping kernel can read it instead of re-reading and re-hashing every row. Rows only load their entries when a hash collision requires a full comparison. The postings fill gains a one-pass variant that seeds local counters from precomputed offsets. Vocabulary fit-end gathers its scattered small device words with one tiny kernel and one copy, and the zero-ranges kernel can also write a few words. These cut memory traffic and small transfers, at the cost of an extra hash buffer and more kernel variants.

Result: no change. 105.0 million, median of 2 (+0.1%).

```diff
diff --git a/string_grouper_amd/csrc/sg_api.hip b/string_grouper_amd/csrc/sg_api.hip
--- a/string_grouper_amd/csrc/sg_api.hip
+++ b/string_grouper_amd/csrc/sg_api.hip
@@ -451,6 +451,7 @@
     v->left_state = 0;
     v->n_rows = r1 - r0;
     v->d_indptr = m->d_indptr + r0;
+    if (m->d_row_hash) v->d_row_hash = m->d_row_hash + r0;
     int64_t ends[2] = {0, 0};
     SG_HIP_TRY(hipMemcpyAsync(&ends[0], m->d_indptr + r0, sizeof(int64_t), hipMemcpyDeviceToHost, ctx->stream));
     SG_HIP_TRY(hipMemcpyAsync(&ends[1], m->d_indptr + r1, sizeof(int64_t), hipMemcpyDeviceToHost, ctx->stream));
@@ -468,6 +469,7 @@
         m->ctx->release((void *)m->d_indices);
         m->ctx->release((void *)m->d_data);
         m->ctx->release(m->d_props_words);
+        m->ctx->release(m->d_row_hash);
     }
     delete m;
     return SG_OK;
@@ -478,8 +480,12 @@
     uint64_t words[8];
     uint64_t first[8];
     int n;
+    int put_words;
+    uint32_t *put_dst;
+    uint32_t put[16];
 };
 __global__ void __launch_bounds__(256) zero_ranges_kernel(SgZeroJobs jobs) {
+    if (blockIdx.x == 0 && (int)threadIdx.x < jobs.put_words) jobs.put_dst[threadIdx.x] = jobs.put[threadIdx.x];
     const uint64_t total = jobs.first[jobs.n < 8 ? jobs.n : 7] + (jobs.n == 8 ? jobs.words[7] : 0);
     for (uint64_t q = ((uint64_t)blockIdx.x * blockDim.x + threadIdx.x) * 4; q < total; q += (uint64_t)gridDim.x * blockDim.x * 4) {
         int r = 0;
@@ -497,8 +503,15 @@
     }
 }
 
-int sg_zero_ranges(sg_ctx *ctx, int n, void *const *ptrs, const size_t *bytes) {
+int sg_zero_ranges(sg_ctx *ctx, int n, void *const *ptrs, const size_t *bytes) { return sg_zero_ranges_put(ctx, n, ptrs, bytes, nullptr, nullptr, 0); }
+
+int sg_zero_ranges_put(sg_ctx *ctx, int n, void *const *ptrs, const size_t *bytes, void *put_dst, const void *put, size_t put_bytes) {
     SgZeroJobs jobs;
+    SG_REQUIRE(put_bytes <= sizeof(jobs.put) && (put_bytes & 3u) == 0 && ((uintptr_t)put_dst & 3u) == 0, "words to put: at most sixteen");
+    jobs.put_words = put_dst ? (int)(put_bytes / 4) : 0;
+    jobs.put_dst = (uint32_t *)put_dst;
+    memset(jobs.put, 0, sizeof(jobs.put));
+    if (jobs.put_words > 0) memcpy(jobs.put, put, put_bytes);
     jobs.n = 0;
     uint64_t first = 0;
     for (int i = 0; i < n; ++i) {
@@ -513,7 +526,7 @@
         first += (jobs.words[jobs.n] + 3) & ~(uint64_t)3;
         ++jobs.n;
     }
-    if (jobs.n == 0) return SG_OK;
+    if (jobs.n == 0 && jobs.put_words == 0) return SG_OK;
     for (int i = jobs.n; i < 8; ++i) {
         jobs.ptr[i] = nullptr;
         jobs.words[i] = 0;
diff --git a/string_grouper_amd/csrc/sg_collapse.hip b/string_grouper_amd/csrc/sg_collapse.hip
--- a/string_grouper_amd/csrc/sg_collapse.hip
+++ b/string_grouper_amd/csrc/sg_collapse.hip
@@ -10,18 +10,8 @@
     uint64_t h = 0;
     if (r < n_rows) {
         const int64_t lo = indptr[r], hi = indptr[r + 1];
-        for (int64_t p = lo + sub; p < hi; p += 16) {
-            uint64_t v;
-            if (sizeof(T) == 4) v = (uint64_t)__float_as_uint((float)data[p]);
-            else v = (uint64_t)__double_as_longlong((double)data[p]);
-            uint64_t x = ((uint64_t)(uint32_t)indices[p] << 32) ^ v ^ ((uint64_t)(p - lo) * 0x9E3779B97F4A7C15ull);
-            x ^= x >> 33;
-            x *= 0xff51afd7ed558ccdull;
-            x ^= x >> 33;
-            x *= 0xc4ceb9fe1a85ec53ull;
-            x ^= x >> 33;
-            h += x;
-        }
+        for (int64_t p = lo + sub; p < hi; p += 16)
+            h += sg_row_hash_entry(indices[p], sg_row_hash_bits(data[p]), (uint64_t)(p - lo));
     }
 #pragma unroll
     for (int d = 8; d > 0; d >>= 1) {
@@ -30,7 +20,7 @@
     }
     if (r < n_rows && sub == 0) {
         const int64_t len = indptr[r + 1] - indptr[r];
-        hash[r] = h ^ ((uint64_t)len * 0xD6E8FEB86659FD93ull);
+        hash[r] = sg_row_hash_finish(h, (uint64_t)len);
         if (row_id) row_id[r] = (uint32_t)r;
     }
 }
@@ -40,22 +30,24 @@
 #define SG_GROUP_NO_SLOT 0xFFFFFFFFu
 
 #define SG_GROUP_ROWS 2
-template <typename T>
+template <typename T, bool HASHED>
 __global__ void __launch_bounds__(256) group_rows_kernel(const int64_t *__restrict__ indptr, const int32_t *__restrict__ indices,
                                                          const T *__restrict__ data, int64_t n_rows, unsigned long long *table,
-                                                         uint32_t mask, uint32_t *__restrict__ slot_of_row) {
+                                                         uint32_t mask, uint32_t *__restrict__ slot_of_row,
+                                                         const uint64_t *__restrict__ row_hash ) {
     const int64_t grp = ((int64_t)blockIdx.x * blockDim.x + threadIdx.x) >> 4;
     const int sub = threadIdx.x & 15;
     const int lead = (int)(threadIdx.x & 48u);
     int64_t r[SG_GROUP_ROWS], lo[SG_GROUP_ROWS];
     int32_t len[SG_GROUP_ROWS];
-    bool valid[SG_GROUP_ROWS];
+    bool valid[SG_GROUP_ROWS], own[SG_GROUP_ROWS];
 #pragma unroll
     for (int i = 0; i < SG_GROUP_ROWS; ++i) {
         r[i] = grp * SG_GROUP_ROWS + i;
         valid[i] = r[i] < n_rows;
-        lo[i] = valid[i] ? indptr[r[i]] : 0;
-        len[i] = valid[i] ? (int32_t)(indptr[r[i] + 1] - lo[i]) : 0;
+        own[i] = !HASHED;
+        lo[i] = valid[i] && !HASHED ? indptr[r[i]] : 0;
+        len[i] = valid[i] && !HASHED ? (int32_t)(indptr[r[i] + 1] - lo[i]) : 0;
     }
     int32_t k0[SG_GROUP_ROWS], k1[SG_GROUP_ROWS];
     T v0[SG_GROUP_ROWS], v1[SG_GROUP_ROWS];
@@ -78,26 +70,21 @@
 #pragma unroll
     for (int i = 0; i < SG_GROUP_ROWS; ++i) {
         uint64_t h = 0;
-        for (int32_t e = sub; e < len[i]; e += 16) {
-            const int32_t k = e < 16 ? k0[i] : (e < 32 ? k1[i] : indices[lo[i] + e]);
-            const T v = e < 16 ? v0[i] : (e < 32 ? v1[i] : data[lo[i] + e]);
-            uint64_t vb;
-            if (sizeof(T) == 4) vb = (uint64_t)__float_as_uint((float)v);
-            else vb = (uint64_t)__double_as_longlong((double)v);
-            uint64_t x = ((uint64_t)(uint32_t)k << 32) ^ vb ^ ((uint64_t)e * 0x9E3779B97F4A7C15ull);
-            x ^= x >> 33;
-            x *= 0xff51afd7ed558ccdull;
-            x ^= x >> 33;
-            x *= 0xc4ceb9fe1a85ec53ull;
-            x ^= x >> 33;
-            h += x;
-        }
-#pragma unroll
-        for (int d = 8; d > 0; d >>= 1) {
-            const uint32_t lo32 = (uint32_t)__shfl_xor((int)(uint32_t)h, d, 64), hi32 = (uint32_t)__shfl_xor((int)(uint32_t)(h >> 32), d, 64);
-            h += ((uint64_t)hi32 << 32) | lo32;
-        }
-        h ^= (uint64_t)(uint32_t)len[i] * 0xD6E8FEB86659FD93ull;
+        if (HASHED) {
+            h = valid[i] ? row_hash[r[i]] : 0;
+        } else {
+            for (int32_t e = sub; e < len[i]; e += 16) {
+                const int32_t k = e < 16 ? k0[i] : (e < 32 ? k1[i] : indices[lo[i] + e]);
+                const T v = e < 16 ? v0[i] : (e < 32 ? v1[i] : data[lo[i] + e]);
+                h += sg_row_hash_entry(k, sg_row_hash_bits(v), (uint64_t)e);
+            }
+#pragma unroll
+            for (int d = 8; d > 0; d >>= 1) {
+                const uint32_t lo32 = (uint32_t)__shfl_xor((int)(uint32_t)h, d, 64), hi32 = (uint32_t)__shfl_xor((int)(uint32_t)(h >> 32), d, 64);
+                h += ((uint64_t)hi32 << 32) | lo32;
+            }
+            h = sg_row_hash_finish(h, (uint64_t)(uint32_t)len[i]);
+        }
         h ^= h >> 31;
         mine[i] = ((unsigned long long)(uint32_t)(h >> 32) << 32) | (unsigned long long)(~(uint32_t)r[i]);
         s[i] = (uint32_t)h & mask;
@@ -126,6 +113,29 @@
             o[i] = (int64_t)(~c_lo[i]);
             olo[i] = cmp[i] ? indptr[o[i]] : 0;
             olen[i] = cmp[i] ? (int32_t)(indptr[o[i] + 1] - olo[i]) : -1;
+        }
+        if (HASHED) {
+            bool fetch[SG_GROUP_ROWS];
+#pragma unroll
+            for (int i = 0; i < SG_GROUP_ROWS; ++i) {
+                fetch[i] = cmp[i] && !own[i];
+                if (fetch[i]) {
+                    lo[i] = indptr[r[i]];
+                    len[i] = (int32_t)(indptr[r[i] + 1] - lo[i]);
+                    own[i] = true;
+                }
+            }
+#pragma unroll
+            for (int i = 0; i < SG_GROUP_ROWS; ++i) {
+                if (fetch[i] && sub < len[i]) {
+                    k0[i] = indices[lo[i] + sub];
+                    v0[i] = data[lo[i] + sub];
+                }
+                if (fetch[i] && sub + 16 < len[i]) {
+                    k1[i] = indices[lo[i] + sub + 16];
+                    v1[i] = data[lo[i] + sub + 16];
+                }
+            }
         }
         int32_t ok0[SG_GROUP_ROWS], ok1[SG_GROUP_ROWS];
         T ov0[SG_GROUP_ROWS], ov1[SG_GROUP_ROWS];
@@ -527,12 +537,15 @@
         st = SG_ZERO4(ctx, table, sizeof(unsigned long long) * (size_t)table_size, size, sizeof(uint32_t) * (size_t)(n + 2), cursor,
                       sizeof(uint32_t) * (size_t)(n + 2), totals, (64 + 32 * 32) * sizeof(uint32_t));
     if (st == SG_OK) {
-        if (B->dtype == SG_F64)
-            hipLaunchKernelGGL(group_rows_kernel<double>, dim3(g16), dim3(256), 0, ctx->stream, B->d_indptr, B->d_indices,
-                               (const double *)B->d_data, n, table, (uint32_t)(table_size - 1), slot_of_row);
-        else
-            hipLaunchKernelGGL(group_rows_kernel<float>, dim3(g16), dim3(256), 0, ctx->stream, B->d_indptr, B->d_indices,
-                               (const float *)B->d_data, n, table, (uint32_t)(table_size - 1), slot_of_row);
+        const uint64_t *rh = B->d_row_hash;
+        auto group = [&](auto kernel, auto *data) {
+            hipLaunchKernelGGL(kernel, dim3(g16), dim3(256), 0, ctx->stream, B->d_indptr, B->d_indices, data, n, table,
+                               (uint32_t)(table_size - 1), slot_of_row, rh);
+        };
+        if (B->dtype == SG_F64 && rh) group(group_rows_kernel<double, true>, (const double *)B->d_data);
+        else if (B->dtype == SG_F64) group(group_rows_kernel<double, false>, (const double *)B->d_data);
+        else if (rh) group(group_rows_kernel<float, true>, (const float *)B->d_data);
+        else group(group_rows_kernel<float, false>, (const float *)B->d_data);
         st = sg_scan_launch<uint32_t>(ctx, GroupRepLoad{table, slot_of_row, rep_of_row}, SgScanStoreArray<uint32_t>{rep_excl}, n, totals);
     }
     if (st == SG_OK) {
diff --git a/string_grouper_amd/csrc/sg_internal.h b/string_grouper_amd/csrc/sg_internal.h
--- a/string_grouper_amd/csrc/sg_internal.h
+++ b/string_grouper_amd/csrc/sg_internal.h
@@ -150,10 +150,24 @@
     bool from_vectoriser = false;
     mutable bool props_by_construction = false;
     uint32_t *d_props_words = nullptr;
+    uint64_t *d_row_hash = nullptr;
     mutable int left_state = 0;
     mutable struct SgCollapse *left_groups = nullptr;
     struct SgCollapse *rows_of = nullptr;
 };
+
+__device__ __forceinline__ uint64_t sg_row_hash_entry(int32_t col, uint64_t value_bits, uint64_t place) {
+    uint64_t x = ((uint64_t)(uint32_t)col << 32) ^ value_bits ^ (place * 0x9E3779B97F4A7C15ull);
+    x ^= x >> 33;
+    x *= 0xff51afd7ed558ccdull;
+    x ^= x >> 33;
+    x *= 0xc4ceb9fe1a85ec53ull;
+    x ^= x >> 33;
+    return x;
+}
+__device__ __forceinline__ uint64_t sg_row_hash_bits(float v) { return (uint64_t)__float_as_uint(v); }
+__device__ __forceinline__ uint64_t sg_row_hash_bits(double v) { return (uint64_t)__double_as_longlong(v); }
+__device__ __forceinline__ uint64_t sg_row_hash_finish(uint64_t entry_sum, uint64_t len) { return entry_sum ^ (len * 0xD6E8FEB86659FD93ull); }
 
 struct SgScoreCtx {
     const uint32_t *fwd_ptr = nullptr;
@@ -306,6 +320,7 @@
 int sg_sort_unique_u64(sg_ctx *ctx, uint64_t *d_keys, int64_t n, uint64_t *d_unique, int32_t *d_counts, int64_t *n_unique);
 
 int sg_zero_ranges(sg_ctx *ctx, int n, void *const *ptrs, const size_t *bytes);
+int sg_zero_ranges_put(sg_ctx *ctx, int n, void *const *ptrs, const size_t *bytes, void *put_dst, const void *put, size_t put_bytes);
 #define SG_ZERO2(ctx, p0, b0, p1, b1) [&]() { void *const pp_[] = {(void *)(p0), (void *)(p1)}; const size_t bb_[] = {(size_t)(b0), (size_t)(b1)}; return sg_zero_ranges(ctx, 2, pp_, bb_); }()
 #define SG_ZERO3(ctx, p0, b0, p1, b1, p2, b2) [&]() { void *const pp_[] = {(void *)(p0), (void *)(p1), (void *)(p2)}; const size_t bb_[] = {(size_t)(b0), (size_t)(b1), (size_t)(b2)}; return sg_zero_ranges(ctx, 3, pp_, bb_); }()
 #define SG_ZERO4(ctx, p0, b0, p1, b1, p2, b2, p3, b3) [&]() { void *const pp_[] = {(void *)(p0), (void *)(p1), (void *)(p2), (void *)(p3)}; const size_t bb_[] = {(size_t)(b0), (size_t)(b1), (size_t)(b2), (size_t)(b3)}; return sg_zero_ranges(ctx, 4, pp_, bb_); }()
diff --git a/string_grouper_amd/csrc/sg_postings.hip b/string_grouper_amd/csrc/sg_postings.hip
--- a/string_grouper_amd/csrc/sg_postings.hip
+++ b/string_grouper_amd/csrc/sg_postings.hip
@@ -311,11 +311,12 @@
 }
 
 __device__ __forceinline__ uint32_t lds_get16(const uint32_t *w, uint32_t k) { return (w[k >> 1] >> ((k & 1u) << 4)) & 0xffffu; }
-template <typename T>
+template <typename T, bool ONE>
 __global__ void __launch_bounds__(1024) postings_fill_staged(const int64_t *__restrict__ indptr, const int32_t *__restrict__ indices,
                                                              const T *__restrict__ data, int64_t n_rows, int32_t tile_log2,
                                                              int32_t n_terms, int32_t split, int32_t chunk_rows, uint32_t stage_cap,
                                                              uint32_t *cnt , const uint32_t *__restrict__ term_start,
+                                                             const uint32_t *__restrict__ term_len ,
                                                              const uint8_t *__restrict__ is_frequent, uint32_t *__restrict__ out_filt,
                                                              float inv_norm_up, int32_t fold_log2) {
     extern __shared__ uint32_t lds[];
@@ -328,6 +329,9 @@
     const int64_t t = blockIdx.x / split;
     const int32_t part = blockIdx.x % split;
     uint32_t *mine = cnt + (int64_t)blockIdx.x * n_terms;
+    const uint32_t *upto = blockIdx.x + 1u < gridDim.x ? mine + n_terms : term_len;
+    const uint32_t cur_split = (w16 + 3u) & ~3u;
+    auto cur = [&](uint32_t k) -> uint32_t * { return k < cur_split ? lcnt + k : stage + (k - cur_split); };
     for (uint32_t k = threadIdx.x; k < (((uint32_t)n_terms + 31u) >> 5); k += blockDim.x) freq_bits[k] = 0;
     __syncthreads();
     for (int k = threadIdx.x; k < n_terms; k += blockDim.x)
@@ -350,6 +354,10 @@
         const int64_t c1 = c0 + chunk_rows < j1 ? c0 + chunk_rows : j1;
         const int64_t trips = (c1 - c0 + groups * SG_POST_ROWS - 1) / (groups * SG_POST_ROWS);
         if (any_big) {
+            if (ONE) {
+                for (uint32_t k = threadIdx.x; k < (uint32_t)n_terms; k += blockDim.x) *cur(k) = 0u;
+                __syncthreads();
+            }
             for (int64_t it = 0; it < trips; ++it) {
                 const int64_t jb = c0 + (it * groups + (threadIdx.x >> 4)) * SG_POST_ROWS;
 #pragma unroll
@@ -371,7 +379,7 @@
                     const uint32_t col = (uint32_t)(jb + r - (t << tile_log2));
                     for (int64_t p = lo + sub; p < hi; p += 16) {
                         const int32_t k = indices[p];
-                        const uint32_t pos = term_start[k] + atomicAdd(&mine[k], 1u);
+                        const uint32_t pos = term_start[k] + (ONE ? mine[k] + atomicAdd(cur((uint32_t)k), 1u) : atomicAdd(&mine[k], 1u));
                         out_filt[pos] = filter_posting(col, (float)data[p], fq, tile_log2, inv_norm_up, (uint32_t)t, fold_log2);
                     }
                 }
@@ -379,9 +387,18 @@
             __syncthreads();
             continue;
         }
-        for (uint32_t w = threadIdx.x; w < w16; w += blockDim.x) lcnt[w] = 0;
+        if (ONE) {
+            for (uint32_t w = threadIdx.x; w < w16; w += blockDim.x) {
+                const uint32_t k = 2u * w;
+                const uint32_t even = upto[k] - mine[k];
+                const uint32_t odd = k + 1u < (uint32_t)n_terms ? upto[k + 1u] - mine[k + 1u] : 0u;
+                lcnt[w] = even | (odd << 16);
+            }
+        } else {
+            for (uint32_t w = threadIdx.x; w < w16; w += blockDim.x) lcnt[w] = 0;
+        }
         __syncthreads();
-        for (int64_t it = 0; it < trips; ++it) {
+        for (int64_t it = 0; !ONE && it < trips; ++it) {
             const int64_t jb = c0 + (it * groups + (threadIdx.x >> 4)) * SG_POST_ROWS;
             int64_t lo[SG_POST_ROWS], hi[SG_POST_ROWS];
 #pragma unroll
@@ -456,7 +473,24 @@
             }
 #pragma unroll
             for (int r = 0; r < SG_POST_ROWS; ++r) {
-                const float fq = jb + r < c1 ? fqrow[jb + r - c0] : 0.f;
+                float fq;
+                if (ONE) {
+                    double f2 = 0.0;
+                    if (k0[r] >= 0 && ((freq_bits[k0[r] >> 5] >> (k0[r] & 31)) & 1u)) f2 = (double)v0[r] * (double)v0[r];
+                    for (int64_t p = lo[r] + sub + 16; p < hi[r]; p += 16) {
+                        const int32_t k = indices[p];
+                        if ((freq_bits[k >> 5] >> (k & 31)) & 1u) f2 += (double)data[p] * (double)data[p];
+                    }
+#pragma unroll
+                    for (int d = 8; d > 0; d >>= 1) {
+                        const uint64_t bits = (uint64_t)__double_as_longlong(f2);
+                        const uint32_t l = (uint32_t)__shfl_xor((int)(uint32_t)bits, d, 64), h = (uint32_t)__shfl_xor((int)(uint32_t)(bits >> 32), d, 64);
+                        f2 += __longlong_as_double((long long)(((uint64_t)h << 32) | l));
+                    }
+                    fq = frequent_norm_ratio_of(f2, inv_norm_up);
+                } else {
+                    fq = jb + r < c1 ? fqrow[jb + r - c0] : 0.f;
+                }
                 const uint32_t col = (uint32_t)(jb + r - (t << tile_log2));
                 if (k0[r] >= 0) {
                     const uint32_t sh = ((uint32_t)k0[r] & 1u) << 4;
@@ -519,7 +553,7 @@
                         const uint32_t G_t = (uint32_t)__shfl((int)G[b], (int)tsel, 64);
                         if (e < Eg) out_filt[G_t + (e - start_t)] = stage[e];
                     }
-                    if (mine_has[b]) mine[k] = before[b] + (end_k[b] - start_k[b]);
+                    if (!ONE && mine_has[b]) mine[k] = before[b] + (end_k[b] - start_k[b]);
                 }
             }
         }
@@ -921,6 +955,7 @@
             inner->caller_b_copy = *B_in;
             inner->caller_b_copy.owned = false;
             inner->caller_b_copy.d_props_words = nullptr;
+            inner->caller_b_copy.d_row_hash = nullptr;
             inner->caller_b_copy.left_groups = nullptr;
             inner->caller_b_copy.left_state = 0;
             inner->caller_b = &inner->caller_b_copy;
@@ -1056,6 +1091,7 @@
     p->built_from = *B_in;
     p->built_from.owned = false;
     p->built_from.d_props_words = nullptr;
+    p->built_from.d_row_hash = nullptr;
     p->built_from.left_groups = nullptr;
     p->built_from.left_state = 0;
     p->built_from_valid = true;
@@ -1077,6 +1113,7 @@
     p->src = *B;
     p->src.owned = false;
     p->src.d_props_words = nullptr;
+    p->src.d_row_hash = nullptr;
     p->src.left_groups = nullptr;
     p->src.left_state = 0;
     if (st == SG_OK && !lazy_full && B->dtype == SG_F64) st = sg_alloc(ctx, (size_t)B->nnz + 64, &p->d_rows);
@@ -1148,12 +1185,14 @@
                 (void)hipFuncSetAttribute((const void *)postings_count_lds, hipFuncAttributeMaxDynamicSharedMemorySize, 124 * 1024);
                 (void)hipFuncSetAttribute((const void *)postings_fill_lds<float>, hipFuncAttributeMaxDynamicSharedMemorySize, 124 * 1024);
                 (void)hipFuncSetAttribute((const void *)postings_fill_lds<double>, hipFuncAttributeMaxDynamicSharedMemorySize, 124 * 1024);
-                (void)hipFuncSetAttribute((const void *)postings_fill_staged<float>, hipFuncAttributeMaxDynamicSharedMemorySize, 160 * 1024);
-                (void)hipFuncSetAttribute((const void *)postings_fill_staged<double>, hipFuncAttributeMaxDynamicSharedMemorySize, 160 * 1024);
+                (void)hipFuncSetAttribute((const void *)postings_fill_staged<float, false>, hipFuncAttributeMaxDynamicSharedMemorySize, 160 * 1024);
+                (void)hipFuncSetAttribute((const void *)postings_fill_staged<double, false>, hipFuncAttributeMaxDynamicSharedMemorySize, 160 * 1024);
+                (void)hipFuncSetAttribute((const void *)postings_fill_staged<float, true>, hipFuncAttributeMaxDynamicSharedMemorySize, 160 * 1024);
+                (void)hipFuncSetAttribute((const void *)postings_fill_staged<double, true>, hipFuncAttributeMaxDynamicSharedMemorySize, 160 * 1024);
                 attr_done = true;
             }
             bool staged = p->d_filt != nullptr && p->d_vals == nullptr && !(ctx->opt("SG_FILL_STAGED") && ctx->opt("SG_FILL_STAGED")[0] == '0');
-            uint32_t stage_cap = 0;
+            uint32_t stage_cap = 0, stage_words = 0;
             int32_t chunk_rows = 0;
             size_t staged_lds = 0;
             const double mean_nnz = B->n_rows > 0 ? (double)B->nnz / (double)B->n_rows : 1.0;
@@ -1169,7 +1208,10 @@
                     chunk_rows >>= 1;
                 }
                 staged = (double)chunk_rows * mean_nnz * 1.2 + 64.0 <= (double)stage_cap;
+                if (const char *v = ctx->opt("SG_FILL_CHUNK_ROWS"))
+                    if (atoi(v) >= 16 && atoi(v) < chunk_rows) chunk_rows = atoi(v);
                 staged_lds = fixed0 + (size_t)chunk_rows * 4 + (size_t)stage_cap * 4;
+                stage_words = stage_cap;
                 if (const char *v = ctx->opt("SG_FILL_STAGE_CAP"))
                     if (atoi(v) > 0 && (uint32_t)atoi(v) < stage_cap) stage_cap = (uint32_t)atoi(v);
             }
@@ -1187,6 +1229,12 @@
             }
             p->split = split;
             const int64_t wgs64 = (int64_t)p->n_tiles * split;
+            const bool one_chunk = staged && (int64_t)chunk_rows >= tile_cols / split &&
+                                   ((((size_t)B->n_cols + 1) / 2 + 3) & ~(size_t)3) + (size_t)stage_words >= (size_t)B->n_cols;
+            if (ctx->opt_is("SG_FILL_PRINT", '1'))
+                fprintf(stderr, "postings fill: rows %lld terms %lld tiles %d split %d chunk_rows %d stage_cap %u staged %d one_chunk %d\n",
+                        (long long)B->n_rows, (long long)B->n_cols, (int)p->n_tiles, (int)split, (int)chunk_rows, stage_cap, (int)staged,
+                        (int)one_chunk);
             uint32_t *cnt = nullptr;
             uint8_t *is_frequent = nullptr;
             st = sg_alloc(ctx, (size_t)(wgs64 * B->n_cols) + 1, &cnt);
@@ -1229,16 +1277,18 @@
                                            (const uint32_t *)p->d_term_start, (int32_t)B->n_cols, p->n_tiles, split, p->d_seg, p->d_ends,
                                            p->nt_pad, p->d_ends8, p->nv_pad, p->fold_log2, sc, p->d_score_ctx,
                                            p->d_filt ? p->d_filt + B->nnz : (uint32_t *)nullptr);
-                        if (staged && B->dtype == SG_F64)
-                            hipLaunchKernelGGL(postings_fill_staged<double>, dim3(wgs), dim3(1024), staged_lds, ctx->stream, B->d_indptr,
-                                               B->d_indices, (const double *)B->d_data, B->n_rows, tile_log2, (int32_t)B->n_cols, split,
-                                               chunk_rows, stage_cap, cnt, (const uint32_t *)p->d_term_start, (const uint8_t *)is_frequent,
-                                               p->d_filt, inv_norm, p->fold_log2);
-                        else if (staged)
-                            hipLaunchKernelGGL(postings_fill_staged<float>, dim3(wgs), dim3(1024), staged_lds, ctx->stream, B->d_indptr,
-                                               B->d_indices, (const float *)B->d_data, B->n_rows, tile_log2, (int32_t)B->n_cols, split,
-                                               chunk_rows, stage_cap, cnt, (const uint32_t *)p->d_term_start, (const uint8_t *)is_frequent,
-                                               p->d_filt, inv_norm, p->fold_log2);
+                        if (staged) {
+                            auto fill = [&](auto kernel, auto *data) {
+                                hipLaunchKernelGGL(kernel, dim3(wgs), dim3(1024), staged_lds, ctx->stream, B->d_indptr, B->d_indices, data,
+                                                   B->n_rows, tile_log2, (int32_t)B->n_cols, split, chunk_rows, stage_cap, cnt,
+                                                   (const uint32_t *)p->d_term_start, (const uint32_t *)p->d_term_len,
+                                                   (const uint8_t *)is_frequent, p->d_filt, inv_norm, p->fold_log2);
+                            };
+                            if (B->dtype == SG_F64 && one_chunk) fill(postings_fill_staged<double, true>, (const double *)B->d_data);
+                            else if (B->dtype == SG_F64) fill(postings_fill_staged<double, false>, (const double *)B->d_data);
+                            else if (one_chunk) fill(postings_fill_staged<float, true>, (const float *)B->d_data);
+                            else fill(postings_fill_staged<float, false>, (const float *)B->d_data);
+                        }
                         if (hipGetLastError() != hipSuccess) st = SG_ERR_HIP;
                         aux_written = st == SG_OK;
                     }
diff --git a/string_grouper_amd/csrc/sg_spgemm_pruned.hip b/string_grouper_amd/csrc/sg_spgemm_pruned.hip
--- a/string_grouper_amd/csrc/sg_spgemm_pruned.hip
+++ b/string_grouper_amd/csrc/sg_spgemm_pruned.hip
@@ -1464,9 +1464,8 @@
     uint32_t row_step = 1;
     uint32_t rows() const { return (row_hi - row_lo + row_step - 1u) / row_step; }
     const SgPairSink *d_sink = nullptr;
+    uint32_t *d_l1 = nullptr;
 };
-
-__global__ void pair_sink_kernel(SgPairSink v, SgPairSink *out) { *out = v; }
 
 bool sg_q8_applies(const sg_ctx *ctx, const sg_postings *Bt, double threshold) {
     if (!Bt->d_q8 || Bt->fold_log2 <= 0) return false;
@@ -1518,9 +1517,12 @@
 static int launch_both(sg_ctx *ctx, const sg_csr *A, const sg_postings *Bt, int32_t keep, sg_topn *r, T thr,
                        float s_budget, uint32_t *row_counter, uint32_t *flagged_count, uint32_t *flagged_rows,
                        unsigned long long *stats, const PairList &pl) {
-    uint32_t *l1 = nullptr;
-    SG_TRY(sg_alloc(ctx, (size_t)A->n_rows + 8, &l1));
-    int st = hipMemsetAsync(l1, 0, 4 * sizeof(uint32_t), ctx->stream) == hipSuccess ? SG_OK : SG_ERR_HIP;
+    uint32_t *l1 = pl.d_l1;
+    int st = SG_OK;
+    if (!l1) {
+        SG_TRY(sg_alloc(ctx, (size_t)A->n_rows + 8, &l1));
+        st = hipMemsetAsync(l1, 0, 4 * sizeof(uint32_t), ctx->stream) == hipSuccess ? SG_OK : SG_ERR_HIP;
+    }
     uint32_t *heavy = nullptr;
     uint32_t heavy_rounds = 0;
     if (SYM && FOLD_LOG2 > 0 && st == SG_OK) {
@@ -1559,7 +1561,7 @@
                 hipSuccess)
             st = SG_ERR_HIP;
     }
-    ctx->release(l1);
+    if (l1 != pl.d_l1) ctx->release(l1);
     return st;
 }
 
@@ -1660,6 +1662,7 @@
     if (st == SG_OK) st = sg_alloc(ctx, (size_t)n + 2, &cnt);
     if (st == SG_OK) st = sg_alloc(ctx, (size_t)n + 2, &cursor);
     if (st == SG_OK) st = sg_alloc(ctx, (size_t)n + 2, &flagged_rows);
+    if (st == SG_OK && !exact_all) st = sg_alloc(ctx, (size_t)n + 8, &pl.d_l1);
     unsigned long long *h = (unsigned long long *)ctx->h_stat_words;
     auto cleanup = [&]() {
         ctx->release(words);
@@ -1669,6 +1672,7 @@
         ctx->release(cnt);
         ctx->release(cursor);
         ctx->release(flagged_rows);
+        ctx->release(pl.d_l1);
         ctx->release(lcol);
         ctx->release(lval);
     };
@@ -1685,10 +1689,6 @@
     unsigned long long *d_stats3 = nullptr;
     st = sg_alloc(ctx, (size_t)8, &d_stats3);
     hipError_t e = hipSuccess;
-    if (st == SG_OK) {
-        st = SG_ZERO4(ctx, words, (128 + (size_t)pl.chunks) * sizeof(uint32_t), d_stats3, 8 * sizeof(unsigned long long), cnt,
-                      sizeof(uint32_t) * (size_t)(n + 2), cursor, sizeof(uint32_t) * (size_t)(n + 2));
-    }
     const float s_budget = prune_budget(Bt, threshold, delta);
     SgPairSink sink;
     sink.d_i = pl.d_i;
@@ -1700,8 +1700,12 @@
     sink.d_totals = pl.d_totals;
     sink.chunks = pl.chunks;
     if (st == SG_OK) {
-        hipLaunchKernelGGL(pair_sink_kernel, dim3(1), dim3(1), 0, ctx->stream, sink, (SgPairSink *)(words + 64));
-        if (hipGetLastError() != hipSuccess) st = SG_ERR_HIP;
+        void *const zp[] = {words, words + 80, d_stats3, cnt, cursor, pl.d_l1};
+        const size_t zb[] = {64 * sizeof(uint32_t), (48 + (size_t)pl.chunks) * sizeof(uint32_t), 8 * sizeof(unsigned long long),
+                             sizeof(uint32_t) * (size_t)(n + 2), sizeof(uint32_t) * (size_t)(n + 2), pl.d_l1 ? 4 * sizeof(uint32_t) : 0};
+        uint32_t sink_words[16] = {0};
+        memcpy(sink_words, &sink, sizeof(sink));
+        st = sg_zero_ranges_put(ctx, 6, zp, zb, words + 64, sink_words, sizeof(sink_words));
     }
     if (st == SG_OK && exact_all) {
         SgTimer kt(ctx, SG_K_SPGEMM_KERNEL);
@@ -1754,6 +1758,7 @@
             PairList first = pl, rest = pl;
             first.row_lo = (uint32_t)n - k_first;
             rest.row_hi = (uint32_t)n - k_first;
+            rest.d_l1 = nullptr;
             st = pruned_pass(first);
             if (st == SG_OK) {
                 e = hipMemcpyAsync(h, words, 24, hipMemcpyDeviceToHost, ctx->stream);
diff --git a/string_grouper_amd/csrc/sg_spgemm_topn.hip b/string_grouper_amd/csrc/sg_spgemm_topn.hip
--- a/string_grouper_amd/csrc/sg_spgemm_topn.hip
+++ b/string_grouper_amd/csrc/sg_spgemm_topn.hip
@@ -650,6 +650,7 @@
         view.n_rows = block;
         view.d_indptr = A->d_indptr + starts[b];
         view.owned = false;
+        view.d_row_hash = nullptr;
         e = hipMemsetAsync(words, 0, 8 * sizeof(uint32_t), ctx->stream);
         if (e == hipSuccess) e = hipMemsetAsync(scratch->d_counts, 0, sizeof(int32_t) * (size_t)block, ctx->stream);
         if (e == hipSuccess)
diff --git a/string_grouper_amd/csrc/sg_vectorize.hip b/string_grouper_amd/csrc/sg_vectorize.hip
--- a/string_grouper_amd/csrc/sg_vectorize.hip
+++ b/string_grouper_amd/csrc/sg_vectorize.hip
@@ -688,7 +688,7 @@
                                                                       const T *__restrict__ idf, int64_t n,
                                                                       const int64_t *__restrict__ indptr,
                                                                       int32_t *__restrict__ out_idx, T *__restrict__ out_val,
-                                                                      uint32_t *props) {
+                                                                      uint32_t *props, uint64_t *__restrict__ row_hash ) {
     const int lane = threadIdx.x & 63, sub = lane & 15, grp_shift = lane & 48;
     const int64_t row = ((int64_t)blockIdx.x * blockDim.x + threadIdx.x) >> 4;
     const bool valid = row < n;
@@ -725,6 +725,7 @@
     }
     float n2 = 0.f;
     uint32_t len = 0;
+    uint64_t hsum = 0;
     if (carry != 0.0) {
         const double nrm = __dsqrt_rn(carry);
         double s2 = 0.0;
@@ -742,19 +743,29 @@
             }
             const uint32_t km = (uint32_t)(__ballot(col >= 0) >> grp_shift) & 0xFFFFu;
             if (col >= 0) {
-                const int64_t o = o0 + kept_before + __popc(km & ((1u << sub) - 1u));
+                const int place = kept_before + __popc(km & ((1u << sub) - 1u));
+                const int64_t o = o0 + place;
                 const T v = (T)__ddiv_rn((double)w, nrm);
                 out_idx[o] = col;
                 out_val[o] = v;
                 s2 += (double)v * (double)v;
+                if (row_hash) hsum += sg_row_hash_entry(col, sg_row_hash_bits(v), (uint64_t)place);
             }
             kept_before += __popc(km);
         }
         len = (uint32_t)kept_before;
 #pragma unroll
         for (int d = 8; d > 0; d >>= 1) s2 += shfl_double(s2, lane ^ d);
+        if (row_hash) {
+#pragma unroll
+            for (int d = 8; d > 0; d >>= 1) {
+                const uint32_t lo32 = (uint32_t)__shfl_xor((int)(uint32_t)hsum, d, 64), hi32 = (uint32_t)__shfl_xor((int)(uint32_t)(hsum >> 32), d, 64);
+                hsum += ((uint64_t)hi32 << 32) | lo32;
+            }
+        }
         n2 = __double2float_ru(s2 * (1.0 + 1e-12));
     }
+    if (row_hash && valid && sub == 0) row_hash[row] = sg_row_hash_finish(hsum, (uint64_t)len);
     uint32_t nb = __float_as_uint(n2);
 #pragma unroll
     for (int d = 32; d > 0; d >>= 1) {
@@ -1169,6 +1180,28 @@
     return st;
 }
 
+#define SG_FIT_WORDS_COLUMNS 7
+struct FitWordsJob {
+    const uint32_t *total;
+    const uint32_t *longs[SG_FIT_WORDS_COLUMNS];
+    const int64_t *nnz[SG_FIT_WORDS_COLUMNS];
+    int n;
+};
+__global__ void fit_words_kernel(FitWordsJob job, uint32_t *__restrict__ out ) {
+    const int q = (int)threadIdx.x;
+    if (q == 0) {
+        out[0] = job.total[0];
+        out[1] = 0u;
+    }
+    if (q < job.n) {
+        out[2 + 4 * q] = job.longs[q] ? job.longs[q][0] : 0u;
+        out[3 + 4 * q] = 0u;
+        const unsigned long long z = job.nnz[q] ? (unsigned long long)job.nnz[q][0] : ~0ull;
+        out[4 + 4 * q] = (uint32_t)z;
+        out[5 + 4 * q] = (uint32_t)(z >> 32);
+    }
+}
+
 extern "C" int sg_vec_fit_end(sg_ctx *ctx, sg_vocab *v, int64_t n_docs_total) {
     SG_REQUIRE(ctx && v && v->impl, "null argument");
     SG_REQUIRE(v->n_terms == 0, "the vocabulary is already finished");
@@ -1180,8 +1213,9 @@
         if (v->sorted_mode) {
             st = finish_sorted_vocabulary(ctx, v);
         } else {
-            uint32_t *d_total = nullptr;
+            uint32_t *d_total = nullptr, *d_words = nullptr;
             st = sg_alloc(ctx, 4, &d_total);
+            if (st == SG_OK && im->caches.size() <= SG_FIT_WORDS_COLUMNS) st = sg_alloc(ctx, 4 + 4 * SG_FIT_WORDS_COLUMNS, &d_words);
             if (st == SG_OK) {
                 const unsigned grid = (unsigned)((v->key_space + 255) / 256);
                 (void)grid;
@@ -1200,8 +1234,24 @@
                 if (st != SG_OK) break;
                 uint32_t *hf = ctx->h_fetch;
                 const bool pinned = 4 * im->caches.size() + 4 <= SG_H_FETCH_WORDS;
-                hipError_t e = hipMemcpyAsync(pinned ? (void *)hf : (void *)&n_terms, d_total, 4, hipMemcpyDeviceToHost, ctx->stream);
-                for (size_t q = 0; q < im->caches.size() && e == hipSuccess; ++q) {
+                const bool packed = pinned && im->caches.size() <= SG_FIT_WORDS_COLUMNS && d_words != nullptr;
+                hipError_t e = hipSuccess;
+                if (packed) {
+                    FitWordsJob job;
+                    job.total = d_total;
+                    job.n = (int)im->caches.size();
+                    for (int q = 0; q < SG_FIT_WORDS_COLUMNS; ++q) {
+                        job.longs[q] = q < job.n ? im->caches[q].d_longs : nullptr;
+                        job.nnz[q] = q < job.n && im->caches[q].d_indptr ? im->caches[q].d_indptr + im->caches[q].n : nullptr;
+                    }
+                    hipLaunchKernelGGL(fit_words_kernel, dim3(1), dim3(64), 0, ctx->stream, job, d_words);
+                    e = hipGetLastError();
+                    if (e == hipSuccess)
+                        e = hipMemcpyAsync(hf, d_words, (4 + 4 * im->caches.size()) * sizeof(uint32_t), hipMemcpyDeviceToHost, ctx->stream);
+                } else {
+                    e = hipMemcpyAsync(pinned ? (void *)hf : (void *)&n_terms, d_total, 4, hipMemcpyDeviceToHost, ctx->stream);
+                }
+                for (size_t q = 0; q < im->caches.size() && e == hipSuccess && !packed; ++q) {
                     if (im->caches[q].d_longs)
                         e = hipMemcpyAsync(pinned ? (void *)(hf + 2 + 4 * q) : (void *)&n_long[q], im->caches[q].d_longs, 4, hipMemcpyDeviceToHost, ctx->stream);
                     if (e == hipSuccess && im->caches[q].d_indptr)
@@ -1234,6 +1284,7 @@
                 st = sg_exclusive_scan_positive_i32(ctx, im->d_df_table, (uint32_t *)v->d_key_to_col, v->key_space, d_total);
             }
             ctx->release(d_total);
+            ctx->release(d_words);
             if (st == SG_OK) {
                 v->n_terms = n_terms;
                 if (v->n_terms > 0) {
@@ -1419,7 +1470,7 @@
 
 template <typename T, typename KeyT, typename Lookup>
 static void launch_weight(sg_ctx *ctx, const TokenCache *tc, Lookup lookup, const sg_vocab *v, int64_t n, const int64_t *indptr,
-                          int32_t *idx, void *val, uint32_t *props) {
+                          int32_t *idx, void *val, uint32_t *props, uint64_t *row_hash ) {
     const char *pe = ctx->opt("SG_K2_PLAIN");
     const bool plain = pe && pe[0] == '1';
     if (plain)
@@ -1429,7 +1480,7 @@
     else
         hipLaunchKernelGGL((weight_normalize_rows16_kernel<T, KeyT, Lookup>), dim3((unsigned)((n + 15) / 16)), dim3(256), 0,
                            ctx->stream, (const int64_t *)tc->d_ub_ptr, (const int32_t *)tc->d_cnt, (const KeyT *)tc->d_keys,
-                           (const int32_t *)tc->d_tf, lookup, (const T *)v->d_idf, n, indptr, idx, (T *)val, props);
+                           (const int32_t *)tc->d_tf, lookup, (const T *)v->d_idf, n, indptr, idx, (T *)val, props, row_hash);
 }
 
 extern "C" int sg_vec_transform(sg_ctx *ctx, const sg_vocab *v, const sg_strings *strings, sg_csr **out) {
@@ -1513,18 +1564,26 @@
             st = sg_alloc(ctx, (size_t)4, &m->d_props_words);
             if (st == SG_OK && hipMemsetAsync(m->d_props_words, 0, 16, ctx->stream) != hipSuccess) st = SG_ERR_HIP;
         }
+        {
+            const bool plain_k2 = ctx->opt_is("SG_K2_PLAIN", '1');
+            const bool forced = ctx->opt_is("SG_COLLAPSE", '1') || ctx->opt_is("SG_COLLAPSE_LEFT", '1');
+            if (st == SG_OK && n >= 2 && nnz > 0 && v->idf_trusted && !plain_k2 && !ctx->opt_is("SG_ROW_HASH", '0') &&
+                !ctx->opt_is("SG_COLLAPSE", '0') && (forced || n >= 8192))
+                st = sg_alloc(ctx, (size_t)n + 1, &m->d_row_hash);
+        }
         if (st == SG_OK && n > 0) {
             uint32_t *props = m->d_props_words;
+            uint64_t *const rh = m->d_row_hash;
             if (v->sorted_mode) {
-                if (m->dtype == SG_F64) launch_weight<double, uint64_t>(ctx, tc, sorted, v, n, indptr, idx, val, props);
-                else launch_weight<float, uint64_t>(ctx, tc, sorted, v, n, indptr, idx, val, props);
+                if (m->dtype == SG_F64) launch_weight<double, uint64_t>(ctx, tc, sorted, v, n, indptr, idx, val, props, rh);
+                else launch_weight<float, uint64_t>(ctx, tc, sorted, v, n, indptr, idx, val, props, rh);
             } else if (tc->keys_are_columns) {
                 const ColumnsLookup cols{};
-                if (m->dtype == SG_F64) launch_weight<double, uint32_t>(ctx, tc, cols, v, n, indptr, idx, val, props);
-                else launch_weight<float, uint32_t>(ctx, tc, cols, v, n, indptr, idx, val, props);
+                if (m->dtype == SG_F64) launch_weight<double, uint32_t>(ctx, tc, cols, v, n, indptr, idx, val, props, rh);
+                else launch_weight<float, uint32_t>(ctx, tc, cols, v, n, indptr, idx, val, props, rh);
             } else {
-                if (m->dtype == SG_F64) launch_weight<double, uint32_t>(ctx, tc, dense, v, n, indptr, idx, val, props);
-                else launch_weight<float, uint32_t>(ctx, tc, dense, v, n, indptr, idx, val, props);
+                if (m->dtype == SG_F64) launch_weight<double, uint32_t>(ctx, tc, dense, v, n, indptr, idx, val, props, rh);
+                else launch_weight<float, uint32_t>(ctx, tc, dense, v, n, indptr, idx, val, props, rh);
             }
             if (hipGetLastError() != hipSuccess) st = SG_ERR_HIP;
         }
```
